# laclouis5/StructureDetector

Measured on AMD Instinct MI355X. Metric: images/sec (train fwd+bwd) and decode us/img at 512x512, higher is better.
Workload: dtype f32

## Files before the change

include/sdnet_hip.h:

```cpp
#ifndef SDNET_HIP_H
#define SDNET_HIP_H

#include <stddef.h>
#include <stdint.h>

#ifdef __cplusplus
extern "C" {
#endif

#define SD_ERR_INVALID   (-1)
#define SD_ERR_WORKSPACE (-2)
#define SD_ERR_ALIGN     (-3)

#define SD_MAX_TOPK 1024

typedef void* sd_stream_t;

int         sd_version(void);
const char* sd_last_error(void);
int         sd_build_flags(void);


int sd_clamped_sigmoid(const float* x, float* y, int64_t n, sd_stream_t stream);

// ... 80 lines not shown

typedef struct sd_loss_desc {
    const float* anchor_hm;  int64_t a_sb, a_sc;
    const float* part_hm;    int64_t p_sb, p_sc;
    const float* offsets;    int64_t o_sb, o_sc;
    const float* embeddings; int64_t e_sb, e_sc;
    const float* t_anchor_hm; int64_t ta_sb, ta_sc;
    const float* t_part_hm;   int64_t tp_sb, tp_sc;
    const int64_t* anchor_inds;
    const int64_t* part_inds;
    const float* anchor_offsets;
    const float* part_offsets;
    const float* t_embeddings;
    const uint8_t* anchor_mask;
    const uint8_t* part_mask;
    int B, M, N, h, w, K, P;
    int hm_loss_fn;
    float hm_weight, offset_weight, embedding_weight;
} sd_loss_desc;

size_t sd_loss_workspace_bytes(int B, int M, int N, int h, int w);
int sd_loss_fwd(const sd_loss_desc* d, float* out8, void* workspace, size_t workspace_bytes, sd_stream_t stream);

int sd_loss_fwd_per_image(const sd_loss_desc* d, float* out, void* workspace, size_t workspace_bytes, sd_stream_t stream);

int sd_loss_bwd(const sd_loss_desc* d, const float* out8, const float* grad_out, float* dhead, sd_stream_t stream);



typedef struct sd_conv_desc {
    int B, Hi, Wi, Cin, Ho, Wo, Cout, R, S, stride, pad;
} sd_conv_desc;

size_t sd_conv2d_fwd_workspace_bytes(const sd_conv_desc* d);
int sd_conv2d_fwd(const float* x_nhwc, const float* w_krsc, float* y_nhwc, const sd_conv_desc* d,
                  const float* scale, const float* shift, const float* residual, int res_up2, int relu,
                  void* workspace, size_t workspace_bytes, sd_stream_t stream);
size_t sd_conv2d_stem_fwd_workspace_bytes(const sd_conv_desc* d);
int sd_conv2d_stem_fwd(const float* x_nchw, const float* w_krsc, void* y_nhwc, const sd_conv_desc* d,
                       const float* scale, const float* shift, int relu, int out_bf16, void* workspace,
                       size_t workspace_bytes, sd_stream_t stream);

int    sd_conv2d_fwd_sb_supported(const sd_conv_desc* d, int bf16);
size_t sd_conv2d_fwd_sb_workspace_bytes(const sd_conv_desc* d, int bf16);
size_t sd_conv2d_fwd_sb_state_bytes(const sd_conv_desc* d, int bf16);
int sd_conv2d_fwd_sb(const void* x_nhwc, const void* w_krsc, void* y_nhwc, const sd_conv_desc* d, const float* scale, const float* shift,
                     const void* residual, int res_up2, int relu, int bf16, void* workspace, size_t workspace_bytes, void* state,
                     size_t state_bytes, sd_stream_t stream);

size_t sd_conv2d_stem_fwd_bn_stats_workspace_bytes(const sd_conv_desc* d);
int sd_conv2d_stem_fwd_bn_stats(const float* x_nchw, const float* w, float* y, const sd_conv_desc* d, float eps, float momentum,
                                float* running_mean, float* running_var, float* mean, float* invstd, void* workspace,
                                size_t workspace_bytes, sd_stream_t stream);

size_t sd_conv2d_fwd_bn_stats_workspace_bytes(const sd_conv_desc* d);
int sd_conv2d_fwd_bn_stats(const float* x, const float* w, float* y, const sd_conv_desc* d, float eps, float momentum,
                           float* running_mean, float* running_var, float* mean, float* invstd, void* workspace,
                           size_t workspace_bytes, sd_stream_t stream);
int sd_bn_finalize_scratch_rows(int rows);
int sd_bn_finalize_stats(const float* partial, int rows, int64_t M, int C, float eps, float momentum, float* running_mean,
                         float* running_var, float* mean, float* invstd, float* scratch, sd_stream_t stream);

size_t sd_conv2d_dgrad_bn_reduce_workspace_bytes(const sd_conv_desc* d);
int sd_conv2d_dgrad_bn_reduce(const float* dy, const float* w_t, float* dx, const sd_conv_desc* d, const float* residual,
                              const float* bn_x, const float* bn_y, int relu, const float* mean, const float* invstd,
                              const float* gamma, const float* beta, float* dgamma, float* dbeta, int accumulate,
                              float* means_out, void* workspace, size_t workspace_bytes, sd_stream_t stream);
int sd_bn_bwd_finalize(const float* partial, int rows, int64_t M, int C, float* dgamma, float* dbeta, int accumulate,
                       float* means_out, float* scratch, sd_stream_t stream);
int sd_bn_bwd_apply(const float* dy, const float* x, const float* y, int relu, int64_t M, int C, const float* mean,
                    const float* invstd, const float* gamma, const float* beta, const float* means, float* dx, float* g_out,
                    sd_stream_t stream);

int sd_set_option(const char* name, int value);

const char* sd_conv2d_kernel_name(const sd_conv_desc* d, int pass);

int sd_cast_f32_to_bf16(const float* x, void* y_bf16, int64_t n, sd_stream_t stream);
size_t sd_conv2d_fwd_bf16_workspace_bytes(const sd_conv_desc* d);
int sd_conv2d_fwd_bf16(const void* x_nhwc_bf16, const void* w_krsc_bf16, void* y_nhwc_bf16, const sd_conv_desc* d,
                       const float* scale, const float* shift, const void* residual_bf16, int res_up2, int relu,
                       void* workspace, size_t workspace_bytes, sd_stream_t stream);
int sd_maxpool3x3s2_fwd_bf16(const void* x_bf16, void* y_bf16, int B, int Hi, int Wi, int C, sd_stream_t stream);
int sd_stem_bn_relu_maxpool_fwd_bf16(const float* x_nchw, const float* w, const float* scale, const float* shift, void* y_bf16,
                                     const sd_conv_desc* d, sd_stream_t stream);

int sd_cast_bf16_to_f32(const void* x_bf16, float* y, int64_t n, sd_stream_t stream);
size_t sd_conv2d_fwd_bf16_bn_stats_workspace_bytes(const sd_conv_desc* d);
int sd_conv2d_fwd_bf16_bn_stats(const void* x_nhwc_bf16, const void* w_krsc_bf16, void* y_nhwc_bf16, const sd_conv_desc* d, float eps,
                                float momentum, float* running_mean, float* running_var, float* mean, float* invstd,
                                void* workspace, size_t workspace_bytes, sd_stream_t stream);
int sd_conv2d_stem_fwd_bn_stats_bf16mm(const float* x_nchw, const float* w, float* y, const sd_conv_desc* d, float eps, float momentum,
                                       float* running_mean, float* running_var, float* mean, float* invstd,
                                       void* workspace, size_t workspace_bytes, sd_stream_t stream);
int sd_conv2d_stem_fwd_bn_stats_bf16(const float* x_nchw, const float* w, void* y_bf16, const sd_conv_desc* d, float eps, float momentum,
                                     float* running_mean, float* running_var, float* mean, float* invstd, void* workspace,
                                     size_t workspace_bytes, sd_stream_t stream);
int sd_bn_relu_maxpool_fwd_bf16(const void* x_bf16, int B, int Hi, int Wi, int C, const float* mean, const float* invstd, const float* gamma,
                                const float* beta, void* y_pool_bf16, uint8_t* idx, sd_stream_t stream);
int sd_maxpool_bn_relu_bwd_bf16(const void* dpool_bf16, const uint8_t* idx, const void* x_bf16, int B, int Hi, int Wi, int C, const float* mean,
                                const float* invstd, const float* gamma, const float* beta, float* dx, float* dgamma, float* dbeta, int accumulate,
                                void* workspace, size_t workspace_bytes, sd_stream_t stream);
int sd_maxpool_bn_relu_bwd_bf16_dx16(const void* dpool_bf16, const uint8_t* idx, const void* x_bf16, int B, int Hi, int Wi, int C, const float* mean,
                                     const float* invstd, const float* gamma, const float* beta, void* dx_bf16, float* dgamma, float* dbeta,
                                     int accumulate, void* workspace, size_t workspace_bytes, sd_stream_t stream);
int sd_conv2d_transpose_weights_bf16(const float* w, void* w_t_bf16, int Cout, int taps, int Cin, sd_stream_t stream);

int sd_conv2d_fwd_bf16_head_supported(const sd_conv_desc* d, int head_co);
size_t sd_head_split_bf16_bytes(void);
int sd_head_split_bf16(const float* head_w, const float* head_bias, int head_co, void* prepared, sd_stream_t stream);
int sd_conv2d_fwd_bf16_head(const void* x_bf16, const void* w_bf16, const sd_conv_desc* d, const float* scale, const float* shift, int relu,
                            const void* head_prepared, int head_co, float* head_y, sd_stream_t stream);
int sd_conv2d_dgrad_bf16(const void* dy_bf16, const void* w_t_bf16, void* dx_bf16, const sd_conv_desc* d, const void* residual_bf16,
                         int res_mode, sd_stream_t stream);
size_t sd_conv2d_wgrad_bf16_workspace_bytes(const sd_conv_desc* d);
int sd_conv2d_wgrad_bf16(const void* dy_bf16, const void* x_nhwc_bf16, float* dw_krsc, const sd_conv_desc* d, int accumulate,
                         void* workspace, size_t workspace_bytes, sd_stream_t stream);
int sd_bn_apply_bf16(const void* x, void* y, int64_t M, int C, const float* mean, const float* invstd, const float* gamma,
                     const float* beta, const void* residual, int relu, uint8_t* relu_mask_out, sd_stream_t stream);
int sd_bn_bwd_bf16(const void* dy, const void* x, const void* y, int relu, int64_t M, int C, const float* mean, const float* invstd,
                   const float* gamma, const float* beta, void* dx, void* g_out, float* dgamma, float* dbeta, int accumulate,
                   void* workspace, size_t workspace_bytes, sd_stream_t stream);
int sd_bn_train_stats_bf16(const void* x, int64_t M, int C, float eps, float momentum, float* running_mean, float* running_var,
                           float* mean, float* invstd, void* workspace, size_t workspace_bytes, sd_stream_t stream);
int sd_col_sum_bf16(const void* x, int64_t M, int C, float* out, int accumulate, void* workspace, size_t workspace_bytes, sd_stream_t stream);
int sd_upsample2x_bwd_bf16(const void* dy, const void* add, void* dx, int B, int H, int W, int C, sd_stream_t stream);
int sd_head_fwd_bf16(const void* x_nhwc_bf16, const float* w, const float* bias, float* y_nchw, int B, int HW, int C,
                     int Co, sd_stream_t stream);
int sd_conv2d_dgrad(const float* dy_nhwc, const float* w_t, float* dx_nhwc, const sd_conv_desc* d,
                    const float* residual, sd_stream_t stream);
int sd_conv2d_dgrad_half_res(const float* dy, const float* w_t, float* dx, const sd_conv_desc* d, const float* residual_half,
                             sd_stream_t stream);
int sd_conv2d_transpose_weights(const float* w, float* w_t, int Cout, int taps, int Cin, sd_stream_t stream);
int sd_conv2d_transpose_weights_batched(const float* w_base, void* w_t_base, const int* table, int nconv, int total_blocks, int out_bf16,
                                        sd_stream_t stream);
size_t sd_conv2d_wgrad_workspace_bytes(const sd_conv_desc* d);
int sd_conv2d_wgrad(const float* dy_nhwc, const float* x_nhwc, float* dw_krsc, const sd_conv_desc* d,
                    int accumulate, void* workspace, size_t workspace_bytes, sd_stream_t stream);
size_t sd_conv2d_stem_wgrad_workspace_bytes(const sd_conv_desc* d);
int sd_conv2d_stem_wgrad(const float* dy_nhwc, const float* x_nchw, float* dw_krsc, const sd_conv_desc* d,
                         int accumulate, void* workspace, size_t workspace_bytes, sd_stream_t stream);
int sd_conv2d_stem_wgrad_bf16mm(const float* dy, const float* x_nchw, float* dw, const sd_conv_desc* d, int accumulate, void* workspace,
                                size_t workspace_bytes, sd_stream_t stream);
int sd_conv2d_stem_wgrad_bf16(const void* dy_bf16, const float* x_nchw, float* dw, const sd_conv_desc* d, int accumulate, void* workspace,
                              size_t workspace_bytes, sd_stream_t stream);

size_t sd_col_reduce_workspace_bytes(int64_t M, int C);
int sd_bn_train_stats(const float* x, int64_t M, int C, float eps, float momentum, float* running_mean,
                      float* running_var, float* mean, float* invstd, void* workspace, size_t workspace_bytes,
                      sd_stream_t stream);
int sd_bn_apply(const float* x, float* y, int64_t M, int C, const float* mean, const float* invstd,
                const float* gamma, const float* beta, const float* residual, int relu, uint8_t* relu_mask_out,
                sd_stream_t stream);
int sd_bn_fold(const float* gamma, const float* beta, const float* running_mean, const float* running_var,
               float eps, int C, float* scale, float* shift, sd_stream_t stream);
int sd_bn_bwd(const float* dy, const float* x, const float* y, int relu, int64_t M, int C, const float* mean,
              const float* invstd, const float* gamma, const float* beta, float* dx, float* g_out, float* dgamma,
              float* dbeta, int accumulate, void* workspace, size_t workspace_bytes, sd_stream_t stream);
int sd_col_sum(const float* x, int64_t M, int C, float* out, int accumulate, void* workspace,
               size_t workspace_bytes, sd_stream_t stream);

int sd_maxpool3x3s2_fwd(const float* x, float* y, uint8_t* idx, int B, int Hi, int Wi, int C, sd_stream_t stream);
int sd_maxpool3x3s2_bwd(const float* dy, const uint8_t* idx, float* dx, int B, int Hi, int Wi, int C, sd_stream_t stream);
int sd_bn_relu_maxpool_fwd(const float* x, int B, int Hi, int Wi, int C, const float* mean, const float* invstd, const float* gamma,
                           const float* beta, float* y_pool, uint8_t* idx, sd_stream_t stream);
int sd_maxpool_bn_relu_bwd(const float* dpool, const uint8_t* idx, const float* x, int B, int Hi, int Wi, int C, const float* mean,
                           const float* invstd, const float* gamma, const float* beta, float* dx, float* dgamma, float* dbeta,
                           int accumulate, void* workspace, size_t workspace_bytes, sd_stream_t stream);
int sd_upsample2x_bwd(const float* dy, const float* add, float* dx, int B, int H, int W, int C, sd_stream_t stream);

#define SD_HEAD_MAX_CO 256
int sd_head_fwd(const float* x_nhwc, const float* w, const float* bias, float* y_nchw, int B, int HW, int C, int Co,
                sd_stream_t stream);
size_t sd_head_bwd_workspace_bytes(int B, int HW, int C, int Co);
int sd_head_bwd(const float* dy_nchw, const float* x_nhwc, const float* w, float* dx_nhwc, float* dw, float* dbias,
                int B, int HW, int C, int Co, int accumulate, void* workspace, size_t workspace_bytes, sd_stream_t stream);
int sd_head_bwd_bf16(const float* dy, const void* x_bf16, const float* w, void* dx_bf16, float* dw, float* dbias, int B, int HW, int C, int Co,
                     int accumulate, void* workspace, size_t workspace_bytes, sd_stream_t stream);

int sd_adam_step(float* param, const float* grad, float* exp_avg, float* exp_avg_sq, int64_t n, int step,
                 float lr, float beta1, float beta2, float eps, float grad_scale, sd_stream_t stream);

#define SD_COMM_ID_BYTES 128
int sd_allreduce_unique_id(void* id_out);
int sd_allreduce_init(const void* id, int rank, int world, void** comm_out);
int sd_allreduce_run(void* comm, float* buf, int64_t count, sd_stream_t stream);
int sd_allreduce_destroy(void* comm);

int sd_comm_sim_copy(const void* src, void* dst, size_t src_bytes, size_t move_bytes, int workgroups, float gbps, sd_stream_t stream);

double sd_mfma_bf16_stream_flops(int iters);
int    sd_mfma_bf16_stream(const void* operands64k, float* out, int iters, sd_stream_t stream);

int         sd_range_enabled(void);
const char* sd_range_library(void);
int         sd_range_push(const char* name);
int         sd_range_pop(void);
int         sd_range_mark(const char* name);

#ifdef __cplusplus
}
#endif
#endif
```

structuredetector_amd/_lib.py:

```python
from __future__ import annotations

import ctypes as C
import os
from pathlib import Path

import torch

_HERE = Path(__file__).resolve().parent
LIB_PATH = Path(os.environ.get("SDNET_HIP_LIB", _HERE / "csrc" / "libsdnet_hip.so"))

_lib = None

c_f32p = C.c_void_p
c_i64 = C.c_int64
c_int = C.c_int
c_float = C.c_float
c_size = C.c_size_t
c_vp = C.c_void_p


class SdError(RuntimeError):
    pass


class LossDesc(C.Structure):
    _fields_ = [
        ("anchor_hm", c_vp), ("a_sb", c_i64), ("a_sc", c_i64),
        ("part_hm", c_vp), ("p_sb", c_i64), ("p_sc", c_i64),
        ("offsets", c_vp), ("o_sb", c_i64), ("o_sc", c_i64),
        ("embeddings", c_vp), ("e_sb", c_i64), ("e_sc", c_i64),
        ("t_anchor_hm", c_vp), ("ta_sb", c_i64), ("ta_sc", c_i64),
        ("t_part_hm", c_vp), ("tp_sb", c_i64), ("tp_sc", c_i64),
        ("anchor_inds", c_vp), ("part_inds", c_vp),
        ("anchor_offsets", c_vp), ("part_offsets", c_vp), ("t_embeddings", c_vp),
        ("anchor_mask", c_vp), ("part_mask", c_vp),
        ("B", c_int), ("M", c_int), ("N", c_int), ("h", c_int), ("w", c_int), ("K", c_int), ("P", c_int),
        ("hm_loss_fn", c_int),
        ("hm_weight", c_float), ("offset_weight", c_float), ("embedding_weight", c_float),
    ]


class ConvDesc(C.Structure):
    _fields_ = [(n, c_int) for n in ("B", "Hi", "Wi", "Cin", "Ho", "Wo", "Cout", "R", "S", "stride", "pad")]


_MAP = [c_vp, c_i64, c_i64]
_PEAK_OUT = [c_vp, c_vp, c_vp, c_vp, c_vp]

_SIGNATURES = {
    "sd_version": (c_int, []),
    "sd_last_error": (C.c_char_p, []),
    "sd_build_flags": (c_int, []),
    "sd_clamped_sigmoid": (c_int, [c_vp, c_vp, c_i64, c_vp]),
    "sd_nms5": (c_int, _MAP + [c_vp, c_int, c_int, c_int, c_int, c_int, c_vp]),
    "sd_topk_workspace_bytes": (c_size, [c_int] * 5),
    "sd_topk": (c_int, _MAP + [c_int] * 5 + _PEAK_OUT + [c_vp, c_size, c_vp]),
    "sd_transpose_and_gather": (c_int, _MAP + [c_int, c_int, c_i64, c_vp, c_int, c_vp, c_vp]),
    "sd_hypot": (c_int, [c_vp, c_vp, c_i64, c_vp]),
    "sd_decode_peaks_workspace_bytes": (c_size, [c_int] * 5),
    "sd_decode_peaks": (c_int, _MAP + [c_int] * 5 + _PEAK_OUT + [c_vp, c_size, c_vp]),
    "sd_decode_workspace_bytes": (c_size, [c_int] * 7),
    "sd_decode_packed_words": (c_size, [c_int] * 3),
    "sd_decode": (c_int, _MAP * 4 + [c_int] * 7 + [c_float, c_float, c_int, c_vp, c_vp, c_size, c_vp]),
    "sd_decode_state_bytes": (c_size, [c_int] * 5),
    "sd_decode_fused_supported": (c_int, [c_int] * 7),
    "sd_decode_fused_recommended": (c_int, [c_int] * 8),
    "sd_stream_synchronize": (c_int, [c_vp]),
    "sd_selfcheck_sigmoid": (c_int, [c_vp, c_vp]),
    "sd_decode_fused_workspace_bytes": (c_size, [c_int] * 7),
    "sd_decode_fused": (c_int, _MAP * 4 + [c_int] * 7 + [c_float, c_float, c_int, c_vp, c_vp, c_size, c_vp, c_size, c_vp]),
    "sd_decode_group": (c_int, [c_vp] * 6 + _MAP * 2 + [c_int] * 5 + [c_float, c_float, c_vp, c_vp]),
    "sd_preprocess_workspace_bytes": (c_size, [c_int] * 4),
    "sd_preprocess_images": (c_int, [c_vp] + [c_int] * 5 + [c_vp, c_vp, c_int, c_vp, c_vp, c_int, c_vp, C.POINTER(c_float), C.POINTER(c_float),
                                                c_vp, c_vp, c_size, c_vp]),
    "sd_preprocess_jitter_workspace_bytes": (c_size, [c_int] * 5),
    "sd_preprocess_images_jitter": (c_int, [c_vp] + [c_int] * 5 + [c_vp, c_vp, c_int, c_vp, c_vp, c_int, c_vp, c_vp, c_vp, C.POINTER(c_float), C.POINTER(c_float),
                                            c_vp, c_vp, c_size, c_vp]),
    "sd_preprocess_images_list": (c_int, [c_vp] + [c_int] * 5 + [c_vp, c_vp, c_int, c_vp, c_vp, c_int, c_vp, C.POINTER(c_float), C.POINTER(c_float),
                                                     c_vp, c_vp, c_size, c_vp]),
    "sd_preprocess_images_list_jitter": (c_int, [c_vp] + [c_int] * 5 + [c_vp, c_vp, c_int, c_vp, c_vp, c_int, c_vp, c_vp, c_vp, C.POINTER(c_float),
                                                            C.POINTER(c_float), c_vp, c_vp, c_size, c_vp]),
    "sd_render_targets": (c_int, [c_vp, c_vp, c_vp, c_int, c_int, c_int, c_int, c_float, c_vp, c_vp]),
    "sd_loss_workspace_bytes": (c_size, [c_int] * 5),
    "sd_loss_fwd": (c_int, [C.POINTER(LossDesc), c_vp, c_vp, c_size, c_vp]),
    "sd_loss_fwd_per_image": (c_int, [C.POINTER(LossDesc), c_vp, c_vp, c_size, c_vp]),
    "sd_loss_bwd": (c_int, [C.POINTER(LossDesc), c_vp, c_vp, c_vp, c_vp]),
    "sd_conv2d_fwd_workspace_bytes": (c_size, [C.POINTER(ConvDesc)]),
    "sd_conv2d_fwd": (c_int, [c_vp, c_vp, c_vp, C.POINTER(ConvDesc), c_vp, c_vp, c_vp, c_int, c_int, c_vp, c_size, c_vp]),
    "sd_conv2d_fwd_sb_supported": (c_int, [C.POINTER(ConvDesc), c_int]),
    "sd_conv2d_fwd_sb_workspace_bytes": (c_size, [C.POINTER(ConvDesc), c_int]),
    "sd_conv2d_fwd_sb_state_bytes": (c_size, [C.POINTER(ConvDesc), c_int]),
    "sd_conv2d_fwd_sb": (c_int, [c_vp, c_vp, c_vp, C.POINTER(ConvDesc), c_vp, c_vp, c_vp, c_int, c_int, c_int, c_vp, c_size, c_vp, c_size, c_vp]),
    "sd_conv2d_stem_fwd_workspace_bytes": (c_size, [C.POINTER(ConvDesc)]),
    "sd_conv2d_stem_fwd": (c_int, [c_vp, c_vp, c_vp, C.POINTER(ConvDesc), c_vp, c_vp, c_int, c_int, c_vp, c_size, c_vp]),
    "sd_cast_f32_to_bf16": (c_int, [c_vp, c_vp, c_i64, c_vp]),
    "sd_conv2d_fwd_bf16_workspace_bytes": (c_size, [C.POINTER(ConvDesc)]),
    "sd_conv2d_fwd_bf16": (c_int, [c_vp, c_vp, c_vp, C.POINTER(ConvDesc), c_vp, c_vp, c_vp, c_int, c_int, c_vp, c_size, c_vp]),
    "sd_conv2d_fwd_bf16_head_supported": (c_int, [C.POINTER(ConvDesc), c_int]),
    "sd_head_split_bf16_bytes": (c_size, []),
    "sd_head_split_bf16": (c_int, [c_vp, c_vp, c_int, c_vp, c_vp]),
    "sd_conv2d_fwd_bf16_head": (c_int, [c_vp, c_vp, C.POINTER(ConvDesc), c_vp, c_vp, c_int, c_vp, c_int, c_vp, c_vp]),
    "sd_cast_bf16_to_f32": (c_int, [c_vp, c_vp, c_i64, c_vp]),
    "sd_conv2d_fwd_bf16_bn_stats_workspace_bytes": (c_size, [c_vp]),
    "sd_conv2d_fwd_bf16_bn_stats": (c_int, [c_vp, c_vp, c_vp, c_vp, c_float, c_float, c_vp, c_vp, c_vp, c_vp, c_vp, c_size, c_vp]),
    "sd_conv2d_wgrad_bf16_workspace_bytes": (c_size, [c_vp]),
    "sd_conv2d_wgrad_bf16": (c_int, [c_vp, c_vp, c_vp, c_vp, c_int, c_vp, c_size, c_vp]),
    "sd_conv2d_transpose_weights_bf16": (c_int, [c_vp, c_vp, c_int, c_int, c_int, c_vp]),
    "sd_conv2d_dgrad_bf16": (c_int, [c_vp, c_vp, c_vp, c_vp, c_vp, c_int, c_vp]),
    "sd_bn_apply_bf16": (c_int, [c_vp, c_vp, c_i64, c_int, c_vp, c_vp, c_vp, c_vp, c_vp, c_int, c_vp, c_vp]),
    "sd_bn_bwd_bf16": (c_int, [c_vp, c_vp, c_vp, c_int, c_i64, c_int, c_vp, c_vp, c_vp, c_vp, c_vp, c_vp, c_vp, c_vp, c_int, c_vp, c_size, c_vp]),
    "sd_bn_train_stats_bf16": (c_int, [c_vp, c_i64, c_int, c_float, c_float, c_vp, c_vp, c_vp, c_vp, c_vp, c_size, c_vp]),
    "sd_col_sum_bf16": (c_int, [c_vp, c_i64, c_int, c_vp, c_int, c_vp, c_size, c_vp]),
    "sd_upsample2x_bwd_bf16": (c_int, [c_vp, c_vp, c_vp, c_int, c_int, c_int, c_int, c_vp]),
    "sd_maxpool3x3s2_fwd_bf16": (c_int, [c_vp, c_vp, c_int, c_int, c_int, c_int, c_vp]),
    "sd_stem_bn_relu_maxpool_fwd_bf16": (c_int, [c_vp, c_vp, c_vp, c_vp, c_vp, c_vp, c_vp]),
    "sd_head_fwd_bf16": (c_int, [c_vp, c_vp, c_vp, c_vp, c_int, c_int, c_int, c_int, c_vp]),
    "sd_conv2d_dgrad": (c_int, [c_vp, c_vp, c_vp, C.POINTER(ConvDesc), c_vp, c_vp]),
    "sd_conv2d_transpose_weights": (c_int, [c_vp, c_vp, c_int, c_int, c_int, c_vp]),
    "sd_conv2d_transpose_weights_batched": (c_int, [c_vp, c_vp, c_vp, c_int, c_int, c_int, c_vp]),
    "sd_conv2d_wgrad_workspace_bytes": (c_size, [C.POINTER(ConvDesc)]),
    "sd_conv2d_wgrad": (c_int, [c_vp, c_vp, c_vp, C.POINTER(ConvDesc), c_int, c_vp, c_size, c_vp]),
    "sd_conv2d_stem_wgrad_workspace_bytes": (c_size, [C.POINTER(ConvDesc)]),
    "sd_conv2d_stem_wgrad": (c_int, [c_vp, c_vp, c_vp, C.POINTER(ConvDesc), c_int, c_vp, c_size, c_vp]),
    "sd_conv2d_stem_wgrad_bf16mm": (c_int, [c_vp, c_vp, c_vp, C.POINTER(ConvDesc), c_int, c_vp, c_size, c_vp]),
    "sd_conv2d_stem_wgrad_bf16": (c_int, [c_vp, c_vp, c_vp, C.POINTER(ConvDesc), c_int, c_vp, c_size, c_vp]),
    "sd_col_reduce_workspace_bytes": (c_size, [c_i64, c_int]),
    "sd_bn_train_stats": (c_int, [c_vp, c_i64, c_int, c_float, c_float, c_vp, c_vp, c_vp, c_vp, c_vp, c_size, c_vp]),
    "sd_bn_apply": (c_int, [c_vp, c_vp, c_i64, c_int, c_vp, c_vp, c_vp, c_vp, c_vp, c_int, c_vp, c_vp]),
    "sd_bn_fold": (c_int, [c_vp, c_vp, c_vp, c_vp, c_float, c_int, c_vp, c_vp, c_vp]),
    "sd_bn_bwd": (c_int, [c_vp, c_vp, c_vp, c_int, c_i64, c_int, c_vp, c_vp, c_vp, c_vp, c_vp, c_vp, c_vp, c_vp, c_int, c_vp, c_size, c_vp]),
    "sd_col_sum": (c_int, [c_vp, c_i64, c_int, c_vp, c_int, c_vp, c_size, c_vp]),
    "sd_maxpool3x3s2_fwd": (c_int, [c_vp, c_vp, c_vp, c_int, c_int, c_int, c_int, c_vp]),
    "sd_maxpool3x3s2_bwd": (c_int, [c_vp, c_vp, c_vp, c_int, c_int, c_int, c_int, c_vp]),
    "sd_upsample2x_bwd": (c_int, [c_vp, c_vp, c_vp, c_int, c_int, c_int, c_int, c_vp]),
    "sd_head_fwd": (c_int, [c_vp, c_vp, c_vp, c_vp, c_int, c_int, c_int, c_int, c_vp]),
    "sd_head_bwd_workspace_bytes": (c_size, [c_int] * 4),
    "sd_head_bwd": (c_int, [c_vp] * 6 + [c_int] * 5 + [c_vp, c_size, c_vp]),
    "sd_head_bwd_bf16": (c_int, [c_vp] * 6 + [c_int] * 5 + [c_vp, c_size, c_vp]),
    "sd_adam_step": (c_int, [c_vp, c_vp, c_vp, c_vp, c_i64, c_int, c_float, c_float, c_float, c_float, c_float, c_vp]),
    "sd_conv2d_kernel_name": (C.c_char_p, [c_vp, c_int]),
    "sd_set_option": (c_int, [C.c_char_p, c_int]),
    "sd_decode_set_option": (c_int, [C.c_char_p, c_int]),
    "sd_conv2d_stem_fwd_bn_stats_workspace_bytes": (c_size, [c_vp]),
    "sd_conv2d_stem_fwd_bn_stats": (c_int, [c_vp, c_vp, c_vp, c_vp, c_float, c_float, c_vp, c_vp, c_vp, c_vp, c_vp, c_size, c_vp]),
    "sd_conv2d_stem_fwd_bn_stats_bf16mm": (c_int, [c_vp, c_vp, c_vp, c_vp, c_float, c_float, c_vp, c_vp, c_vp, c_vp, c_vp, c_size, c_vp]),
    "sd_conv2d_stem_fwd_bn_stats_bf16": (c_int, [c_vp, c_vp, c_vp, c_vp, c_float, c_float, c_vp, c_vp, c_vp, c_vp, c_vp, c_size, c_vp]),
    "sd_conv2d_dgrad_half_res": (c_int, [c_vp] * 6),
    "sd_bn_relu_maxpool_fwd": (c_int, [c_vp, c_int, c_int, c_int, c_int] + [c_vp] * 7),
    "sd_bn_relu_maxpool_fwd_bf16": (c_int, [c_vp, c_int, c_int, c_int, c_int] + [c_vp] * 7),
    "sd_maxpool_bn_relu_bwd": (c_int, [c_vp, c_vp, c_vp, c_int, c_int, c_int, c_int] + [c_vp] * 7 + [c_int, c_vp, c_size, c_vp]),
    "sd_maxpool_bn_relu_bwd_bf16": (c_int, [c_vp, c_vp, c_vp, c_int, c_int, c_int, c_int] + [c_vp] * 7 + [c_int, c_vp, c_size, c_vp]),
    "sd_maxpool_bn_relu_bwd_bf16_dx16": (c_int, [c_vp, c_vp, c_vp, c_int, c_int, c_int, c_int] + [c_vp] * 7 + [c_int, c_vp, c_size, c_vp]),
    "sd_conv2d_fwd_bn_stats_workspace_bytes": (c_size, [c_vp]),
    "sd_conv2d_fwd_bn_stats": (c_int, [c_vp, c_vp, c_vp, c_vp, c_float, c_float, c_vp, c_vp, c_vp, c_vp, c_vp, c_size, c_vp]),
    "sd_conv2d_dgrad_bn_reduce_workspace_bytes": (c_size, [c_vp]),
    "sd_conv2d_dgrad_bn_reduce": (c_int, [c_vp] * 5 + [c_vp, c_vp, c_int] + [c_vp] * 6 + [c_int, c_vp, c_vp, c_size, c_vp]),
    "sd_bn_bwd_finalize": (c_int, [c_vp, c_int, c_i64, c_int, c_vp, c_vp, c_int, c_vp, c_vp, c_vp]),
    "sd_bn_bwd_apply": (c_int, [c_vp, c_vp, c_vp, c_int, c_i64, c_int] + [c_vp] * 8),
    "sd_bn_finalize_scratch_rows": (c_int, [c_int]),
    "sd_bn_finalize_stats": (c_int, [c_vp, c_int, c_i64, c_int, c_float, c_float, c_vp, c_vp, c_vp, c_vp, c_vp, c_vp]),
    "sd_allreduce_unique_id": (c_int, [c_vp]),
    "sd_allreduce_init": (c_int, [c_vp, c_int, c_int, C.POINTER(c_vp)]),
    "sd_allreduce_run": (c_int, [c_vp, c_vp, c_i64, c_vp]),
    "sd_allreduce_destroy": (c_int, [c_vp]),
    "sd_mfma_bf16_stream_flops": (C.c_double, [c_int]),
    "sd_mfma_bf16_stream": (c_int, [c_vp, c_vp, c_int, c_vp]),
    "sd_comm_sim_copy": (c_int, [c_vp, c_vp, c_size, c_size, c_int, c_float, c_vp]),
    "sd_range_enabled": (c_int, []),
    "sd_range_library": (C.c_char_p, []),
    "sd_range_push": (c_int, [C.c_char_p]),
    "sd_range_pop": (c_int, []),
    "sd_range_mark": (c_int, [C.c_char_p]),
}


def declared_symbols():
    return sorted(_SIGNATURES)


def lib():
    global _lib
    if _lib is None:
        if not LIB_PATH.exists():
            raise SdError(
                f"{LIB_PATH} not found: build it with `python -c 'import __graft_entry__ as g; g.build()'` "
                f"(or `make -C {LIB_PATH.parent}`); structuredetector_amd has no CPU / eager fallback.")
        handle = C.CDLL(str(LIB_PATH))
        for name, (res, args) in _SIGNATURES.items():
            fn = getattr(handle, name)
            fn.restype = res
            fn.argtypes = args
        flags = handle.sd_build_flags()
        if flags and os.environ.get("SDNET_ALLOW_ABLATION") != "1":
            raise SdError(f"{LIB_PATH} is a timing-only ablation build (sd_build_flags = {flags}: SD_ABLATE_* switches make the conv "
                          "kernels compute wrong results on purpose); rebuild without EXTRA=-DSD_ABLATE_... "
                          "(set SDNET_ALLOW_ABLATION=1 only for timing experiments)")
        _lib = handle
    return _lib


def check(rc: int, what: str = ""):
    if rc != 0:
        msg = lib().sd_last_error().decode(errors="replace")
        raise SdError(f"{what or 'libsdnet_hip'} failed (code {rc}): {msg}")


def stream() -> int:
    try:
        return torch._C._cuda_getCurrentRawStream(torch.cuda.current_device())
    except AttributeError:
        return torch.cuda.current_stream().cuda_stream


def require_cuda(*tensors):
    for t in tensors:
        if not t.is_cuda:
            raise SdError("structuredetector_amd ops need tensors on the GPU (device 'cuda'); got a "
                          f"{t.device} tensor and there is no CPU fallback")


def map_view(t: torch.Tensor):
    if t.dtype != torch.float32:
        t = t.float()
    B, Cc, h, w = t.shape
    s0, s1, s2, s3 = t.stride()
    ptr = t.data_ptr()
    if not (s3 == 1 and s2 == w and s1 >= h * w and (B == 1 or s0 >= h * w) and s1 % 4 == 0 and s0 % 4 == 0 and ptr % 16 == 0):
        t = t.contiguous()
        s0, s1 = t.stride(0), t.stride(1)
        ptr = t.data_ptr()
    return t, ptr, s0, s1


_ws_cache: dict = {}


def workspace(nbytes: int, device) -> torch.Tensor:
    key = (device.index if device.index is not None else torch.cuda.current_device(), stream())
    buf = _ws_cache.get(key)
    if buf is None or buf.numel() < nbytes:
        buf = torch.empty(max(nbytes, 1 << 20), dtype=torch.uint8, device=device)
        _ws_cache[key] = buf
    return buf


_state_cache: dict = {}


def zero_state(nbytes: int, device, tag: str = "conv") -> torch.Tensor:
    key = (device.index if device.index is not None else torch.cuda.current_device(), stream(), tag)
    buf = _state_cache.get(key)
    if buf is None or buf.numel() < nbytes:
        if buf is not None:
            torch.cuda.current_stream().synchronize()
        buf = torch.zeros(max(nbytes, 1 << 16), dtype=torch.uint8, device=device)
        _state_cache[key] = buf
    return buf
```

structuredetector_amd/csrc/sd_common.h:

```cpp
#pragma once
#include <hip/hip_runtime.h>
#include <stdint.h>
#include <stdio.h>
#include "../../include/sdnet_hip.h"

namespace sd {

void set_error(const char* fmt, ...);

#define SD_REQUIRE(cond, code, ...)            \
    do {                                       \
        if (!(cond)) {                         \
            sd::set_error(__VA_ARGS__);        \
            return (code);                     \
        }                                      \
    } while (0)

#define SD_HIP(call)                                                                    \
    do {                                                                                \
        hipError_t e_ = (call);                                                         \
        if (e_ != hipSuccess) {                                                         \
            sd::set_error("%s failed: %s (%s:%d)", #call, hipGetErrorString(e_), __FILE__, __LINE__); \
            return (int)e_;                                                             \
        }                                                                               \
    } while (0)

#define SD_LAUNCH_CHECK()                                                               \
    do {                                                                                \
        hipError_t e_ = hipGetLastError();                                              \
        if (e_ != hipSuccess) {                                                         \
            sd::set_error("kernel launch failed: %s (%s:%d)", hipGetErrorString(e_), __FILE__, __LINE__); \
            return (int)e_;                                                             \
        }                                                                               \
    } while (0)

static inline bool aligned16(const void* p) { return (reinterpret_cast<uintptr_t>(p) & 15u) == 0; }
static inline size_t align_up(size_t v, size_t a) { return (v + a - 1) / a * a; }
static inline int cdiv(int64_t a, int64_t b) { return (int)((a + b - 1) / b); }

constexpr float kClampLo = 1e-6f;
constexpr float kClampHi = (float)(1.0 - 1e-6);

__device__ __forceinline__ float sigmoid_raw(float x) { return 1.0f / (1.0f + expf(-x)); }
__device__ __forceinline__ float clamped_sigmoid(float x) {
    return fminf(fmaxf(sigmoid_raw(x), kClampLo), kClampHi);
}

__device__ __forceinline__ float bf16_to_f32(uint16_t v) { return __uint_as_float((uint32_t)v << 16); }
__device__ __forceinline__ uint16_t f32_to_bf16(float v) { return __builtin_bit_cast(uint16_t, (__bf16)v); }
typedef float sd_f32x4_nt __attribute__((ext_vector_type(4)));
__device__ __forceinline__ float4 ld4(const float* p, int64_t i) {
    const sd_f32x4_nt v = __builtin_nontemporal_load(reinterpret_cast<const sd_f32x4_nt*>(p) + i);
    return make_float4(v[0], v[1], v[2], v[3]);
}
__device__ __forceinline__ float4 ld4(const uint16_t* p, int64_t i) {
    const uint2 r = reinterpret_cast<const uint2*>(p)[i];
    return make_float4(bf16_to_f32((uint16_t)(r.x & 0xffff)), bf16_to_f32((uint16_t)(r.x >> 16)), bf16_to_f32((uint16_t)(r.y & 0xffff)),
                       bf16_to_f32((uint16_t)(r.y >> 16)));
}
__device__ __forceinline__ void st4(float* p, int64_t i, const float4 v) { reinterpret_cast<float4*>(p)[i] = v; }
__device__ __forceinline__ void st4(uint16_t* p, int64_t i, const float4 v) {
    uint2 pk;
    pk.x = (uint32_t)f32_to_bf16(v.x) | ((uint32_t)f32_to_bf16(v.y) << 16);
    pk.y = (uint32_t)f32_to_bf16(v.z) | ((uint32_t)f32_to_bf16(v.w) << 16);
    reinterpret_cast<uint2*>(p)[i] = pk;
}

constexpr int HEAD_NARROW_MAX_CO = 32;
int head_wide_check(const char* fn, int64_t P, int C, int Co);
int head_wide_fwd(const float* x, const float* w, const float* bias, float* y, int B, int HW, int C, int Co, hipStream_t st);
int head_wide_fwd_bf16(const void* x, const float* w, const float* bias, float* y, int B, int HW, int C, int Co, hipStream_t st);
size_t head_wide_bwd_workspace_bytes(int64_t P, int C, int Co);
int head_wide_wgrad(const float* dy, const float* x, float* partial, int B, int HW, int C, int Co, hipStream_t st, int& rows);
int head_wide_dgrad(const float* dy, const float* w, float* dx, int B, int HW, int C, int Co, hipStream_t st);

__device__ __forceinline__ float wave_sum(float v) {
#pragma unroll
    for (int o = 32; o > 0; o >>= 1) v += __shfl_down(v, o, 64);
    return v;
}
__device__ __forceinline__ double wave_sum(double v) {
#pragma unroll
    for (int o = 32; o > 0; o >>= 1) v += __shfl_down(v, o, 64);
    return v;
}

}
```

structuredetector_amd/csrc/sd_nn.hip:

```cpp
#include "sd_common.h"
#include "sd_mfma.h"
#include <type_traits>

namespace sd {

constexpr int RED_ROWS_PER_BLOCK = 256;

template <int MODE, typename T = float>
__global__ __launch_bounds__(256) void k_col_reduce(const T* __restrict__ a, const T* __restrict__ b, const T* __restrict__ y,
                                                     const float* __restrict__ mean, const float* __restrict__ invstd,
                                                     const float* __restrict__ gamma, const float* __restrict__ beta, int relu,
                                                     int64_t M, int C, float* __restrict__ partial, int rpb) {
    __shared__ float4 red[2][256];
    const int cols = C >> 2;
    const int lanes = 256 / cols;
    const int col = threadIdx.x % cols, rl = threadIdx.x / cols;
    const int64_t r0 = (int64_t)blockIdx.x * rpb;
    const int64_t r1 = min(r0 + rpb, M);
    float4 s0 = make_float4(0.f, 0.f, 0.f, 0.f), s1 = s0;
    float4 mu = s0, is = s0, ga = s0, be = s0;
    if (MODE == 1 && rl < lanes) {
        mu = reinterpret_cast<const float4*>(mean)[col];
        is = reinterpret_cast<const float4*>(invstd)[col];
        if (relu == 2) { ga = reinterpret_cast<const float4*>(gamma)[col]; be = reinterpret_cast<const float4*>(beta)[col]; }
    }
    if (rl < lanes) {
#pragma unroll 4
        for (int64_t r = r0 + rl; r < r1; r += lanes) {
            const float4 v = ld4(a, r * cols + col);
            if (MODE == 0) {
                s0.x += v.x; s0.y += v.y; s0.z += v.z; s0.w += v.w;
                s1.x += v.x * v.x; s1.y += v.y * v.y; s1.z += v.z * v.z; s1.w += v.w * v.w;
            } else if (MODE == 2) {
                s0.x += v.x; s0.y += v.y; s0.z += v.z; s0.w += v.w;
            } else {
                float4 g = v;
                const float4 xv = ld4(b, r * cols + col);
                if (relu == 1) {
                    const float4 yy = ld4(y, r * cols + col);
                    g.x = yy.x > 0.f ? g.x : 0.f; g.y = yy.y > 0.f ? g.y : 0.f;
                    g.z = yy.z > 0.f ? g.z : 0.f; g.w = yy.w > 0.f ? g.w : 0.f;
                } else if (relu == 2) {
                    g.x = ((xv.x - mu.x) * is.x * ga.x + be.x) > 0.f ? g.x : 0.f; g.y = ((xv.y - mu.y) * is.y * ga.y + be.y) > 0.f ? g.y : 0.f;
                    g.z = ((xv.z - mu.z) * is.z * ga.z + be.z) > 0.f ? g.z : 0.f; g.w = ((xv.w - mu.w) * is.w * ga.w + be.w) > 0.f ? g.w : 0.f;
                } else if (relu == 3) {
                    const uint8_t mb = reinterpret_cast<const uint8_t*>(y)[r * cols + col];
                    g.x = (mb & 1) ? g.x : 0.f; g.y = (mb & 2) ? g.y : 0.f; g.z = (mb & 4) ? g.z : 0.f; g.w = (mb & 8) ? g.w : 0.f;
                }
                s0.x += g.x; s0.y += g.y; s0.z += g.z; s0.w += g.w;
                s1.x += g.x * ((xv.x - mu.x) * is.x); s1.y += g.y * ((xv.y - mu.y) * is.y);
                s1.z += g.z * ((xv.z - mu.z) * is.z); s1.w += g.w * ((xv.w - mu.w) * is.w);
            }
        }
    }
    red[0][threadIdx.x] = s0;
    red[1][threadIdx.x] = s1;
    __syncthreads();
    if (rl == 0) {
        for (int l = 1; l < lanes; ++l) {
            const float4 u = red[0][l * cols + col], w = red[1][l * cols + col];
            s0.x += u.x; s0.y += u.y; s0.z += u.z; s0.w += u.w;
            s1.x += w.x; s1.y += w.y; s1.z += w.z; s1.w += w.w;
        }
        float* dst = partial + (int64_t)blockIdx.x * 2 * C;
        reinterpret_cast<float4*>(dst)[col] = s0;
        reinterpret_cast<float4*>(dst + C)[col] = s1;
    }
}

__global__ __launch_bounds__(256) void k_rows_fold(const float* __restrict__ in, int rows, int W, int slab, float* __restrict__ out) {
    __shared__ float4 red[256];
    const int cols = W >> 2, lanes = 256 / cols;
    const int col = threadIdx.x % cols, rl = threadIdx.x / cols;
    const int r0 = blockIdx.x * slab, r1 = min(r0 + slab, rows);
    float4 s = make_float4(0.f, 0.f, 0.f, 0.f);
    if (rl < lanes) {
#pragma unroll 4
        for (int r = r0 + rl; r < r1; r += lanes) {
            const float4 v = reinterpret_cast<const float4*>(in + (int64_t)r * W)[col];
            s.x += v.x; s.y += v.y; s.z += v.z; s.w += v.w;
        }
    }
    red[threadIdx.x] = s;
    __syncthreads();
    if (rl == 0) {
        for (int l = 1; l < lanes; ++l) { const float4 u = red[l * cols + col]; s.x += u.x; s.y += u.y; s.z += u.z; s.w += u.w; }
        reinterpret_cast<float4*>(out + (int64_t)blockIdx.x * W)[col] = s;
    }
}

template <int FIN>
__global__ __launch_bounds__(256) void k_col_finalize(const float* __restrict__ partial, int nblocks, int C, double M, float eps,
                                                       float momentum, float* __restrict__ out0, float* __restrict__ out1,
                                                       float* __restrict__ run_mean, float* __restrict__ run_var,
                                                       float* __restrict__ aux0, float* __restrict__ aux1, int accumulate) {
    __shared__ double r0[4][4], r1[4][4];
    const int lc = threadIdx.x & 3, lr = threadIdx.x >> 2;
    const int c = blockIdx.x * 4 + lc;
    double s0 = 0.0, s1 = 0.0;
    if (c < C) {
        double t0[8] = {0, 0, 0, 0, 0, 0, 0, 0}, t1[8] = {0, 0, 0, 0, 0, 0, 0, 0};
        for (int b = lr; b < nblocks; b += 64 * 8) {
            float v0[8], v1[8];
#pragma unroll
            for (int u = 0; u < 8; ++u) {
                const int row = b + 64 * u;
                const int64_t o = (int64_t)(row < nblocks ? row : 0) * 2 * C + c;
                v0[u] = partial[o];
                v1[u] = partial[o + C];
            }
#pragma unroll
            for (int u = 0; u < 8; ++u) {
                const bool ok = b + 64 * u < nblocks;
                t0[u] += ok ? (double)v0[u] : 0.0; t1[u] += ok ? (double)v1[u] : 0.0;
            }
        }
        s0 = ((t0[0] + t0[1]) + (t0[2] + t0[3])) + ((t0[4] + t0[5]) + (t0[6] + t0[7]));
        s1 = ((t1[0] + t1[1]) + (t1[2] + t1[3])) + ((t1[4] + t1[5]) + (t1[6] + t1[7]));
    }
#pragma unroll
    for (int o = 4; o < 64; o <<= 1) { s0 += __shfl_xor(s0, o); s1 += __shfl_xor(s1, o); }
    if ((threadIdx.x & 63) < 4) { r0[threadIdx.x >> 6][lc] = s0; r1[threadIdx.x >> 6][lc] = s1; }
    __syncthreads();
    if (lr != 0 || c >= C) return;
    s0 = (r0[0][lc] + r0[1][lc]) + (r0[2][lc] + r0[3][lc]);
    s1 = (r1[0][lc] + r1[1][lc]) + (r1[2][lc] + r1[3][lc]);
    if (FIN == 0) {
        const double mean = s0 / M;
        const double var = fmax(s1 / M - mean * mean, 0.0);
        out0[c] = (float)mean;
        out1[c] = (float)(1.0 / sqrt(var + (double)eps));
        if (run_mean) {
            const double unb = M > 1.0 ? var * M / (M - 1.0) : var;
            run_mean[c] = (float)((1.0 - momentum) * run_mean[c] + momentum * mean);
            run_var[c] = (float)((1.0 - momentum) * run_var[c] + momentum * unb);
        }
    } else if (FIN == 1) {
        out0[c] = (accumulate ? out0[c] : 0.f) + (float)s1;
        out1[c] = (accumulate ? out1[c] : 0.f) + (float)s0;
        aux0[c] = (float)(s0 / M);
        aux1[c] = (float)(s1 / M);
    } else {
        out0[c] = (accumulate ? out0[c] : 0.f) + (float)s0;
    }
}

template <typename T>
__global__ __launch_bounds__(256) void k_bn_apply(const T* __restrict__ x, T* __restrict__ y, int64_t n4, int C,
                                                   const float* __restrict__ mean, const float* __restrict__ invstd,
                                                   const float* __restrict__ gamma, const float* __restrict__ beta,
                                                   const T* __restrict__ res, int relu, uint8_t* __restrict__ mask) {
    const int64_t stride = (int64_t)gridDim.x * 256;
    const int cols = C >> 2;
    const bool fixed = stride % cols == 0;
    const int col0 = (int)(((int64_t)blockIdx.x * 256 + threadIdx.x) % cols);
    float4 mu = reinterpret_cast<const float4*>(mean)[col0], is = reinterpret_cast<const float4*>(invstd)[col0];
    float4 g = reinterpret_cast<const float4*>(gamma)[col0], b = reinterpret_cast<const float4*>(beta)[col0];
    for (int64_t i = (int64_t)blockIdx.x * 256 + threadIdx.x; i < n4; i += stride) {
        const float4 v = ld4(x, i);
        if (!fixed) {
            const int col = (int)(i % cols);
            mu = reinterpret_cast<const float4*>(mean)[col]; is = reinterpret_cast<const float4*>(invstd)[col];
            g = reinterpret_cast<const float4*>(gamma)[col]; b = reinterpret_cast<const float4*>(beta)[col];
        }
        float4 o;
        o.x = (v.x - mu.x) * is.x * g.x + b.x; o.y = (v.y - mu.y) * is.y * g.y + b.y;
        o.z = (v.z - mu.z) * is.z * g.z + b.z; o.w = (v.w - mu.w) * is.w * g.w + b.w;
        if (res) {
            const float4 r = ld4(res, i);
            o.x += r.x; o.y += r.y; o.z += r.z; o.w += r.w;
        }
        if (mask) mask[i] = (uint8_t)((o.x > 0.f ? 1 : 0) | (o.y > 0.f ? 2 : 0) | (o.z > 0.f ? 4 : 0) | (o.w > 0.f ? 8 : 0));
        if (relu) { o.x = fmaxf(o.x, 0.f); o.y = fmaxf(o.y, 0.f); o.z = fmaxf(o.z, 0.f); o.w = fmaxf(o.w, 0.f); }
        st4(y, i, o);
    }
}

__global__ __launch_bounds__(256) void k_bn_fold(const float* gamma, const float* beta, const float* rm, const float* rv, float eps,
                                                  int C, float* scale, float* shift) {
    const int c = blockIdx.x * 256 + threadIdx.x;
    if (c >= C) return;
    const float s = gamma[c] / sqrtf(rv[c] + eps);
    scale[c] = s;
    shift[c] = beta[c] - rm[c] * s;
}

template <typename T>
__global__ __launch_bounds__(256) void k_bn_bwd_apply(const T* __restrict__ dy, const T* __restrict__ x, const T* __restrict__ y,
                                                       int relu, int64_t n4, int C, const float* __restrict__ mean,
                                                       const float* __restrict__ invstd, const float* __restrict__ gamma,
                                                       const float* __restrict__ beta, const float* __restrict__ mg,
                                                       const float* __restrict__ mgx, T* __restrict__ dx, T* __restrict__ g_out) {
    const int64_t stride = (int64_t)gridDim.x * 256;
    const int cols = C >> 2;
    const bool fixed = stride % cols == 0;
    const int col0 = (int)(((int64_t)blockIdx.x * 256 + threadIdx.x) % cols);
    float4 mu = reinterpret_cast<const float4*>(mean)[col0], is = reinterpret_cast<const float4*>(invstd)[col0];
    float4 ga = reinterpret_cast<const float4*>(gamma)[col0];
    float4 be = relu == 2 ? reinterpret_cast<const float4*>(beta)[col0] : make_float4(0.f, 0.f, 0.f, 0.f);
    float4 a = reinterpret_cast<const float4*>(mg)[col0], b = reinterpret_cast<const float4*>(mgx)[col0];
    for (int64_t i = (int64_t)blockIdx.x * 256 + threadIdx.x; i < n4; i += stride) {
        float4 g = ld4(dy, i);
        const float4 xv = ld4(x, i);
        if (!fixed) {
            const int col = (int)(i % cols);
            mu = reinterpret_cast<const float4*>(mean)[col]; is = reinterpret_cast<const float4*>(invstd)[col];
            ga = reinterpret_cast<const float4*>(gamma)[col];
            if (relu == 2) be = reinterpret_cast<const float4*>(beta)[col];
            a = reinterpret_cast<const float4*>(mg)[col]; b = reinterpret_cast<const float4*>(mgx)[col];
        }
        if (relu == 1) {
            const float4 yy = ld4(y, i);
            g.x = yy.x > 0.f ? g.x : 0.f; g.y = yy.y > 0.f ? g.y : 0.f; g.z = yy.z > 0.f ? g.z : 0.f; g.w = yy.w > 0.f ? g.w : 0.f;
        } else if (relu == 3) {
            const uint8_t mb = reinterpret_cast<const uint8_t*>(y)[i];
            g.x = (mb & 1) ? g.x : 0.f; g.y = (mb & 2) ? g.y : 0.f; g.z = (mb & 4) ? g.z : 0.f; g.w = (mb & 8) ? g.w : 0.f;
        } else if (relu == 2) {
            g.x = ((xv.x - mu.x) * is.x * ga.x + be.x) > 0.f ? g.x : 0.f; g.y = ((xv.y - mu.y) * is.y * ga.y + be.y) > 0.f ? g.y : 0.f;
            g.z = ((xv.z - mu.z) * is.z * ga.z + be.z) > 0.f ? g.z : 0.f; g.w = ((xv.w - mu.w) * is.w * ga.w + be.w) > 0.f ? g.w : 0.f;
        }
        float4 o;
        o.x = ga.x * is.x * (g.x - a.x - (xv.x - mu.x) * is.x * b.x);
        o.y = ga.y * is.y * (g.y - a.y - (xv.y - mu.y) * is.y * b.y);
        o.z = ga.z * is.z * (g.z - a.z - (xv.z - mu.z) * is.z * b.z);
        o.w = ga.w * is.w * (g.w - a.w - (xv.w - mu.w) * is.w * b.w);
        st4(dx, i, o);
        if (g_out) st4(g_out, i, g);
    }
}

__global__ __launch_bounds__(256) void k_maxpool_fwd(const float* __restrict__ x, float* __restrict__ y, uint8_t* __restrict__ idx, int B,
                                                      int Hi, int Wi, int Ho, int Wo, int C) {
    const int cols = C >> 2;
    const int64_t n4 = (int64_t)B * Ho * Wo * cols;
    const int64_t i = (int64_t)blockIdx.x * 256 + threadIdx.x;
    if (i >= n4) return;
    const int col = (int)(i % cols);
    int64_t t = i / cols;
    const int ox = (int)(t % Wo); t /= Wo;
    const int oy = (int)(t % Ho);
    const int b = (int)(t / Ho);
    float4 m = make_float4(-INFINITY, -INFINITY, -INFINITY, -INFINITY);
    uchar4 w = make_uchar4(0, 0, 0, 0);
#pragma unroll
    for (int r = 0; r < 3; ++r) {
#pragma unroll
        for (int s = 0; s < 3; ++s) {
            const int iy = oy * 2 - 1 + r, ix = ox * 2 - 1 + s;
            if (iy < 0 || iy >= Hi || ix < 0 || ix >= Wi) continue;
            const float4 v = reinterpret_cast<const float4*>(x + (((int64_t)b * Hi + iy) * Wi + ix) * C)[col];
            const uint8_t tap = (uint8_t)(r * 3 + s);
            if (v.x > m.x) { m.x = v.x; w.x = tap; }
            if (v.y > m.y) { m.y = v.y; w.y = tap; }
            if (v.z > m.z) { m.z = v.z; w.z = tap; }
            if (v.w > m.w) { m.w = v.w; w.w = tap; }
        }
    }
    reinterpret_cast<float4*>(y)[i] = m;
    reinterpret_cast<uchar4*>(idx)[i] = w;
}

__global__ __launch_bounds__(256) void k_maxpool_bwd(const float* __restrict__ dy, const uint8_t* __restrict__ idx, float* __restrict__ dx,
                                                      int B, int Hi, int Wi, int Ho, int Wo, int C) {
    const int cols = C >> 2;
    const int64_t n4 = (int64_t)B * Hi * Wi * cols;
    const int64_t i = (int64_t)blockIdx.x * 256 + threadIdx.x;
    if (i >= n4) return;
    const int col = (int)(i % cols);
    int64_t t = i / cols;
    const int ix = (int)(t % Wi); t /= Wi;
    const int iy = (int)(t % Hi);
    const int b = (int)(t / Hi);
    float4 acc = make_float4(0.f, 0.f, 0.f, 0.f);
    for (int oy = (iy + 1) / 2 - ((iy + 1) % 2 == 0 ? 1 : 0); oy <= (iy + 1) / 2; ++oy) {
        if (oy < 0 || oy >= Ho) continue;
        const int r = iy - (oy * 2 - 1);
        if (r < 0 || r > 2) continue;
        for (int ox = (ix + 1) / 2 - ((ix + 1) % 2 == 0 ? 1 : 0); ox <= (ix + 1) / 2; ++ox) {
            if (ox < 0 || ox >= Wo) continue;
            const int s = ix - (ox * 2 - 1);
            if (s < 0 || s > 2) continue;
            const int64_t o = (((int64_t)b * Ho + oy) * Wo + ox) * cols + col;
            const uchar4 w = reinterpret_cast<const uchar4*>(idx)[o];
            const float4 g = reinterpret_cast<const float4*>(dy)[o];
            const uint8_t tap = (uint8_t)(r * 3 + s);
            if (w.x == tap) acc.x += g.x;
            if (w.y == tap) acc.y += g.y;
            if (w.z == tap) acc.z += g.z;
            if (w.w == tap) acc.w += g.w;
        }
    }
    reinterpret_cast<float4*>(dx)[i] = acc;
}

template <typename XT, typename PT>
__global__ __launch_bounds__(256) void k_bn_relu_maxpool_fwd(const XT* __restrict__ x, const float* __restrict__ mean,
                                                              const float* __restrict__ invstd, const float* __restrict__ gamma,
                                                              const float* __restrict__ beta, PT* __restrict__ y,
                                                              uint8_t* __restrict__ idx, int B, int Hi, int Wi, int Ho, int Wo, int C) {
    const int cols = C >> 2;
    const int64_t n4 = (int64_t)B * Ho * Wo * cols;
    const int64_t i = (int64_t)blockIdx.x * 256 + threadIdx.x;
    if (i >= n4) return;
    const int col = (int)(i % cols);
    int64_t t = i / cols;
    const int ox = (int)(t % Wo); t /= Wo;
    const int oy = (int)(t % Ho);
    const int b = (int)(t / Ho);
    const float4 mu = reinterpret_cast<const float4*>(mean)[col], is = reinterpret_cast<const float4*>(invstd)[col];
    const float4 ga = reinterpret_cast<const float4*>(gamma)[col], be = reinterpret_cast<const float4*>(beta)[col];
    float4 m = make_float4(-INFINITY, -INFINITY, -INFINITY, -INFINITY);
    uchar4 w = make_uchar4(0, 0, 0, 0);
#pragma unroll
    for (int r = 0; r < 3; ++r) {
#pragma unroll
        for (int s = 0; s < 3; ++s) {
            const int iy = oy * 2 - 1 + r, ix = ox * 2 - 1 + s;
            if (iy < 0 || iy >= Hi || ix < 0 || ix >= Wi) continue;
            const float4 xv = ld4(x, (((int64_t)b * Hi + iy) * Wi + ix) * cols + col);
            float4 v;
            v.x = fmaxf((xv.x - mu.x) * is.x * ga.x + be.x, 0.f); v.y = fmaxf((xv.y - mu.y) * is.y * ga.y + be.y, 0.f);
            v.z = fmaxf((xv.z - mu.z) * is.z * ga.z + be.z, 0.f); v.w = fmaxf((xv.w - mu.w) * is.w * ga.w + be.w, 0.f);
            const uint8_t tap = (uint8_t)(r * 3 + s);
            if (v.x > m.x) { m.x = v.x; w.x = tap; }
// ... 201 lines not shown
    const float4 ga = reinterpret_cast<const float4*>(gamma)[col], be = reinterpret_cast<const float4*>(beta)[col];
    const float4 a = reinterpret_cast<const float4*>(mg)[col], bb = reinterpret_cast<const float4*>(mgx)[col];
    const int64_t p00 = (((int64_t)b * Hi + 2 * k) * Wi + 2 * j) * cols + col;
    const int64_t off[4] = {p00, p00 + cols, p00 + (int64_t)Wi * cols, p00 + (int64_t)(Wi + 1) * cols};
    float4 xv[4], g[4];
#pragma unroll
    for (int u = 0; u < 4; ++u) xv[u] = ld4(x, off[u]);
    pool_relu_grad_quad(dpool, idx, b, k, j, col, cols, Ho, Wo, xv, mu, is, ga, be, g);
#pragma unroll
    for (int u = 0; u < 4; ++u) {
        float4 o;
        o.x = ga.x * is.x * (g[u].x - a.x - (xv[u].x - mu.x) * is.x * bb.x);
        o.y = ga.y * is.y * (g[u].y - a.y - (xv[u].y - mu.y) * is.y * bb.y);
        o.z = ga.z * is.z * (g[u].z - a.z - (xv[u].z - mu.z) * is.z * bb.z);
        o.w = ga.w * is.w * (g[u].w - a.w - (xv[u].w - mu.w) * is.w * bb.w);
        st4(dx, off[u], o);
    }
}
#undef SD_ADD4

__global__ __launch_bounds__(256) void k_pool_bn_bwd_reduce(const float* __restrict__ dpool, const uint8_t* __restrict__ idx,
                                                             const float* __restrict__ x, const float* __restrict__ mean,
                                                             const float* __restrict__ invstd, const float* __restrict__ gamma,
                                                             const float* __restrict__ beta, int Hi, int Wi, int Ho, int Wo, int64_t M,
                                                             int C, float* __restrict__ partial) {
    __shared__ float4 red[2][256];
    const int cols = C >> 2, lanes = 256 / cols;
    const int col = threadIdx.x % cols, rl = threadIdx.x / cols;
    const int64_t r0 = (int64_t)blockIdx.x * RED_ROWS_PER_BLOCK, r1 = min(r0 + RED_ROWS_PER_BLOCK, M);
    float4 s0 = make_float4(0.f, 0.f, 0.f, 0.f), s1 = s0;
    if (rl < lanes) {
        const float4 mu = reinterpret_cast<const float4*>(mean)[col], is = reinterpret_cast<const float4*>(invstd)[col];
        const float4 ga = reinterpret_cast<const float4*>(gamma)[col], be = reinterpret_cast<const float4*>(beta)[col];
        for (int64_t r = r0 + rl; r < r1; r += lanes) {
            const int ix = (int)(r % Wi);
            const int64_t t = r / Wi;
            const int iy = (int)(t % Hi), b = (int)(t / Hi);
            const float4 xv = reinterpret_cast<const float4*>(x + r * C)[col];
            const float4 g = pool_relu_grad(dpool, idx, b, iy, ix, col, cols, Ho, Wo, xv, mu, is, ga, be);
            s0.x += g.x; s0.y += g.y; s0.z += g.z; s0.w += g.w;
            s1.x += g.x * ((xv.x - mu.x) * is.x); s1.y += g.y * ((xv.y - mu.y) * is.y);
            s1.z += g.z * ((xv.z - mu.z) * is.z); s1.w += g.w * ((xv.w - mu.w) * is.w);
        }
    }
    red[0][threadIdx.x] = s0;
    red[1][threadIdx.x] = s1;
    __syncthreads();
    if (rl == 0) {
        for (int l = 1; l < lanes; ++l) {
            const float4 u = red[0][l * cols + col], w = red[1][l * cols + col];
            s0.x += u.x; s0.y += u.y; s0.z += u.z; s0.w += u.w;
            s1.x += w.x; s1.y += w.y; s1.z += w.z; s1.w += w.w;
        }
        float* dst = partial + (int64_t)blockIdx.x * 2 * C;
        reinterpret_cast<float4*>(dst)[col] = s0;
        reinterpret_cast<float4*>(dst + C)[col] = s1;
    }
}

__global__ __launch_bounds__(256) void k_pool_bn_bwd_apply(const float* __restrict__ dpool, const uint8_t* __restrict__ idx,
                                                            const float* __restrict__ x, const float* __restrict__ mean,
                                                            const float* __restrict__ invstd, const float* __restrict__ gamma,
                                                            const float* __restrict__ beta, const float* __restrict__ mg,
                                                            const float* __restrict__ mgx, int Hi, int Wi, int Ho, int Wo, int64_t n4, int C,
                                                            float* __restrict__ dx) {
    const int64_t i = (int64_t)blockIdx.x * 256 + threadIdx.x;
    if (i >= n4) return;
    const int cols = C >> 2;
    const int col = (int)(i % cols);
    const int64_t r = i / cols;
    const int ix = (int)(r % Wi);
    const int64_t t = r / Wi;
    const int iy = (int)(t % Hi), b = (int)(t / Hi);
    const float4 mu = reinterpret_cast<const float4*>(mean)[col], is = reinterpret_cast<const float4*>(invstd)[col];
    const float4 ga = reinterpret_cast<const float4*>(gamma)[col], be = reinterpret_cast<const float4*>(beta)[col];
    const float4 xv = reinterpret_cast<const float4*>(x)[i];
    const float4 g = pool_relu_grad(dpool, idx, b, iy, ix, col, cols, Ho, Wo, xv, mu, is, ga, be);
    const float4 a = reinterpret_cast<const float4*>(mg)[col], bb = reinterpret_cast<const float4*>(mgx)[col];
    float4 o;
    o.x = ga.x * is.x * (g.x - a.x - (xv.x - mu.x) * is.x * bb.x);
    o.y = ga.y * is.y * (g.y - a.y - (xv.y - mu.y) * is.y * bb.y);
    o.z = ga.z * is.z * (g.z - a.z - (xv.z - mu.z) * is.z * bb.z);
    o.w = ga.w * is.w * (g.w - a.w - (xv.w - mu.w) * is.w * bb.w);
    reinterpret_cast<float4*>(dx)[i] = o;
}

template <typename T>
__global__ __launch_bounds__(256) void k_up2_bwd(const T* __restrict__ dy, const T* __restrict__ add, T* __restrict__ dx, int B,
                                                  int H, int W, int C) {
    const int cols = C >> 2;
    const int64_t n4 = (int64_t)B * H * W * cols;
    const int64_t i = (int64_t)blockIdx.x * 256 + threadIdx.x;
    if (i >= n4) return;
    const int col = (int)(i % cols);
    int64_t t = i / cols;
    const int x = (int)(t % W); t /= W;
    const int y = (int)(t % H);
    const int b = (int)(t / H);
    const T* base = dy + (((int64_t)b * 2 * H + 2 * y) * 2 * W + 2 * x) * C;
    const float4 v0 = ld4(base, col), v1 = ld4(base + C, col);
    const float4 v2 = ld4(base + (int64_t)2 * W * C, col);
    const float4 v3 = ld4(base + (int64_t)2 * W * C + C, col);
    float4 o = make_float4(v0.x + v1.x + v2.x + v3.x, v0.y + v1.y + v2.y + v3.y, v0.z + v1.z + v2.z + v3.z, v0.w + v1.w + v2.w + v3.w);
    if (add) {
        const float4 a = ld4(add, i);
        o.x += a.x; o.y += a.y; o.z += a.z; o.w += a.w;
    }
    st4(dx, i, o);
}

__global__ __launch_bounds__(256) void k_head_fwd(const float* __restrict__ x, const float* __restrict__ w, const float* __restrict__ bias,
                                                   float* __restrict__ y, int64_t M, int HW, int C, int Co) {
    extern __shared__ __attribute__((aligned(16))) float lds[];
    const int LD = C + 4;
    float* xs = lds;
    float* ws = lds + 64 * LD;
    const int64_t m0 = (int64_t)blockIdx.x * 64;
    const int c4 = C >> 2;
    for (int i = threadIdx.x; i < 64 * c4; i += 256) {
        const int row = i / c4, col = i - row * c4;
        const int64_t m = m0 + row;
        const float4 v = m < M ? reinterpret_cast<const float4*>(x + m * C)[col] : make_float4(0.f, 0.f, 0.f, 0.f);
        *reinterpret_cast<float4*>(xs + row * LD + col * 4) = v;
    }
    for (int i = threadIdx.x; i < Co * C; i += 256) ws[i] = w[i];
    __syncthreads();
    const int px = threadIdx.x & 63, grp = threadIdx.x >> 6;
    float acc[HEAD_NARROW_MAX_CO / 4];
#pragma unroll
    for (int j = 0; j < HEAD_NARROW_MAX_CO / 4; ++j) acc[j] = 0.f;
    for (int c = 0; c < C; c += 4) {
        const float4 v = *reinterpret_cast<const float4*>(xs + px * LD + c);
#pragma unroll
        for (int j = 0; j < HEAD_NARROW_MAX_CO / 4; ++j) {
            const int co = grp + 4 * j;
            if (co < Co) {
                const float4 ww = *reinterpret_cast<const float4*>(ws + co * C + c);
                acc[j] += v.x * ww.x + v.y * ww.y + v.z * ww.z + v.w * ww.w;
            }
        }
    }
    const int64_t m = m0 + px;
    if (m < M) {
        const int64_t b = m / HW, pix = m - b * HW;
#pragma unroll
        for (int j = 0; j < HEAD_NARROW_MAX_CO / 4; ++j) {
            const int co = grp + 4 * j;
            if (co < Co) y[(b * Co + co) * HW + pix] = acc[j] + bias[co];
        }
    }
}

constexpr int HF_NST = 4;
__global__ __launch_bounds__(256) void k_head_fwd_f32_c128(const float* __restrict__ x, const float* __restrict__ w, const float* __restrict__ bias,
                                                            float* __restrict__ y, int HW, int Co, int ntiles) {
    extern __shared__ __attribute__((aligned(16))) float hf_lds[];
    const int lane = threadIdx.x & 63, wave = __builtin_amdgcn_readfirstlane(threadIdx.x >> 6);
    float* const T = hf_lds + wave * (HF_NST * 2048);
    const uint32_t t_base = lds_addr(T);
    const int row = lane & 15, kq = lane >> 4;
    f32x4 bw[8];
#pragma unroll
    for (int j = 0; j < 8; ++j) {
        bw[j] = f32x4{0.f, 0.f, 0.f, 0.f};
        if (row < Co) bw[j] = *reinterpret_cast<const f32x4*>(w + row * 128 + 16 * j + 4 * kq);
    }
    const float bv = row < Co ? bias[row] : 0.f;
    const int nwaves = gridDim.x * 4;
    const int dr = lane >> 5, dsl = lane & 31;
#define HF_ISSUE(t_, st_)                                                                                          \
    {                                                                                                              \
        const int64_t m0_ = (int64_t)min((t_), ntiles - 1) * 16;                                                  \
        _Pragma("unroll") for (int d = 0; d < 8; ++d) {                                                            \
            const int r = 2 * d + dr;                                                                              \
            lds_dma16(x + (m0_ + r) * 128 + ((dsl ^ (r & 15)) << 2), T + (st_) * 2048 + d * 256);                   \
        }                                                                                                          \
    }
    int tile = blockIdx.x * 4 + wave;
#pragma unroll
    for (int s = 0; s < HF_NST - 1; ++s) HF_ISSUE(tile + s * nwaves, s)
    int stage = 0;
    for (; tile < ntiles; tile += nwaves) {
        const int nst = stage == 0 ? HF_NST - 1 : stage - 1;
        HF_ISSUE(tile + (HF_NST - 1) * nwaves, nst)
        wait_vmcnt<8 * (HF_NST - 1)>();
        const uint32_t a0 = t_base + (uint32_t)stage * 8192u + (uint32_t)row * 512u;
        f32x4 a[8];
#pragma unroll
        for (int j = 0; j < 8; ++j) a[j] = lds_read128_async<0>(a0 + (uint32_t)(((4 * j + kq) ^ row) << 4));
        SD_LDS_WAIT4(0, a[0], a[1], a[2], a[3]);
        SD_LDS_WAIT4(0, a[4], a[5], a[6], a[7]);
        f32x4 acc0 = {0.f, 0.f, 0.f, 0.f}, acc1 = {0.f, 0.f, 0.f, 0.f};
#pragma unroll
        for (int j = 0; j < 8; j += 2)
#pragma unroll
            for (int t = 0; t < 4; ++t) {
                acc0 = __builtin_amdgcn_mfma_f32_16x16x4f32(a[j][t], bw[j][t], acc0, 0, 0, 0);
                acc1 = __builtin_amdgcn_mfma_f32_16x16x4f32(a[j + 1][t], bw[j + 1][t], acc1, 0, 0, 0);
            }
        if (row < Co) {
            const uint32_t m0 = (uint32_t)tile * 16u;
            const uint32_t b = m0 / (uint32_t)HW, pix = m0 - b * (uint32_t)HW;
            const f32x4 o = {acc0[0] + acc1[0] + bv, acc0[1] + acc1[1] + bv, acc0[2] + acc1[2] + bv, acc0[3] + acc1[3] + bv};
            *reinterpret_cast<f32x4*>(y + ((int64_t)b * Co + row) * HW + pix + 4 * kq) = o;
        }
        stage = stage + 1 == HF_NST ? 0 : stage + 1;
    }
    wait_vmcnt<0>();
#undef HF_ISSUE
}

constexpr int HEAD_WG_PIX = 1024;
template <typename T>
__global__ __launch_bounds__(256) void k_head_dgrad(const float* __restrict__ dy, const float* __restrict__ w, T* __restrict__ dx,
                                                     int64_t M, int HW, int C, int Co) {
    __shared__ float gs[HEAD_NARROW_MAX_CO][64];
    extern __shared__ __attribute__((aligned(16))) float lds[];
    float* ws = lds;
    const int64_t m0 = (int64_t)blockIdx.x * 64;
    for (int i = threadIdx.x; i < Co * 64; i += 256) {
        const int co = i >> 6, px = i & 63;
        const int64_t m = m0 + px;
        float v = 0.f;
        if (m < M) { const int64_t b = m / HW, pix = m - b * HW; v = dy[(b * Co + co) * HW + pix]; }
        gs[co][px] = v;
    }
    for (int i = threadIdx.x; i < Co * C; i += 256) ws[i] = w[i];
    __syncthreads();
    const int c4 = C >> 2;
    for (int i = threadIdx.x; i < 64 * c4; i += 256) {
        const int row = i / c4, col = i - row * c4;
        const int64_t m = m0 + row;
        if (m >= M) continue;
        float4 o = make_float4(0.f, 0.f, 0.f, 0.f);
        for (int co = 0; co < Co; ++co) {
            const float g = gs[co][row];
            const float4 ww = *reinterpret_cast<const float4*>(ws + co * C + col * 4);
            o.x += g * ww.x; o.y += g * ww.y; o.z += g * ww.z; o.w += g * ww.w;
        }
        if constexpr (sizeof(T) == 2) {
            uint2 pk;
            pk.x = (uint32_t)f32_to_bf16(o.x) | ((uint32_t)f32_to_bf16(o.y) << 16);
            pk.y = (uint32_t)f32_to_bf16(o.z) | ((uint32_t)f32_to_bf16(o.w) << 16);
            reinterpret_cast<uint2*>(dx + m * C)[col] = pk;
        } else {
            reinterpret_cast<float4*>(dx + m * C)[col] = o;
        }
    }
}

template <int CO>
__global__ __launch_bounds__(256) void k_head_wgrad_bf16(const float* __restrict__ dy, const uint16_t* __restrict__ x, float* __restrict__ partial,
                                                          int64_t M, int HW, int C, int Co) {
    __shared__ float gs[CO][64];
    __shared__ float comb[4][CO * 128];
    const int64_t mb = (int64_t)blockIdx.x * HEAD_WG_PIX;
    const int CG = C >> 3, PL = 256 / CG;
    const int cg = threadIdx.x % CG, pl = threadIdx.x / CG;
    float acc[CO][8];
#pragma unroll
    for (int j = 0; j < CO; ++j)
#pragma unroll
        for (int k = 0; k < 8; ++k) acc[j][k] = 0.f;
    float bsum = 0.f;
    for (int64_t m0 = mb; m0 < min(mb + HEAD_WG_PIX, M); m0 += 64) {
        __syncthreads();
        for (int i = threadIdx.x; i < Co * 64; i += 256) {
            const int co = i >> 6, px = i & 63;
            const int64_t m = m0 + px;
            float v = 0.f;
            if (m < M) { const int64_t b = m / HW, pix = m - b * HW; v = dy[(b * Co + co) * HW + pix]; }
            gs[co][px] = v;
        }
        __syncthreads();
        for (int p0 = 0; p0 < 64; p0 += 4 * PL) {
            uint4 xv[4];
#pragma unroll
            for (int u = 0; u < 4; ++u) {
                const int px = p0 + u * PL + pl;
                const int64_t m = m0 + px;
                xv[u] = reinterpret_cast<const uint4*>(x + (px < 64 && m < M ? m : mb) * C)[cg];
            }
#pragma unroll
            for (int u = 0; u < 4; ++u) {
                const int px = p0 + u * PL + pl;
                if (px >= 64) continue;
                const float f[8] = {__uint_as_float(xv[u].x << 16), __uint_as_float(xv[u].x & 0xffff0000u), __uint_as_float(xv[u].y << 16),
                                    __uint_as_float(xv[u].y & 0xffff0000u), __uint_as_float(xv[u].z << 16), __uint_as_float(xv[u].z & 0xffff0000u),
                                    __uint_as_float(xv[u].w << 16), __uint_as_float(xv[u].w & 0xffff0000u)};
#pragma unroll
                for (int j = 0; j < CO; ++j) {
                    if (j < Co) {
                        const float g = gs[j][px];
#pragma unroll
                        for (int k = 0; k < 8; ++k) acc[j][k] += g * f[k];
                    }
                }
            }
        }
        if (threadIdx.x < Co) {
            for (int px = 0; px < 64; ++px) bsum += gs[threadIdx.x][px];
        }
    }
    const int lane = threadIdx.x & 63, wave = threadIdx.x >> 6;
#pragma unroll
    for (int j = 0; j < CO; ++j)
#pragma unroll
        for (int k = 0; k < 8; ++k) {
            float v = acc[j][k];
            for (int o = CG; o < 64; o <<= 1) v += __shfl_xor(v, o);
            acc[j][k] = v;
        }
    if (lane < CG) {
#pragma unroll
        for (int j = 0; j < CO; ++j)
            if (j < Co) {
#pragma unroll
                for (int k = 0; k < 8; ++k) comb[wave][j * C + lane * 8 + k] = acc[j][k];
            }
    }
    __syncthreads();
    float* dst = partial + (int64_t)blockIdx.x * (Co * C + Co);
    for (int i = threadIdx.x; i < Co * C; i += 256) dst[i] = (comb[0][i] + comb[1][i]) + (comb[2][i] + comb[3][i]);
    if (threadIdx.x < Co) dst[Co * C + threadIdx.x] = bsum;
}

__global__ __launch_bounds__(256) void k_head_wgrad(const float* __restrict__ dy, const float* __restrict__ x, float* __restrict__ partial,
                                                     int64_t M, int HW, int C, int Co) {
    __shared__ float gs[HEAD_NARROW_MAX_CO][64];
    __shared__ float comb[HEAD_NARROW_MAX_CO][256];
    const int64_t mb = (int64_t)blockIdx.x * HEAD_WG_PIX;
    const int halves = max(1, 256 / C);
    const int c = threadIdx.x % C, hf = threadIdx.x / C;
    const int span = 64 / halves;
    float acc[HEAD_NARROW_MAX_CO];
#pragma unroll
    for (int j = 0; j < HEAD_NARROW_MAX_CO; ++j) acc[j] = 0.f;
    float bsum = 0.f;
    for (int64_t m0 = mb; m0 < min(mb + HEAD_WG_PIX, M); m0 += 64) {
        __syncthreads();
        for (int i = threadIdx.x; i < Co * 64; i += 256) {
            const int co = i >> 6, px = i & 63;
            const int64_t m = m0 + px;
            float v = 0.f;
            if (m < M) { const int64_t b = m / HW, pix = m - b * HW; v = dy[(b * Co + co) * HW + pix]; }
            gs[co][px] = v;
        }
        __syncthreads();
        if (hf < halves) {
            const int p0 = hf * span;
#pragma unroll 1
            for (int pb = 0; pb < span; pb += 8) {
                float xv[8];
#pragma unroll
                for (int u = 0; u < 8; ++u) {
                    const int64_t m = m0 + p0 + pb + u;
                    xv[u] = x[(m < M ? m : mb) * C + c];
                }
#pragma unroll
                for (int u = 0; u < 8; ++u)
#pragma unroll
                    for (int j = 0; j < HEAD_NARROW_MAX_CO; ++j)
                        if (j < Co) acc[j] += gs[j][p0 + pb + u] * xv[u];
            }
        }
        if (threadIdx.x < Co) {
            for (int px = 0; px < 64; ++px) bsum += gs[threadIdx.x][px];
        }
    }
    for (int j = 0; j < Co; ++j) comb[j][threadIdx.x] = (hf < halves) ? acc[j] : 0.f;
    __syncthreads();
    float* dst = partial + (int64_t)blockIdx.x * (Co * C + Co);
    if (threadIdx.x < C) {
        for (int j = 0; j < Co; ++j) {
            float t = 0.f;
            for (int h2 = 0; h2 < halves; ++h2) t += comb[j][h2 * C + threadIdx.x];
            dst[j * C + threadIdx.x] = t;
        }
    }
    if (threadIdx.x < Co) dst[Co * C + threadIdx.x] = bsum;
}

constexpr int HWG_STAGE = 2048 + 256;
__global__ __launch_bounds__(256) void k_head_wgrad_f32_c128(const float* __restrict__ dy, const float* __restrict__ x, float* __restrict__ partial,
                                                              int HW, int Co, int ntiles) {
    extern __shared__ __attribute__((aligned(16))) float hw_lds[];
    const int lane = threadIdx.x & 63, wave = __builtin_amdgcn_readfirstlane(threadIdx.x >> 6);
    float* const T = hw_lds + wave * (HF_NST * HWG_STAGE);
    const uint32_t t_base = lds_addr(T);
    const int n = lane & 15, kq = lane >> 4;
    const int gw = blockIdx.x * 4 + wave, nwaves = gridDim.x * 4;
    const int dr = lane >> 5, dsl = lane & 31;
    const int nco = min(n, Co - 1);
#define HWG_ISSUE(t_, st_)                                                                                         \
    {                                                                                                              \
        const uint32_t m0_ = (uint32_t)min((t_), ntiles - 1) * 16u;                              \
        const uint32_t b_ = m0_ / (uint32_t)HW, pix_ = m0_ - b_ * (uint32_t)HW;                                     \
        _Pragma("unroll") for (int d = 0; d < 8; ++d) {                                                            \
            const int r = 2 * d + dr;                                                                              \
            lds_dma16(x + ((int64_t)m0_ + r) * 128 + ((dsl ^ (r & 15)) << 2), T + (st_) * HWG_STAGE + d * 256);     \
        }                                                                                                          \
        lds_dma16(dy + ((int64_t)b_ * Co + nco) * HW + pix_ + 4 * kq, T + (st_) * HWG_STAGE + 2048);               \
    }
    f32x4 acc[8];
#pragma unroll
    for (int cb = 0; cb < 8; ++cb) acc[cb] = f32x4{0.f, 0.f, 0.f, 0.f};
    float bsum = 0.f;
    int tile = gw;
#pragma unroll
    for (int s = 0; s < HF_NST - 1; ++s) HWG_ISSUE(tile + s * nwaves, s)
    int stage = 0;
    for (; tile < ntiles; tile += nwaves) {
        const int nst = stage == 0 ? HF_NST - 1 : stage - 1;
        HWG_ISSUE(tile + (HF_NST - 1) * nwaves, nst)
        wait_vmcnt<9 * (HF_NST - 1)>();
        const uint32_t s0 = t_base + (uint32_t)stage * (HWG_STAGE * 4);
        f32x4 a = lds_read128_async<0>(s0 + 8192u + (uint32_t)lane * 16u);
        f32x4 xa[4], xb[4];
#pragma unroll
        for (int i = 0; i < 4; ++i) {
            const uint32_t row = (uint32_t)(4 * kq + i);
            xa[i] = lds_read128_async<0>(s0 + row * 512u + (((uint32_t)n ^ (row & 15u)) << 4));
            xb[i] = lds_read128_async<0>(s0 + row * 512u + (((uint32_t)(16 + n) ^ (row & 15u)) << 4));
        }
        SD_LDS_WAIT4(0, xa[0], xa[1], xa[2], xa[3]);
        SD_LDS_WAIT4(0, xb[0], xb[1], xb[2], xb[3]);
        SD_LDS_WAIT2(0, a, xa[0]);
        if (n >= Co) a = f32x4{0.f, 0.f, 0.f, 0.f};
#pragma unroll
        for (int i = 0; i < 4; ++i)
#pragma unroll
            for (int cb = 0; cb < 4; ++cb) {
                acc[cb] = __builtin_amdgcn_mfma_f32_16x16x4f32(a[i], xa[i][cb], acc[cb], 0, 0, 0);
                acc[4 + cb] = __builtin_amdgcn_mfma_f32_16x16x4f32(a[i], xb[i][cb], acc[4 + cb], 0, 0, 0);
            }
        bsum += (a[0] + a[1]) + (a[2] + a[3]);
        stage = stage + 1 == HF_NST ? 0 : stage + 1;
    }
    wait_vmcnt<0>();
#undef HWG_ISSUE
    float* dst = partial + (int64_t)gw * (Co * 128 + Co);
#pragma unroll
    for (int r = 0; r < 4; ++r) {
        const int co = 4 * kq + r;
        if (co < Co) {
#pragma unroll
            for (int cb = 0; cb < 4; ++cb) { dst[co * 128 + 4 * n + cb] = acc[cb][r]; dst[co * 128 + 64 + 4 * n + cb] = acc[4 + cb][r]; }
        }
    }
    bsum += __shfl_xor(bsum, 16);
    bsum += __shfl_xor(bsum, 32);
    if (kq == 0 && n < Co) dst[Co * 128 + n] = bsum;
}

__global__ __launch_bounds__(256) void k_head_wgrad_fin(const float* __restrict__ partial, int nblocks, int n, float* __restrict__ dw,
                                                         float* __restrict__ db, int nw, int accumulate) {
    __shared__ double red[32][8];
    const int lo = threadIdx.x & 7, lr = threadIdx.x >> 3;
    const int i = blockIdx.x * 8 + lo;
    double s = 0.0;
    if (i < n)
        for (int b = lr; b < nblocks; b += 32) s += (double)partial[(int64_t)b * n + i];
    red[lr][lo] = s;
    __syncthreads();
    if (lr != 0 || i >= n) return;
    for (int k = 1; k < 32; ++k) s += red[k][lo];
    float* dst = i < nw ? dw + i : db + (i - nw);
    *dst = (accumulate ? *dst : 0.f) + (float)s;
}

__global__ __launch_bounds__(256) void k_adam(float* __restrict__ p, const float* __restrict__ g, float* __restrict__ m,
                                               float* __restrict__ v, int64_t n4, float lr, float b1, float b2, float eps, float bc1,
                                               float bc2_sqrt, float gscale) {
    const int64_t stride = (int64_t)gridDim.x * 256;
    for (int64_t i = (int64_t)blockIdx.x * 256 + threadIdx.x; i < n4; i += stride) {
        float4 pp = reinterpret_cast<float4*>(p)[i];
        const float4 gg = reinterpret_cast<const float4*>(g)[i];
        float4 mm = reinterpret_cast<float4*>(m)[i], vv = reinterpret_cast<float4*>(v)[i];
        float* P = &pp.x; const float* G = &gg.x; float* Mo = &mm.x; float* V = &vv.x;
#pragma unroll
        for (int j = 0; j < 4; ++j) {
            const float gr = G[j] * gscale;
            Mo[j] = b1 * Mo[j] + (1.f - b1) * gr;
            V[j] = b2 * V[j] + (1.f - b2) * gr * gr;
            const float denom = sqrtf(V[j]) / bc2_sqrt + eps;
            P[j] -= (lr / bc1) * (Mo[j] / denom);
        }
        reinterpret_cast<float4*>(p)[i] = pp;
        reinterpret_cast<float4*>(m)[i] = mm;
        reinterpret_cast<float4*>(v)[i] = vv;
    }
}

__device__ __forceinline__ float bf2f_(uint16_t v) { return __uint_as_float((uint32_t)v << 16); }
__device__ __forceinline__ uint16_t f2bf_(float v) { return __builtin_bit_cast(uint16_t, (__bf16)v); }

__global__ __launch_bounds__(256) void k_cast_bf16(const float* __restrict__ x, uint16_t* __restrict__ y, int64_t n4) {
    const int64_t stride = (int64_t)gridDim.x * 256;
    for (int64_t i = (int64_t)blockIdx.x * 256 + threadIdx.x; i < n4; i += stride) {
        const float4 v = reinterpret_cast<const float4*>(x)[i];
        reinterpret_cast<ushort4*>(y)[i] = make_ushort4(f2bf_(v.x), f2bf_(v.y), f2bf_(v.z), f2bf_(v.w));
    }
}

__global__ __launch_bounds__(256) void k_cast_f32(const uint16_t* __restrict__ x, float* __restrict__ y, int64_t n4) {
    const int64_t stride = (int64_t)gridDim.x * 256;
    for (int64_t i = (int64_t)blockIdx.x * 256 + threadIdx.x; i < n4; i += stride) st4(y, i, ld4(x, i));
}

__global__ __launch_bounds__(256) void k_maxpool_fwd_bf16(const uint16_t* __restrict__ x, uint16_t* __restrict__ y, int B, int Hi, int Wi,
                                                           int Ho, int Wo, int C) {
    const int cols = C >> 3;
    const int64_t n8 = (int64_t)B * Ho * Wo * cols;
    const int64_t i = (int64_t)blockIdx.x * 256 + threadIdx.x;
    if (i >= n8) return;
    const int col = (int)(i % cols);
    int64_t t = i / cols;
    const int ox = (int)(t % Wo); t /= Wo;
    const int oy = (int)(t % Ho);
    const int b = (int)(t / Ho);
    float m[8];
#pragma unroll
    for (int j = 0; j < 8; ++j) m[j] = -INFINITY;
#pragma unroll
    for (int r = 0; r < 3; ++r)
#pragma unroll
        for (int s = 0; s < 3; ++s) {
            const int iy = oy * 2 - 1 + r, ix = ox * 2 - 1 + s;
            if (iy < 0 || iy >= Hi || ix < 0 || ix >= Wi) continue;
            const uint4 v = reinterpret_cast<const uint4*>(x + (((int64_t)b * Hi + iy) * Wi + ix) * C)[col];
            const uint32_t w[4] = {v.x, v.y, v.z, v.w};
#pragma unroll
            for (int j = 0; j < 4; ++j) {
                m[2 * j] = fmaxf(m[2 * j], __uint_as_float(w[j] << 16));
                m[2 * j + 1] = fmaxf(m[2 * j + 1], __uint_as_float(w[j] & 0xffff0000u));
            }
        }
    uint4 o;
    o.x = (uint32_t)f2bf_(m[0]) | ((uint32_t)f2bf_(m[1]) << 16); o.y = (uint32_t)f2bf_(m[2]) | ((uint32_t)f2bf_(m[3]) << 16);
    o.z = (uint32_t)f2bf_(m[4]) | ((uint32_t)f2bf_(m[5]) << 16); o.w = (uint32_t)f2bf_(m[6]) | ((uint32_t)f2bf_(m[7]) << 16);
    reinterpret_cast<uint4*>(y)[i] = o;
}

__global__ __launch_bounds__(256) void k_head_fwd_bf16(const uint16_t* __restrict__ x, const float* __restrict__ w, const float* __restrict__ bias,
                                                        float* __restrict__ y, int64_t M, int HW, int C, int Co) {
    extern __shared__ __attribute__((aligned(16))) float lds[];
    const int LD = C + 4;
    float* xs = lds;
    float* ws = lds + 64 * LD;
    const int64_t m0 = (int64_t)blockIdx.x * 64;
    const int c8 = C >> 3;
    for (int i = threadIdx.x; i < 64 * c8; i += 256) {
        const int row = i / c8, col = i - row * c8;
        const int64_t m = m0 + row;
        uint4 v = make_uint4(0, 0, 0, 0);
        if (m < M) v = reinterpret_cast<const uint4*>(x + m * C)[col];
        float* d = xs + row * LD + col * 8;
        d[0] = __uint_as_float(v.x << 16); d[1] = __uint_as_float(v.x & 0xffff0000u);
        d[2] = __uint_as_float(v.y << 16); d[3] = __uint_as_float(v.y & 0xffff0000u);
        d[4] = __uint_as_float(v.z << 16); d[5] = __uint_as_float(v.z & 0xffff0000u);
        d[6] = __uint_as_float(v.w << 16); d[7] = __uint_as_float(v.w & 0xffff0000u);
    }
    for (int i = threadIdx.x; i < Co * C; i += 256) ws[i] = w[i];
    __syncthreads();
    const int px = threadIdx.x & 63, grp = threadIdx.x >> 6;
    float acc[HEAD_NARROW_MAX_CO / 4];
#pragma unroll
    for (int j = 0; j < HEAD_NARROW_MAX_CO / 4; ++j) acc[j] = 0.f;
    for (int c = 0; c < C; c += 4) {
        const float4 v = *reinterpret_cast<const float4*>(xs + px * LD + c);
#pragma unroll
        for (int j = 0; j < HEAD_NARROW_MAX_CO / 4; ++j) {
            const int co = grp + 4 * j;
            if (co < Co) {
                const float4 ww = *reinterpret_cast<const float4*>(ws + co * C + c);
                acc[j] += v.x * ww.x + v.y * ww.y + v.z * ww.z + v.w * ww.w;
            }
        }
    }
    const int64_t m = m0 + px;
    if (m < M) {
        const int64_t b = m / HW, pix = m - b * HW;
#pragma unroll
        for (int j = 0; j < HEAD_NARROW_MAX_CO / 4; ++j) {
            const int co = grp + 4 * j;
            if (co < Co) y[(b * Co + co) * HW + pix] = acc[j] + bias[co];
        }
    }
}

typedef float head_f32x16 __attribute__((ext_vector_type(16)));
typedef __bf16 head_bf16x8 __attribute__((ext_vector_type(8)));
template <bool SPLIT>
__global__ __launch_bounds__(256) void k_head_fwd_bf16_c128(const uint16_t* __restrict__ x, const float* __restrict__ w, const float* __restrict__ bias,
                                                             float* __restrict__ y, int64_t M, int HW, int Co, int ntiles) {
    __shared__ __attribute__((aligned(16))) float lds[4 * 4096];
    const int lane = threadIdx.x & 63, wave = __builtin_amdgcn_readfirstlane(threadIdx.x >> 6);
    float* T = lds + wave * 4096;
    const int nwaves = gridDim.x * 4;
    const int rsub = lane >> 4, slot = lane & 15;
    const int fr = lane & 31, fh = lane >> 5;
    head_bf16x8 bh[8], bl[8];
    {
        const int n = SPLIT ? fr : (fr & 15);
        const bool lo_col = !SPLIT && fr >= 16;
// ... 181 lines not shown
        st8(dx, i, o);
        if (g_out) st8(g_out, i, gm);
    }
}

__global__ __launch_bounds__(256) void k_col_reduce_bwd_bf16x8(const uint16_t* __restrict__ a, const uint16_t* __restrict__ b, const uint8_t* __restrict__ maskb,
                                                                const float* __restrict__ mean, const float* __restrict__ invstd,
                                                                const float* __restrict__ gamma, const float* __restrict__ beta, int relu,
                                                                int64_t M, int C, float* __restrict__ partial, int rpb) {
    __shared__ float4 red[4][256];
    const int cols = C >> 3;
    const int lanes = 256 / cols;
    const int col = threadIdx.x % cols, rl = threadIdx.x / cols;
    const int64_t r0 = (int64_t)blockIdx.x * rpb, r1 = min(r0 + rpb, M);
    float4 s0[2], s1[2], mu[2], is[2], ga[2], be[2];
#pragma unroll
    for (int h = 0; h < 2; ++h) {
        s0[h] = s1[h] = ga[h] = be[h] = make_float4(0.f, 0.f, 0.f, 0.f);
        mu[h] = reinterpret_cast<const float4*>(mean)[2 * col + h]; is[h] = reinterpret_cast<const float4*>(invstd)[2 * col + h];
        if (relu == 2) { ga[h] = reinterpret_cast<const float4*>(gamma)[2 * col + h]; be[h] = reinterpret_cast<const float4*>(beta)[2 * col + h]; }
    }
    if (rl < lanes) {
#pragma unroll 2
        for (int64_t r = r0 + rl; r < r1; r += lanes) {
            const F8 gy = ld8(a, r * cols + col), xv = ld8(b, r * cols + col);
            uchar2 mb = make_uchar2(0, 0);
            if (relu == 3) mb = reinterpret_cast<const uchar2*>(maskb)[r * cols + col];
#pragma unroll
            for (int h = 0; h < 2; ++h) {
                const float4 xx = h ? xv.b : xv.a;
                const float4 g = bn_mask4(h ? gy.b : gy.a, xx, mu[h], is[h], ga[h], be[h], relu, h ? mb.y : mb.x);
                s0[h].x += g.x; s0[h].y += g.y; s0[h].z += g.z; s0[h].w += g.w;
                s1[h].x += g.x * ((xx.x - mu[h].x) * is[h].x); s1[h].y += g.y * ((xx.y - mu[h].y) * is[h].y);
                s1[h].z += g.z * ((xx.z - mu[h].z) * is[h].z); s1[h].w += g.w * ((xx.w - mu[h].w) * is[h].w);
            }
        }
    }
    red[0][threadIdx.x] = s0[0]; red[1][threadIdx.x] = s0[1]; red[2][threadIdx.x] = s1[0]; red[3][threadIdx.x] = s1[1];
    __syncthreads();
    if (rl == 0) {
        for (int l = 1; l < lanes; ++l) {
#pragma unroll
            for (int h = 0; h < 2; ++h) {
                const float4 u = red[h][l * cols + col], w = red[2 + h][l * cols + col];
                s0[h].x += u.x; s0[h].y += u.y; s0[h].z += u.z; s0[h].w += u.w;
                s1[h].x += w.x; s1[h].y += w.y; s1[h].z += w.z; s1[h].w += w.w;
            }
        }
        float* dst = partial + (int64_t)blockIdx.x * 2 * C;
#pragma unroll
        for (int h = 0; h < 2; ++h) {
            reinterpret_cast<float4*>(dst)[2 * col + h] = s0[h];
            reinterpret_cast<float4*>(dst + C)[2 * col + h] = s1[h];
        }
    }
}

static inline int ew_grid(int64_t n4) { return (int)std::min<int64_t>(cdiv(n4, 256), 256 * 16); }

}

using namespace sd;

static thread_local int g_pool_pair = 1;
namespace sd { void sd_nn_set_pool_pair(int v) { g_pool_pair = v; } }

extern "C" {

static int red_rows(int64_t M) {
    int r = RED_ROWS_PER_BLOCK;
    while (r > 16 && M / r < 1024) r >>= 1;
    return r;
}

static int fold_rows(int rows) { return rows > 2048 ? cdiv(rows, std::max(16, rows / 128)) : 0; }

size_t sd_col_reduce_workspace_bytes(int64_t M, int C) {
    const int nb = cdiv(M, red_rows(M));
    return align_up(((size_t)nb + fold_rows(nb)) * 2 * C * sizeof(float) + 2 * (size_t)C * sizeof(float), 256);
}

static const float* fold_partials(const float* partial, int& rows, int C, float* scratch, hipStream_t st) {
    if (!scratch || fold_rows(rows) == 0 || 2 * C > 1024) return partial;
    const int slab = std::max(16, rows / 128), nb2 = cdiv(rows, slab);
    hipLaunchKernelGGL(k_rows_fold, dim3(nb2), dim3(256), 0, st, partial, rows, 2 * C, slab, scratch);
    rows = nb2;
    return scratch;
}

static int check_mc(const char* what, int64_t M, int C) {
    SD_REQUIRE(M > 0 && C > 0 && C % 4 == 0 && C <= 1024 && (C / 4) <= 256 && 256 % (C / 4) == 0, SD_ERR_INVALID,
               "%s: needs M > 0 and C in {4..1024} with C/4 dividing 256 (got M=%lld C=%d)", what, (long long)M, C);
    return 0;
}

int sd_bn_train_stats(const float* x, int64_t M, int C, float eps, float momentum, float* running_mean, float* running_var,
                      float* mean, float* invstd, void* workspace, size_t workspace_bytes, sd_stream_t stream) {
    if (int e = check_mc("sd_bn_train_stats", M, C)) return e;
    SD_REQUIRE(x && mean && invstd && workspace, SD_ERR_INVALID, "sd_bn_train_stats: null pointer");
    SD_REQUIRE(workspace_bytes >= sd_col_reduce_workspace_bytes(M, C), SD_ERR_WORKSPACE, "sd_bn_train_stats: workspace too small");
    const int rpb = red_rows(M), nb = cdiv(M, rpb);
    hipStream_t st = (hipStream_t)stream;
    hipLaunchKernelGGL(k_col_reduce<0>, dim3(nb), dim3(256), 0, st, x, (const float*)nullptr, (const float*)nullptr, (const float*)nullptr,
                       (const float*)nullptr, (const float*)nullptr, (const float*)nullptr, 0, M, C, (float*)workspace, rpb);
    SD_LAUNCH_CHECK();
    int rows = nb;
    const float* fin = fold_partials((const float*)workspace, rows, C, (float*)workspace + ((size_t)nb + 1) * 2 * C, st);
    hipLaunchKernelGGL(k_col_finalize<0>, dim3(cdiv(C, 4)), dim3(256), 0, st, fin, rows, C, (double)M, eps, momentum,
                       mean, invstd, running_mean, running_var, (float*)nullptr, (float*)nullptr, 0);
    SD_LAUNCH_CHECK();
    return 0;
}

int sd_bn_train_stats_bf16(const void* x, int64_t M, int C, float eps, float momentum, float* running_mean, float* running_var,
                           float* mean, float* invstd, void* workspace, size_t workspace_bytes, sd_stream_t stream) {
    if (int e = check_mc("sd_bn_train_stats_bf16", M, C)) return e;
    SD_REQUIRE(x && mean && invstd && workspace, SD_ERR_INVALID, "sd_bn_train_stats_bf16: null pointer");
    SD_REQUIRE(workspace_bytes >= sd_col_reduce_workspace_bytes(M, C), SD_ERR_WORKSPACE, "sd_bn_train_stats_bf16: workspace too small");
    const int rpb = red_rows(M), nb = cdiv(M, rpb);
    hipStream_t st = (hipStream_t)stream;
    hipLaunchKernelGGL((k_col_reduce<0, uint16_t>), dim3(nb), dim3(256), 0, st, (const uint16_t*)x, (const uint16_t*)nullptr, (const uint16_t*)nullptr,
                       (const float*)nullptr, (const float*)nullptr, (const float*)nullptr, (const float*)nullptr, 0, M, C, (float*)workspace, rpb);
    SD_LAUNCH_CHECK();
    int rows = nb;
    const float* fin = fold_partials((const float*)workspace, rows, C, (float*)workspace + ((size_t)nb + 1) * 2 * C, st);
    hipLaunchKernelGGL(k_col_finalize<0>, dim3(cdiv(C, 4)), dim3(256), 0, st, fin, rows, C, (double)M, eps, momentum,
                       mean, invstd, running_mean, running_var, (float*)nullptr, (float*)nullptr, 0);
    SD_LAUNCH_CHECK();
    return 0;
}

int sd_bn_finalize_scratch_rows(int rows) { return fold_rows(rows); }

int sd_bn_finalize_stats(const float* partial, int rows, int64_t M, int C, float eps, float momentum, float* running_mean,
                         float* running_var, float* mean, float* invstd, float* scratch, sd_stream_t stream) {
    if (int e = check_mc("sd_bn_finalize_stats", M, C)) return e;
    SD_REQUIRE(partial && mean && invstd && rows > 0, SD_ERR_INVALID, "sd_bn_finalize_stats: bad arguments");
    hipStream_t st = (hipStream_t)stream;
    partial = fold_partials(partial, rows, C, scratch, st);
    SD_LAUNCH_CHECK();
    hipLaunchKernelGGL(k_col_finalize<0>, dim3(cdiv(C, 4)), dim3(256), 0, st, partial, rows, C, (double)M, eps, momentum,
                       mean, invstd, running_mean, running_var, (float*)nullptr, (float*)nullptr, 0);
    SD_LAUNCH_CHECK();
    return 0;
}

int sd_bn_apply(const float* x, float* y, int64_t M, int C, const float* mean, const float* invstd, const float* gamma, const float* beta,
                const float* residual, int relu, uint8_t* relu_mask_out, sd_stream_t stream) {
    if (int e = check_mc("sd_bn_apply", M, C)) return e;
    SD_REQUIRE(x && y && mean && invstd && gamma && beta, SD_ERR_INVALID, "sd_bn_apply: null pointer");
    const int64_t n4 = M * C / 4;
    hipLaunchKernelGGL(k_bn_apply<float>, dim3(ew_grid(n4)), dim3(256), 0, (hipStream_t)stream, x, y, n4, C, mean, invstd, gamma, beta, residual, relu,
                       relu_mask_out);
    SD_LAUNCH_CHECK();
    return 0;
}

int sd_bn_fold(const float* gamma, const float* beta, const float* running_mean, const float* running_var, float eps, int C, float* scale,
               float* shift, sd_stream_t stream) {
    SD_REQUIRE(gamma && beta && running_mean && running_var && scale && shift && C > 0, SD_ERR_INVALID, "sd_bn_fold: bad arguments");
    hipLaunchKernelGGL(k_bn_fold, dim3(cdiv(C, 256)), dim3(256), 0, (hipStream_t)stream, gamma, beta, running_mean, running_var, eps, C, scale, shift);
    SD_LAUNCH_CHECK();
    return 0;
}

int sd_bn_bwd(const float* dy, const float* x, const float* y, int relu, int64_t M, int C, const float* mean, const float* invstd,
              const float* gamma, const float* beta, float* dx, float* g_out, float* dgamma, float* dbeta, int accumulate, void* workspace,
              size_t workspace_bytes, sd_stream_t stream) {
    if (int e = check_mc("sd_bn_bwd", M, C)) return e;
    SD_REQUIRE(relu >= 0 && relu <= 3, SD_ERR_INVALID, "sd_bn_bwd: relu must be 0 (none), 1 (mask from y), 2 (mask recomputed from x) or 3 (mask bytes)");
    SD_REQUIRE(dy && x && mean && invstd && gamma && dx && dgamma && dbeta && workspace && ((relu != 1 && relu != 3) || y) && (relu != 2 || beta),
               SD_ERR_INVALID, "sd_bn_bwd: null pointer");
    SD_REQUIRE(workspace_bytes >= sd_col_reduce_workspace_bytes(M, C), SD_ERR_WORKSPACE, "sd_bn_bwd: workspace too small");
    const int rpb = red_rows(M), nb = cdiv(M, rpb);
    hipStream_t st = (hipStream_t)stream;
    float* partial = (float*)workspace;
    float* mg = partial + (size_t)nb * 2 * C;
    float* mgx = mg + C;
    hipLaunchKernelGGL(k_col_reduce<1>, dim3(nb), dim3(256), 0, st, dy, x, y, mean, invstd, gamma, beta, relu, M, C, partial, rpb);
    SD_LAUNCH_CHECK();
    int rows = nb;
    const float* fin = fold_partials(partial, rows, C, mgx + C, st);
    hipLaunchKernelGGL(k_col_finalize<1>, dim3(cdiv(C, 4)), dim3(256), 0, st, fin, rows, C, (double)M, 0.f, 0.f, dgamma, dbeta,
                       (float*)nullptr, (float*)nullptr, mg, mgx, accumulate);
    SD_LAUNCH_CHECK();
    const int64_t n4 = M * C / 4;
    hipLaunchKernelGGL(k_bn_bwd_apply<float>, dim3(ew_grid(n4)), dim3(256), 0, st, dy, x, y, relu, n4, C, mean, invstd, gamma, beta,
                       (const float*)mg, (const float*)mgx, dx, g_out);
    SD_LAUNCH_CHECK();
    return 0;
}

int sd_bn_bwd_finalize(const float* partial, int rows, int64_t M, int C, float* dgamma, float* dbeta, int accumulate, float* means_out,
                       float* scratch, sd_stream_t stream) {
    if (int e = check_mc("sd_bn_bwd_finalize", M, C)) return e;
    SD_REQUIRE(partial && dgamma && dbeta && means_out && rows > 0, SD_ERR_INVALID, "sd_bn_bwd_finalize: bad arguments");
    hipStream_t st = (hipStream_t)stream;
    const float* fin = fold_partials(partial, rows, C, scratch, st);
    SD_LAUNCH_CHECK();
    hipLaunchKernelGGL(k_col_finalize<1>, dim3(cdiv(C, 4)), dim3(256), 0, st, fin, rows, C, (double)M, 0.f, 0.f, dgamma, dbeta,
                       (float*)nullptr, (float*)nullptr, means_out, means_out + C, accumulate);
    SD_LAUNCH_CHECK();
    return 0;
}

int sd_bn_bwd_apply(const float* dy, const float* x, const float* y, int relu, int64_t M, int C, const float* mean, const float* invstd,
                    const float* gamma, const float* beta, const float* means, float* dx, float* g_out, sd_stream_t stream) {
    if (int e = check_mc("sd_bn_bwd_apply", M, C)) return e;
    SD_REQUIRE(relu >= 0 && relu <= 3, SD_ERR_INVALID, "sd_bn_bwd_apply: relu must be 0 (none), 1 (mask from y), 2 (mask recomputed from x) or 3 (mask bytes)");
    SD_REQUIRE(dy && x && mean && invstd && gamma && means && dx && ((relu != 1 && relu != 3) || y) && (relu != 2 || beta), SD_ERR_INVALID,
               "sd_bn_bwd_apply: null pointer");
    const int64_t n4 = M * C / 4;
    hipLaunchKernelGGL(k_bn_bwd_apply<float>, dim3(ew_grid(n4)), dim3(256), 0, (hipStream_t)stream, dy, x, y, relu, n4, C, mean, invstd, gamma, beta,
                       means, means + C, dx, g_out);
    SD_LAUNCH_CHECK();
    return 0;
}

int sd_col_sum(const float* x, int64_t M, int C, float* out, int accumulate, void* workspace, size_t workspace_bytes, sd_stream_t stream) {
    if (int e = check_mc("sd_col_sum", M, C)) return e;
    SD_REQUIRE(x && out && workspace, SD_ERR_INVALID, "sd_col_sum: null pointer");
    SD_REQUIRE(workspace_bytes >= sd_col_reduce_workspace_bytes(M, C), SD_ERR_WORKSPACE, "sd_col_sum: workspace too small");
    const int rpb = red_rows(M), nb = cdiv(M, rpb);
    hipStream_t st = (hipStream_t)stream;
    hipLaunchKernelGGL(k_col_reduce<2>, dim3(nb), dim3(256), 0, st, x, (const float*)nullptr, (const float*)nullptr, (const float*)nullptr,
                       (const float*)nullptr, (const float*)nullptr, (const float*)nullptr, 0, M, C, (float*)workspace, rpb);
    SD_LAUNCH_CHECK();
    int rows = nb;
    const float* fin = fold_partials((const float*)workspace, rows, C, (float*)workspace + ((size_t)nb + 1) * 2 * C, st);
    hipLaunchKernelGGL(k_col_finalize<2>, dim3(cdiv(C, 4)), dim3(256), 0, st, fin, rows, C, (double)M, 0.f, 0.f, out,
                       (float*)nullptr, (float*)nullptr, (float*)nullptr, (float*)nullptr, (float*)nullptr, accumulate);
    SD_LAUNCH_CHECK();
    return 0;
}

int sd_maxpool3x3s2_fwd(const float* x, float* y, uint8_t* idx, int B, int Hi, int Wi, int C, sd_stream_t stream) {
    SD_REQUIRE(x && y && idx && B > 0 && Hi > 0 && Wi > 0 && C > 0 && C % 4 == 0, SD_ERR_INVALID, "sd_maxpool3x3s2_fwd: bad arguments");
    const int Ho = (Hi + 2 - 3) / 2 + 1, Wo = (Wi + 2 - 3) / 2 + 1;
    const int64_t n4 = (int64_t)B * Ho * Wo * C / 4;
    hipLaunchKernelGGL(k_maxpool_fwd, dim3(cdiv(n4, 256)), dim3(256), 0, (hipStream_t)stream, x, y, idx, B, Hi, Wi, Ho, Wo, C);
    SD_LAUNCH_CHECK();
    return 0;
}

int sd_maxpool3x3s2_bwd(const float* dy, const uint8_t* idx, float* dx, int B, int Hi, int Wi, int C, sd_stream_t stream) {
    SD_REQUIRE(dy && dx && idx && B > 0 && Hi > 0 && Wi > 0 && C > 0 && C % 4 == 0, SD_ERR_INVALID, "sd_maxpool3x3s2_bwd: bad arguments");
    const int Ho = (Hi + 2 - 3) / 2 + 1, Wo = (Wi + 2 - 3) / 2 + 1;
    const int64_t n4 = (int64_t)B * Hi * Wi * C / 4;
    hipLaunchKernelGGL(k_maxpool_bwd, dim3(cdiv(n4, 256)), dim3(256), 0, (hipStream_t)stream, dy, idx, dx, B, Hi, Wi, Ho, Wo, C);
    SD_LAUNCH_CHECK();
    return 0;
}

int sd_bn_relu_maxpool_fwd(const float* x, int B, int Hi, int Wi, int C, const float* mean, const float* invstd, const float* gamma,
                           const float* beta, float* y_pool, uint8_t* idx, sd_stream_t stream) {
    SD_REQUIRE(x && mean && invstd && gamma && beta && y_pool && idx && B > 0 && Hi > 0 && Wi > 0 && C > 0 && C % 4 == 0, SD_ERR_INVALID,
               "sd_bn_relu_maxpool_fwd: bad arguments");
    const int Ho = (Hi + 2 - 3) / 2 + 1, Wo = (Wi + 2 - 3) / 2 + 1;
    const int64_t n4 = (int64_t)B * Ho * Wo * C / 4;
    if (g_pool_pair && Wo % 2 == 0 && aligned16(x) && aligned16(y_pool) && (reinterpret_cast<uintptr_t>(idx) & 3u) == 0)
        hipLaunchKernelGGL((k_bn_relu_maxpool_fwd_pair<float, float, 4>), dim3(cdiv(n4 / 2, 256)), dim3(256), 0, (hipStream_t)stream, x, mean, invstd, gamma, beta,
                           y_pool, idx, B, Hi, Wi, Ho, Wo, C);
    else
    hipLaunchKernelGGL((k_bn_relu_maxpool_fwd<float, float>), dim3(cdiv(n4, 256)), dim3(256), 0, (hipStream_t)stream, x, mean, invstd, gamma, beta, y_pool, idx,
                       B, Hi, Wi, Ho, Wo, C);
    SD_LAUNCH_CHECK();
    return 0;
}

int sd_bn_relu_maxpool_fwd_bf16(const void* x_bf16, int B, int Hi, int Wi, int C, const float* mean, const float* invstd, const float* gamma,
                                const float* beta, void* y_pool_bf16, uint8_t* idx, sd_stream_t stream) {
    SD_REQUIRE(x_bf16 && mean && invstd && gamma && beta && y_pool_bf16 && idx && B > 0 && Hi > 0 && Wi > 0 && C > 0 && C % 4 == 0, SD_ERR_INVALID,
               "sd_bn_relu_maxpool_fwd_bf16: bad arguments");
    const int Ho = (Hi + 2 - 3) / 2 + 1, Wo = (Wi + 2 - 3) / 2 + 1;
    const int64_t n4 = (int64_t)B * Ho * Wo * C / 4;
    if (g_pool_pair && Wo % 2 == 0 && C % 8 == 0 && aligned16(x_bf16) && aligned16(y_pool_bf16) && (reinterpret_cast<uintptr_t>(idx) & 7u) == 0)
        hipLaunchKernelGGL((k_bn_relu_maxpool_fwd_pair<uint16_t, uint16_t, 8>), dim3(cdiv(n4 / 4, 256)), dim3(256), 0, (hipStream_t)stream, (const uint16_t*)x_bf16,
                           mean, invstd, gamma, beta, (uint16_t*)y_pool_bf16, idx, B, Hi, Wi, Ho, Wo, C);
    else
    hipLaunchKernelGGL((k_bn_relu_maxpool_fwd<uint16_t, uint16_t>), dim3(cdiv(n4, 256)), dim3(256), 0, (hipStream_t)stream, (const uint16_t*)x_bf16, mean,
                       invstd, gamma, beta, (uint16_t*)y_pool_bf16, idx, B, Hi, Wi, Ho, Wo, C);
    SD_LAUNCH_CHECK();
    return 0;
}

extern "C++" {
template <typename XT, typename PT, typename DT = float>
static int maxpool_bn_relu_bwd_any(const char* what, const PT* dpool, const uint8_t* idx, const XT* x, int B, int Hi, int Wi, int C, const float* mean,
                                   const float* invstd, const float* gamma, const float* beta, DT* dx, float* dgamma, float* dbeta, int accumulate,
                                   void* workspace, size_t workspace_bytes, sd_stream_t stream) {
    const int64_t M = (int64_t)B * Hi * Wi;
    if (int e = check_mc(what, M, C)) return e;
    SD_REQUIRE(dpool && idx && x && mean && invstd && gamma && beta && dx && dgamma && dbeta && workspace, SD_ERR_INVALID, "%s: null pointer", what);
    SD_REQUIRE(workspace_bytes >= sd_col_reduce_workspace_bytes(M, C), SD_ERR_WORKSPACE, "%s: workspace too small", what);
    const int Ho = (Hi + 2 - 3) / 2 + 1, Wo = (Wi + 2 - 3) / 2 + 1;
    const int nb = cdiv(M, RED_ROWS_PER_BLOCK);
    hipStream_t st = (hipStream_t)stream;
    float* partial = (float*)workspace;
    float* mg = partial + (size_t)nb * 2 * C;
    float* mgx = mg + C;
    const bool quad = Hi % 2 == 0 && Wi % 2 == 0;
    constexpr bool F32 = std::is_same<XT, float>::value && std::is_same<PT, float>::value && std::is_same<DT, float>::value;
    SD_REQUIRE(quad || F32, SD_ERR_INVALID, "%s: the bf16 form needs even Hi, Wi", what);
    if (quad) hipLaunchKernelGGL((k_pool_bn_bwd_reduce_quad<XT, PT>), dim3(nb), dim3(256), 0, st, dpool, idx, x, mean, invstd, gamma, beta, Hi, Wi, Ho, Wo, M / 4, C, partial);
    else if constexpr (F32) hipLaunchKernelGGL(k_pool_bn_bwd_reduce, dim3(nb), dim3(256), 0, st, dpool, idx, x, mean, invstd, gamma, beta, Hi, Wi, Ho, Wo, M, C, partial);
    SD_LAUNCH_CHECK();
// ... 30 lines not shown
                                     const float* invstd, const float* gamma, const float* beta, void* dx_bf16, float* dgamma, float* dbeta, int accumulate,
                                     void* workspace, size_t workspace_bytes, sd_stream_t stream) {
    return maxpool_bn_relu_bwd_any<uint16_t, uint16_t, uint16_t>("sd_maxpool_bn_relu_bwd_bf16_dx16", (const uint16_t*)dpool_bf16, idx, (const uint16_t*)x_bf16,
                                                                 B, Hi, Wi, C, mean, invstd, gamma, beta, (uint16_t*)dx_bf16, dgamma, dbeta, accumulate,
                                                                 workspace, workspace_bytes, stream);
}

int sd_upsample2x_bwd(const float* dy, const float* add, float* dx, int B, int H, int W, int C, sd_stream_t stream) {
    SD_REQUIRE(dy && dx && B > 0 && H > 0 && W > 0 && C > 0 && C % 4 == 0, SD_ERR_INVALID, "sd_upsample2x_bwd: bad arguments");
    const int64_t n4 = (int64_t)B * H * W * C / 4;
    hipLaunchKernelGGL(k_up2_bwd<float>, dim3(cdiv(n4, 256)), dim3(256), 0, (hipStream_t)stream, dy, add, dx, B, H, W, C);
    SD_LAUNCH_CHECK();
    return 0;
}

int sd_cast_f32_to_bf16(const float* x, void* y, int64_t n, sd_stream_t stream) {
    SD_REQUIRE(x && y && n > 0 && n % 4 == 0 && aligned16(x), SD_ERR_INVALID, "sd_cast_f32_to_bf16: bad arguments (n %% 4 == 0, 16-byte aligned source)");
    hipLaunchKernelGGL(k_cast_bf16, dim3(ew_grid(n / 4)), dim3(256), 0, (hipStream_t)stream, x, (uint16_t*)y, n / 4);
    SD_LAUNCH_CHECK();
    return 0;
}

int sd_cast_bf16_to_f32(const void* x, float* y, int64_t n, sd_stream_t stream) {
    SD_REQUIRE(x && y && n > 0 && n % 4 == 0 && aligned16(y) && (reinterpret_cast<uintptr_t>(x) & 7u) == 0, SD_ERR_INVALID,
               "sd_cast_bf16_to_f32: bad arguments (n %% 4 == 0, 8-byte aligned source, 16-byte aligned destination)");
    hipLaunchKernelGGL(k_cast_f32, dim3(ew_grid(n / 4)), dim3(256), 0, (hipStream_t)stream, (const uint16_t*)x, y, n / 4);
    SD_LAUNCH_CHECK();
    return 0;
}

int sd_bn_apply_bf16(const void* x, void* y, int64_t M, int C, const float* mean, const float* invstd, const float* gamma, const float* beta,
                     const void* residual, int relu, uint8_t* relu_mask_out, sd_stream_t stream) {
    if (int e = check_mc("sd_bn_apply_bf16", M, C)) return e;
    SD_REQUIRE(x && y && mean && invstd && gamma && beta, SD_ERR_INVALID, "sd_bn_apply_bf16: null pointer");
    const int64_t n4 = M * C / 4;
    if (C % 8 == 0 && aligned16(x) && aligned16(y) && aligned16(residual)) {
        hipLaunchKernelGGL(k_bn_apply_bf16x8, dim3(ew_grid(n4 / 2)), dim3(256), 0, (hipStream_t)stream, (const uint16_t*)x, (uint16_t*)y, n4 / 2, C, mean,
                           invstd, gamma, beta, (const uint16_t*)residual, relu, relu_mask_out);
        SD_LAUNCH_CHECK();
        return 0;
    }
    hipLaunchKernelGGL(k_bn_apply<uint16_t>, dim3(ew_grid(n4)), dim3(256), 0, (hipStream_t)stream, (const uint16_t*)x, (uint16_t*)y, n4, C, mean,
                       invstd, gamma, beta, (const uint16_t*)residual, relu, relu_mask_out);
    SD_LAUNCH_CHECK();
    return 0;
}

int sd_bn_bwd_bf16(const void* dy, const void* x, const void* y, int relu, int64_t M, int C, const float* mean, const float* invstd,
                   const float* gamma, const float* beta, void* dx, void* g_out, float* dgamma, float* dbeta, int accumulate, void* workspace,
                   size_t workspace_bytes, sd_stream_t stream) {
    if (int e = check_mc("sd_bn_bwd_bf16", M, C)) return e;
    SD_REQUIRE(relu >= 0 && relu <= 3, SD_ERR_INVALID, "sd_bn_bwd_bf16: relu must be 0 (none), 1 (mask from y), 2 (mask recomputed from x) or 3 (mask bytes)");
    SD_REQUIRE(dy && x && mean && invstd && gamma && dx && dgamma && dbeta && workspace && ((relu != 1 && relu != 3) || y) && (relu != 2 || beta),
               SD_ERR_INVALID, "sd_bn_bwd_bf16: null pointer");
    SD_REQUIRE(workspace_bytes >= sd_col_reduce_workspace_bytes(M, C), SD_ERR_WORKSPACE, "sd_bn_bwd_bf16: workspace too small");
    const int rpb = red_rows(M), nb = cdiv(M, rpb);
    hipStream_t st = (hipStream_t)stream;
    float* partial = (float*)workspace;
    float* mg = partial + (size_t)nb * 2 * C;
    float* mgx = mg + C;
    const bool wide = C % 8 == 0 && relu != 1 && aligned16(dy) && aligned16(x) && aligned16(dx) && aligned16(g_out);
    if (wide) hipLaunchKernelGGL(k_col_reduce_bwd_bf16x8, dim3(nb), dim3(256), 0, st, (const uint16_t*)dy, (const uint16_t*)x, (const uint8_t*)y, mean,
                                 invstd, gamma, beta, relu, M, C, partial, rpb);
    else hipLaunchKernelGGL((k_col_reduce<1, uint16_t>), dim3(nb), dim3(256), 0, st, (const uint16_t*)dy, (const uint16_t*)x, (const uint16_t*)y, mean,
                            invstd, gamma, beta, relu, M, C, partial, rpb);
    SD_LAUNCH_CHECK();
    int rows = nb;
    const float* fin = fold_partials(partial, rows, C, mgx + C, st);
    hipLaunchKernelGGL(k_col_finalize<1>, dim3(cdiv(C, 4)), dim3(256), 0, st, fin, rows, C, (double)M, 0.f, 0.f, dgamma, dbeta,
                       (float*)nullptr, (float*)nullptr, mg, mgx, accumulate);
    SD_LAUNCH_CHECK();
    const int64_t n4 = M * C / 4;
    if (wide) hipLaunchKernelGGL(k_bn_bwd_apply_bf16x8, dim3(ew_grid(n4 / 2)), dim3(256), 0, st, (const uint16_t*)dy, (const uint16_t*)x, (const uint8_t*)y,
                                 relu, n4 / 2, C, mean, invstd, gamma, beta, (const float*)mg, (const float*)mgx, (uint16_t*)dx, (uint16_t*)g_out);
    else hipLaunchKernelGGL(k_bn_bwd_apply<uint16_t>, dim3(ew_grid(n4)), dim3(256), 0, st, (const uint16_t*)dy, (const uint16_t*)x, (const uint16_t*)y,
                       relu, n4, C, mean, invstd, gamma, beta, (const float*)mg, (const float*)mgx, (uint16_t*)dx, (uint16_t*)g_out);
    SD_LAUNCH_CHECK();
    return 0;
}

int sd_col_sum_bf16(const void* x, int64_t M, int C, float* out, int accumulate, void* workspace, size_t workspace_bytes, sd_stream_t stream) {
    if (int e = check_mc("sd_col_sum_bf16", M, C)) return e;
    SD_REQUIRE(x && out && workspace, SD_ERR_INVALID, "sd_col_sum_bf16: null pointer");
    SD_REQUIRE(workspace_bytes >= sd_col_reduce_workspace_bytes(M, C), SD_ERR_WORKSPACE, "sd_col_sum_bf16: workspace too small");
    const int rpb = red_rows(M), nb = cdiv(M, rpb);
    hipStream_t st = (hipStream_t)stream;
    hipLaunchKernelGGL((k_col_reduce<2, uint16_t>), dim3(nb), dim3(256), 0, st, (const uint16_t*)x, (const uint16_t*)nullptr, (const uint16_t*)nullptr,
                       (const float*)nullptr, (const float*)nullptr, (const float*)nullptr, (const float*)nullptr, 0, M, C, (float*)workspace, rpb);
    SD_LAUNCH_CHECK();
    int rows = nb;
    const float* fin = fold_partials((const float*)workspace, rows, C, (float*)workspace + ((size_t)nb + 1) * 2 * C, st);
    hipLaunchKernelGGL(k_col_finalize<2>, dim3(cdiv(C, 4)), dim3(256), 0, st, fin, rows, C, (double)M, 0.f, 0.f, out,
                       (float*)nullptr, (float*)nullptr, (float*)nullptr, (float*)nullptr, (float*)nullptr, accumulate);
    SD_LAUNCH_CHECK();
    return 0;
}

int sd_upsample2x_bwd_bf16(const void* dy, const void* add, void* dx, int B, int H, int W, int C, sd_stream_t stream) {
    SD_REQUIRE(dy && dx && B > 0 && H > 0 && W > 0 && C > 0 && C % 4 == 0, SD_ERR_INVALID, "sd_upsample2x_bwd_bf16: bad arguments");
    const int64_t n4 = (int64_t)B * H * W * C / 4;
    hipLaunchKernelGGL(k_up2_bwd<uint16_t>, dim3(cdiv(n4, 256)), dim3(256), 0, (hipStream_t)stream, (const uint16_t*)dy, (const uint16_t*)add,
                       (uint16_t*)dx, B, H, W, C);
    SD_LAUNCH_CHECK();
    return 0;
}

int sd_maxpool3x3s2_fwd_bf16(const void* x, void* y, int B, int Hi, int Wi, int C, sd_stream_t stream) {
    SD_REQUIRE(x && y && B > 0 && Hi > 0 && Wi > 0 && C > 0 && C % 8 == 0, SD_ERR_INVALID, "sd_maxpool3x3s2_fwd_bf16: bad arguments");
    const int Ho = (Hi + 2 - 3) / 2 + 1, Wo = (Wi + 2 - 3) / 2 + 1;
    const int64_t n8 = (int64_t)B * Ho * Wo * C / 8;
    hipLaunchKernelGGL(k_maxpool_fwd_bf16, dim3(cdiv(n8, 256)), dim3(256), 0, (hipStream_t)stream, (const uint16_t*)x, (uint16_t*)y, B, Hi, Wi, Ho, Wo, C);
    SD_LAUNCH_CHECK();
    return 0;
}

int sd_head_fwd_bf16(const void* x, const float* w, const float* bias, float* y, int B, int HW, int C, int Co, sd_stream_t stream) {
    SD_REQUIRE(x && w && bias && y && B > 0 && HW > 0, SD_ERR_INVALID, "sd_head_fwd_bf16: bad arguments");
    if (Co > HEAD_NARROW_MAX_CO) return head_wide_fwd_bf16(x, w, bias, y, B, HW, C, Co, (hipStream_t)stream);
    SD_REQUIRE(C % 8 == 0 && C <= 512 && Co > 0 && Co <= HEAD_NARROW_MAX_CO, SD_ERR_INVALID, "sd_head_fwd_bf16: needs C %% 8 == 0, C <= 512, Co <= %d", HEAD_NARROW_MAX_CO);
    const int64_t M = (int64_t)B * HW;
    if (C == 128 && HW % 4 == 0 && aligned16(x) && aligned16(y)) {
        const int ntiles = (int)cdiv(M, 64), blocks = std::max(1, std::min(cdiv(ntiles, 4), 1024));
        if (Co <= 16) hipLaunchKernelGGL(k_head_fwd_bf16_c128<false>, dim3(blocks), dim3(256), 0, (hipStream_t)stream, (const uint16_t*)x, w, bias, y, M, HW, Co, ntiles);
        else hipLaunchKernelGGL(k_head_fwd_bf16_c128<true>, dim3(blocks), dim3(256), 0, (hipStream_t)stream, (const uint16_t*)x, w, bias, y, M, HW, Co, ntiles);
        SD_LAUNCH_CHECK();
        return 0;
    }
    const size_t lds = ((size_t)64 * (C + 4) + (size_t)Co * C) * sizeof(float);
    hipLaunchKernelGGL(k_head_fwd_bf16, dim3(cdiv(M, 64)), dim3(256), lds, (hipStream_t)stream, (const uint16_t*)x, w, bias, y, M, HW, C, Co);
    SD_LAUNCH_CHECK();
    return 0;
}

int sd_head_fwd(const float* x, const float* w, const float* bias, float* y, int B, int HW, int C, int Co, sd_stream_t stream) {
    SD_REQUIRE(x && w && bias && y && B > 0 && HW > 0, SD_ERR_INVALID, "sd_head_fwd: bad arguments");
    if (Co > HEAD_NARROW_MAX_CO) return head_wide_fwd(x, w, bias, y, B, HW, C, Co, (hipStream_t)stream);
    SD_REQUIRE(C % 4 == 0 && C <= 512 && Co > 0 && Co <= HEAD_NARROW_MAX_CO, SD_ERR_INVALID, "sd_head_fwd: needs C %% 4 == 0, C <= 512, Co <= %d", HEAD_NARROW_MAX_CO);
    const int64_t M = (int64_t)B * HW;
    if (C == 128 && Co <= 16 && HW % 16 == 0 && M < (1ll << 31) && aligned16(x) && aligned16(w) && aligned16(y)) {
        const int ntiles = (int)(M / 16);
        const size_t lds_b = (size_t)4 * HF_NST * 2048 * sizeof(float);
        static const hipError_t attr_once = hipFuncSetAttribute(reinterpret_cast<const void*>(&k_head_fwd_f32_c128), hipFuncAttributeMaxDynamicSharedMemorySize, (int)lds_b);
        SD_HIP(attr_once);
        hipLaunchKernelGGL(k_head_fwd_f32_c128, dim3(std::min(cdiv(ntiles, 4), 256)), dim3(256), lds_b, (hipStream_t)stream, x, w, bias, y, HW, Co, ntiles);
        SD_LAUNCH_CHECK();
        return 0;
    }
    const size_t lds = ((size_t)64 * (C + 4) + (size_t)Co * C) * sizeof(float);
    hipLaunchKernelGGL(k_head_fwd, dim3(cdiv(M, 64)), dim3(256), lds, (hipStream_t)stream, x, w, bias, y, M, HW, C, Co);
    SD_LAUNCH_CHECK();
    return 0;
}

static int head_wgrad_wave_rows(int64_t M) { return (int)std::min<int64_t>(1024, (cdiv(M, 16) + 3) / 4 * 4); }
size_t sd_head_bwd_workspace_bytes(int B, int HW, int C, int Co) {
    const int64_t M = (int64_t)B * HW;
    if (Co > HEAD_NARROW_MAX_CO) return head_wide_bwd_workspace_bytes(M, C, Co);
    return align_up((size_t)std::max<int64_t>(cdiv(M, HEAD_WG_PIX), head_wgrad_wave_rows(M)) * (Co * C + Co) * sizeof(float), 256);
}

int sd_head_bwd(const float* dy, const float* x, const float* w, float* dx, float* dw, float* dbias, int B, int HW, int C, int Co,
                int accumulate, void* workspace, size_t workspace_bytes, sd_stream_t stream) {
    SD_REQUIRE(dy && x && w && dx && dw && dbias && workspace && B > 0 && HW > 0, SD_ERR_INVALID, "sd_head_bwd: bad arguments");
    if (Co > HEAD_NARROW_MAX_CO) {
        const int64_t P = (int64_t)B * HW;
        if (int e = head_wide_check("sd_head_bwd", P, C, Co)) return e;
        SD_REQUIRE(workspace_bytes >= sd_head_bwd_workspace_bytes(B, HW, C, Co), SD_ERR_WORKSPACE, "sd_head_bwd: workspace too small");
        hipStream_t st = (hipStream_t)stream;
        int rows = 0;
        if (int e = head_wide_wgrad(dy, x, (float*)workspace, B, HW, C, Co, st, rows)) return e;
        const int n = Co * C + Co;
        hipLaunchKernelGGL(k_head_wgrad_fin, dim3(cdiv(n, 8)), dim3(256), 0, st, (const float*)workspace, rows, n, dw, dbias, Co * C, accumulate);
        SD_LAUNCH_CHECK();
        return head_wide_dgrad(dy, w, dx, B, HW, C, Co, st);
    }
    SD_REQUIRE(C % 4 == 0 && C <= 256 && (256 % C == 0) && (64 % (256 / C) == 0) && ((64 / (256 / C)) % 8 == 0) && Co > 0 && Co <= HEAD_NARROW_MAX_CO,
               SD_ERR_INVALID, "sd_head_bwd: needs C in {64, 128, 256} and Co <= %d", HEAD_NARROW_MAX_CO);
    SD_REQUIRE(workspace_bytes >= sd_head_bwd_workspace_bytes(B, HW, C, Co), SD_ERR_WORKSPACE, "sd_head_bwd: workspace too small");
    const int64_t M = (int64_t)B * HW;
    hipStream_t st = (hipStream_t)stream;
    int nb = cdiv(M, HEAD_WG_PIX);
    if (C == 128 && Co <= 16 && HW % 16 == 0 && M < (1ll << 31) && aligned16(x) && aligned16(dy)) {
        nb = head_wgrad_wave_rows(M);
        const int blocks = nb / 4;
        const size_t lds_b = (size_t)4 * HF_NST * HWG_STAGE * sizeof(float);
        static const hipError_t attr_once = hipFuncSetAttribute(reinterpret_cast<const void*>(&k_head_wgrad_f32_c128), hipFuncAttributeMaxDynamicSharedMemorySize, (int)lds_b);
        SD_HIP(attr_once);
        hipLaunchKernelGGL(k_head_wgrad_f32_c128, dim3(blocks), dim3(256), lds_b, st, dy, x, (float*)workspace, HW, Co, (int)(M / 16));
    } else {
        hipLaunchKernelGGL(k_head_wgrad, dim3(nb), dim3(256), 0, st, dy, x, (float*)workspace, M, HW, C, Co);
    }
    SD_LAUNCH_CHECK();
    const int n = Co * C + Co;
    hipLaunchKernelGGL(k_head_wgrad_fin, dim3(cdiv(n, 8)), dim3(256), 0, st, (const float*)workspace, nb, n, dw, dbias, Co * C, accumulate);
    SD_LAUNCH_CHECK();
    hipLaunchKernelGGL(k_head_dgrad<float>, dim3(cdiv(M, 64)), dim3(256), (size_t)Co * C * sizeof(float), st, dy, w, dx, M, HW, C, Co);
    SD_LAUNCH_CHECK();
    return 0;
}

int sd_head_bwd_bf16(const float* dy, const void* x_bf16, const float* w, void* dx_bf16, float* dw, float* dbias, int B, int HW, int C, int Co,
                     int accumulate, void* workspace, size_t workspace_bytes, sd_stream_t stream) {
    SD_REQUIRE(dy && x_bf16 && w && dx_bf16 && dw && dbias && workspace && B > 0 && HW > 0, SD_ERR_INVALID, "sd_head_bwd_bf16: bad arguments");
    SD_REQUIRE((C == 64 || C == 128) && Co > 0 && Co <= 8, SD_ERR_INVALID, "sd_head_bwd_bf16: needs C in {64, 128} and Co <= 8 (got %d, %d)", C, Co);
    SD_REQUIRE(aligned16(x_bf16) && aligned16(dx_bf16), SD_ERR_ALIGN, "sd_head_bwd_bf16: x and dx must be 16-byte aligned");
    SD_REQUIRE(workspace_bytes >= sd_head_bwd_workspace_bytes(B, HW, C, Co), SD_ERR_WORKSPACE, "sd_head_bwd_bf16: workspace too small");
    const int64_t M = (int64_t)B * HW;
    hipStream_t st = (hipStream_t)stream;
    hipLaunchKernelGGL(k_head_dgrad<uint16_t>, dim3(cdiv(M, 64)), dim3(256), (size_t)Co * C * sizeof(float), st, dy, w, (uint16_t*)dx_bf16, M, HW, C, Co);
    SD_LAUNCH_CHECK();
    const int nb = cdiv(M, HEAD_WG_PIX);
    hipLaunchKernelGGL(k_head_wgrad_bf16<8>, dim3(nb), dim3(256), 0, st, dy, (const uint16_t*)x_bf16, (float*)workspace, M, HW, C, Co);
    SD_LAUNCH_CHECK();
    const int n = Co * C + Co;
    hipLaunchKernelGGL(k_head_wgrad_fin, dim3(cdiv(n, 8)), dim3(256), 0, st, (const float*)workspace, nb, n, dw, dbias, Co * C, accumulate);
    SD_LAUNCH_CHECK();
    return 0;
}

int sd_adam_step(float* param, const float* grad, float* exp_avg, float* exp_avg_sq, int64_t n, int step, float lr, float beta1, float beta2,
                 float eps, float grad_scale, sd_stream_t stream) {
    SD_REQUIRE(param && grad && exp_avg && exp_avg_sq && n > 0 && n % 4 == 0 && step >= 1, SD_ERR_INVALID, "sd_adam_step: bad arguments (n %% 4 == 0, step >= 1)");
    SD_REQUIRE(aligned16(param) && aligned16(grad) && aligned16(exp_avg) && aligned16(exp_avg_sq), SD_ERR_ALIGN, "sd_adam_step: pointers must be 16-byte aligned");
    const double bc1 = 1.0 - pow((double)beta1, step), bc2 = 1.0 - pow((double)beta2, step);
    hipLaunchKernelGGL(k_adam, dim3(ew_grid(n / 4)), dim3(256), 0, (hipStream_t)stream, param, grad, exp_avg, exp_avg_sq, n / 4, lr, beta1, beta2, eps,
                       (float)bc1, (float)sqrt(bc2), grad_scale);
    SD_LAUNCH_CHECK();
    return 0;
}

}
```

structuredetector_amd/model/network.py:

```python
from __future__ import annotations

import ctypes as C
import math
import warnings

import torch
import torch.nn as nn

from .. import _lib as L
from ..utils import trace as T

BN_EPS = 1e-5
BN_MOMENTUM = 0.1


class ConvParams(nn.Module):
    def __init__(self, cin, cout, k, stride=1, pad=0, bias=False):
        super().__init__()
        self.cin, self.cout, self.k, self.stride, self.pad = cin, cout, k, stride, pad
        w = torch.empty((cout, cin, k, k), memory_format=torch.channels_last)
        self.weight = nn.Parameter(w)
        self.bias = nn.Parameter(torch.zeros(cout)) if bias else None


class BNParams(nn.Module):
    def __init__(self, c):
        super().__init__()
        self.c = c
        self.weight = nn.Parameter(torch.ones(c))
        self.bias = nn.Parameter(torch.zeros(c))
        self.register_buffer("running_mean", torch.zeros(c))
        self.register_buffer("running_var", torch.ones(c))
        self.register_buffer("num_batches_tracked", torch.tensor(0, dtype=torch.long))


class Slot(nn.Module):
    """Parameter-less position (ReLU / MaxPool / Upsample) kept so Sequential indices match the reference."""


class BasicBlock(nn.Module):
    def __init__(self, cin, cout, stride):
        super().__init__()
        self.conv1 = ConvParams(cin, cout, 3, stride, 1)
        self.bn1 = BNParams(cout)
        self.relu = Slot()
        self.conv2 = ConvParams(cout, cout, 3, 1, 1)
        self.bn2 = BNParams(cout)
        self.downsample = None
        if stride != 1 or cin != cout:
            self.downsample = nn.Sequential(ConvParams(cin, cout, 1, stride, 0), BNParams(cout))


class Fpn(nn.Module):

    def __init__(self, in_channels, out_channels):
        super().__init__()
        self.up = Slot()
        self.lateral = ConvParams(in_channels, out_channels, 1, bias=True)
        self.conv = nn.Sequential(ConvParams(out_channels, out_channels, 3, 1, 1), BNParams(out_channels), Slot())


class Head(nn.Module):

    def __init__(self, in_channels, out_channels):
        super().__init__()
        self.conv = ConvParams(in_channels, out_channels, 1, bias=True)


BACKBONE_FILE_GLOB = "resnet34-*.pth"


def find_backbone_weights(args=None):
    import os
    from pathlib import Path
    for given in (getattr(args, "backbone_weights", None), os.environ.get("SDNET_BACKBONE_WEIGHTS")):
        if given:
            path = Path(given).expanduser()
            if not path.is_file():
                raise L.SdError(f"backbone weights file not found: {path}")
            return path
    homes = []
    if os.environ.get("TORCH_HOME"):
        homes.append(Path(os.environ["TORCH_HOME"]))
    homes.append(Path(os.environ.get("XDG_CACHE_HOME", "~/.cache")).expanduser() / "torch")
    for home in homes:
        hits = sorted((home / "hub" / "checkpoints").glob(BACKBONE_FILE_GLOB))
        if hits:
            return hits[0]
    return None


def _layer(cin, cout, n, stride):
    return nn.Sequential(*[BasicBlock(cin if i == 0 else cout, cout, stride if i == 0 else 1) for i in range(n)])


def _desc(B, Hi, Wi, conv: ConvParams):
    d = L.ConvDesc()
    d.B, d.Hi, d.Wi, d.Cin, d.Cout, d.R, d.S, d.stride, d.pad = B, Hi, Wi, conv.cin, conv.cout, conv.k, conv.k, conv.stride, conv.pad
    d.Ho = (Hi + 2 * conv.pad - conv.k) // conv.stride + 1
    d.Wo = (Wi + 2 * conv.pad - conv.k) // conv.stride + 1
    return d


def _ptr(t):
    return 0 if t is None else t.data_ptr()


class _Engine:

    def __init__(self, net: "Network"):
        self.net = net
        self.lib = L.lib()
        self.prof = None
        self.prof_shapes = None
        self._nbt = []
        self.overlap_wgrad = False
        self._side = None
        self.fuse_bn_bwd = False
        self._wt_plan, self._wt_flat, self._wt_valid = None, {}, None
        self._head_ok = {}
        self.stem_ring = True
        self.fuse_head = True
        self.small_batch_kernel = True

    def _kname(self, d, which):
        if self.prof is None:
            return ""
        if self.prof_shapes is not None:
            self.prof_shapes.append((d.B, d.Hi, d.Wi, d.Cin, d.Cout, d.R, d.stride, d.Ho, d.Wo))
        return self.lib.sd_conv2d_kernel_name(C.byref(d), which).decode()

    def _timed(self, kind, flops, fn, phase="fwd"):
        if self.prof is None:
            return fn()
        e0, e1 = torch.cuda.Event(enable_timing=True), torch.cuda.Event(enable_timing=True)
        e0.record()
        fn()
        e1.record()
        self.prof.append((kind, flops, e0, e1, phase))

    def _ws(self, nbytes, dev):
        return L.workspace(max(int(nbytes), 256), dev)

    def _to_bf16(self, t):
        out = torch.empty(t.shape, dtype=torch.bfloat16, device=t.device)
        L.check(self.lib.sd_cast_f32_to_bf16(t.data_ptr(), out.data_ptr(), t.numel(), L.stream()), "sd_cast_f32_to_bf16")
        return out

    def _to_f32(self, t):
        out = torch.empty(t.shape, dtype=torch.float32, device=t.device)
        L.check(self.lib.sd_cast_bf16_to_f32(t.data_ptr(), out.data_ptr(), t.numel(), L.stream()), "sd_cast_bf16_to_f32")
        return out

    def refresh_bf16_weights(self):
        net = self.net
        if net.flat_params_bf16 is None:
            net.flat_params_bf16 = torch.empty(net.flat_params.numel(), dtype=torch.bfloat16, device=net.flat_params.device)
        L.check(self.lib.sd_cast_f32_to_bf16(net.flat_params.data_ptr(), net.flat_params_bf16.data_ptr(), net.flat_params.numel(), L.stream()),
                "sd_cast_f32_to_bf16")

    def _w16(self, conv):
        off, n = self.net._flat_off[id(conv.weight)]
        return self.net.flat_params_bf16[off:off + n]

    def _conv_sb(self, x, w, y, d, scale, shift, res, res_up2, relu, bf16):
        nws = self.lib.sd_conv2d_fwd_sb_workspace_bytes(C.byref(d), bf16)
        ws = self._ws(nws, x.device) if nws else None
        st = L.zero_state(self.lib.sd_conv2d_fwd_sb_state_bytes(C.byref(d), bf16), x.device) if nws else None
        L.check(self.lib.sd_conv2d_fwd_sb(x.data_ptr(), w.data_ptr(), y.data_ptr(), C.byref(d), _ptr(scale), _ptr(shift), _ptr(res), int(res_up2),
                                          int(relu), bf16, _ptr(ws), ws.numel() if nws else 0, _ptr(st), st.numel() if nws else 0, L.stream()),
                "sd_conv2d_fwd_sb")

    def conv(self, x, conv, B, Hi, Wi, scale=None, shift=None, res=None, res_up2=False, relu=False, amp=False, sb=False):
        d = _desc(B, Hi, Wi, conv)
        if amp:
            y = torch.empty((B, d.Ho, d.Wo, conv.cout), dtype=torch.bfloat16, device=x.device)
            flops = 2.0 * B * d.Ho * d.Wo * conv.cout * conv.cin * conv.k * conv.k
            self._timed("bf16:" + self._kname(d, 16), flops, lambda: L.check(
                self.lib.sd_conv2d_fwd_bf16(x.data_ptr(), self._w16(conv).data_ptr(), y.data_ptr(), C.byref(d), _ptr(scale), _ptr(shift),
                                            _ptr(res), int(res_up2), int(relu), 0, 0, L.stream()), "sd_conv2d_fwd_bf16"))
            return y, d
        y = torch.empty((B, d.Ho, d.Wo, conv.cout), dtype=torch.float32, device=x.device)
        flops = 2.0 * B * d.Ho * d.Wo * conv.cout * conv.cin * conv.k * conv.k
        if sb and self.small_batch_kernel and self.lib.sd_conv2d_fwd_sb_supported(C.byref(d), 0):
            self._timed("k_conv_fwd_sb<false>" if self.prof is not None else "", flops,
                        lambda: self._conv_sb(x, conv.weight, y, d, scale, shift, res, res_up2, relu, 0))
            return y, d
        nws = self.lib.sd_conv2d_fwd_workspace_bytes(C.byref(d))
        ws = self._ws(nws, x.device) if nws else None
        self._timed(self._kname(d, 0), flops, lambda: L.check(
            self.lib.sd_conv2d_fwd(x.data_ptr(), conv.weight.data_ptr(), y.data_ptr(), C.byref(d), _ptr(scale), _ptr(shift),
                                   _ptr(res), int(res_up2), int(relu), _ptr(ws), ws.numel() if nws else 0, L.stream()),
            "sd_conv2d_fwd"))
        return y, d

    def conv_stats(self, x, conv, B, Hi, Wi, bn: BNParams, update_running=True, amp=False):
        d = _desc(B, Hi, Wi, conv)
        y = torch.empty((B, d.Ho, d.Wo, conv.cout), dtype=torch.bfloat16 if amp else torch.float32, device=x.device)
        mean = torch.empty(conv.cout, dtype=torch.float32, device=x.device)
        invstd = torch.empty_like(mean)
        flops = 2.0 * B * d.Ho * d.Wo * conv.cout * conv.cin * conv.k * conv.k
        if amp:
            ws = self._ws(self.lib.sd_conv2d_fwd_bf16_bn_stats_workspace_bytes(C.byref(d)), x.device)
            self._timed("bf16:" + self._kname(d, 16), flops, lambda: L.check(
                self.lib.sd_conv2d_fwd_bf16_bn_stats(x.data_ptr(), self._w16(conv).data_ptr(), y.data_ptr(), C.byref(d), BN_EPS, BN_MOMENTUM,
                                                     bn.running_mean.data_ptr() if update_running else 0,
                                                     bn.running_var.data_ptr() if update_running else 0,
                                                     mean.data_ptr(), invstd.data_ptr(), ws.data_ptr(), ws.numel(), L.stream()),
                "sd_conv2d_fwd_bf16_bn_stats"))
            return y, d, (mean, invstd)
        ws = self._ws(self.lib.sd_conv2d_fwd_bn_stats_workspace_bytes(C.byref(d)), x.device)
        self._timed(self._kname(d, 0), flops, lambda: L.check(
            self.lib.sd_conv2d_fwd_bn_stats(x.data_ptr(), conv.weight.data_ptr(), y.data_ptr(), C.byref(d), BN_EPS, BN_MOMENTUM,
                                            bn.running_mean.data_ptr() if update_running else 0,
                                            bn.running_var.data_ptr() if update_running else 0,
                                            mean.data_ptr(), invstd.data_ptr(), ws.data_ptr(), ws.numel(), L.stream()),
            "sd_conv2d_fwd_bn_stats"))
        return y, d, (mean, invstd)

    def bn_train(self, x, bn: BNParams, res=None, relu=True, update_running=True, stats=None, want_mask=False):
        Mrows, Cc = x.numel() // x.shape[-1], x.shape[-1]
        if stats is not None:
            mean, invstd = stats
        else:
            mean = torch.empty(Cc, dtype=torch.float32, device=x.device)
            invstd = torch.empty_like(mean)
            ws = self._ws(self.lib.sd_col_reduce_workspace_bytes(Mrows, Cc), x.device)
            L.check(self.lib.sd_bn_train_stats(x.data_ptr(), Mrows, Cc, BN_EPS, BN_MOMENTUM,
                                               bn.running_mean.data_ptr() if update_running else 0,
                                               bn.running_var.data_ptr() if update_running else 0,
                                               mean.data_ptr(), invstd.data_ptr(), ws.data_ptr(), ws.numel(), L.stream()), "sd_bn_train_stats")
        y = torch.empty_like(x)
        mask = torch.empty(x.numel() // 4, dtype=torch.uint8, device=x.device) if want_mask else None
        apply = self.lib.sd_bn_apply_bf16 if x.dtype == torch.bfloat16 else self.lib.sd_bn_apply
        L.check(apply(x.data_ptr(), y.data_ptr(), Mrows, Cc, mean.data_ptr(), invstd.data_ptr(), bn.weight.data_ptr(),
                      bn.bias.data_ptr(), _ptr(res), int(relu), _ptr(mask), L.stream()), "sd_bn_apply")
        if update_running:
            self._nbt.append(bn.num_batches_tracked)
        return (y, mean, invstd, mask) if want_mask else (y, mean, invstd)

    def bn_fold(self, bn: BNParams):
        cached = self.net._folded.get(id(bn))
        if cached is not None:
            return cached
        scale = torch.empty(bn.c, dtype=torch.float32, device=bn.weight.device)
        shift = torch.empty_like(scale)
        L.check(self.lib.sd_bn_fold(bn.weight.data_ptr(), bn.bias.data_ptr(), bn.running_mean.data_ptr(), bn.running_var.data_ptr(),
                                    BN_EPS, bn.c, scale.data_ptr(), shift.data_ptr(), L.stream()), "sd_bn_fold")
        self.net._folded[id(bn)] = (scale, shift)
        return scale, shift

    def forward(self, x, training, tape=None, amp=False):
        net, lib = self.net, self.lib
        if amp:
            if not training:
                raise L.SdError("amp=True is the mixed-precision TRAINING forward; inference uses forward_bf16")
            self.refresh_bf16_weights()
        if x.dim() != 4 or x.shape[1] != 3:
            raise L.SdError(f"Network expects (B, 3, H, W) input, got {tuple(x.shape)}")
        L.require_cuda(x)
        x = x.contiguous().float()
        B, _, H, W = x.shape
        if H % 32 or W % 32:
            raise L.SdError("input height/width must be multiples of 32 (args.py:181-186)")
        rec = tape is not None

        T.push("fwd:stem")
        stem, bn0 = net.adpater[0], net.adpater[1]
        d0 = _desc(B, H, W, stem)
        amp_stem = bool(amp and training and d0.Ho % 2 == 0 and d0.Wo % 2 == 0)
        s0 = torch.empty((B, d0.Ho, d0.Wo, 64), dtype=torch.bfloat16 if amp_stem else torch.float32, device=x.device)
        wss = self._ws(lib.sd_conv2d_stem_fwd_workspace_bytes(C.byref(d0)), x.device)
        Hp, Wp = (d0.Ho + 2 - 3) // 2 + 1, (d0.Wo + 2 - 3) // 2 + 1
        p1 = torch.empty((B, Hp, Wp, 64), dtype=torch.bfloat16 if amp_stem else torch.float32, device=x.device)
        pidx = torch.empty((B, Hp, Wp, 64), dtype=torch.uint8, device=x.device)
        if training:
            m0 = torch.empty(64, dtype=torch.float32, device=x.device)
            i0 = torch.empty_like(m0)
            ws = self._ws(lib.sd_conv2d_stem_fwd_bn_stats_workspace_bytes(C.byref(d0)), x.device)
            stem_fwd = (lib.sd_conv2d_stem_fwd_bn_stats_bf16 if amp_stem else lib.sd_conv2d_stem_fwd_bn_stats_bf16mm) if amp \
                else lib.sd_conv2d_stem_fwd_bn_stats
            L.check(stem_fwd(x.data_ptr(), stem.weight.data_ptr(), s0.data_ptr(), C.byref(d0), BN_EPS, BN_MOMENTUM,
                             bn0.running_mean.data_ptr(), bn0.running_var.data_ptr(), m0.data_ptr(), i0.data_ptr(),
                             ws.data_ptr(), ws.numel(), L.stream()), "sd_conv2d_stem_fwd_bn_stats")
            self._nbt.append(bn0.num_batches_tracked)
            pool_fwd = lib.sd_bn_relu_maxpool_fwd_bf16 if amp_stem else lib.sd_bn_relu_maxpool_fwd
            L.check(pool_fwd(s0.data_ptr(), B, d0.Ho, d0.Wo, 64, m0.data_ptr(), i0.data_ptr(), bn0.weight.data_ptr(),
                             bn0.bias.data_ptr(), p1.data_ptr(), pidx.data_ptr(), L.stream()), "sd_bn_relu_maxpool_fwd")
        else:
            sc, sh = self.bn_fold(bn0)
            L.check(lib.sd_conv2d_stem_fwd(x.data_ptr(), stem.weight.data_ptr(), s0.data_ptr(), C.byref(d0), sc.data_ptr(), sh.data_ptr(), 1, 0,
                                           wss.data_ptr(), wss.numel(), L.stream()), "stem")
            m0 = i0 = None
            L.check(lib.sd_maxpool3x3s2_fwd(s0.data_ptr(), p1.data_ptr(), pidx.data_ptr(), B, d0.Ho, d0.Wo, 64, L.stream()), "maxpool")
        if rec:
            tape["x"], tape["stem"], tape["amp"] = x, (d0, s0, m0, i0, pidx), bool(amp)
        if amp and not amp_stem:
            p1 = self._to_bf16(p1)

        T.pop()
        feats, cur, Hc, Wc = [], p1, Hp, Wp
        blocks_tape = []
        for li, layer in enumerate((net.down1, net.down2, net.down3, net.down4), start=1):
            T.push(f"fwd:down{li}")
            for blk in layer:
                if training:
                    c1, d1, st1 = self.conv_stats(cur, blk.conv1, B, Hc, Wc, blk.bn1, amp=amp)
                    a1, m1, i1 = self.bn_train(c1, blk.bn1, stats=st1)
                    c2, d2, st2 = self.conv_stats(a1, blk.conv2, B, d1.Ho, d1.Wo, blk.bn2, amp=amp)
                    if blk.downsample is not None:
                        cd, dd, std_ = self.conv_stats(cur, blk.downsample[0], B, Hc, Wc, blk.downsample[1], amp=amp)
                        idt, md, idd = self.bn_train(cd, blk.downsample[1], relu=False, stats=std_)
                    else:
                        cd = dd = md = idd = None
                        idt = cur
                    out, m2, i2, msk = self.bn_train(c2, blk.bn2, res=idt, relu=True, stats=st2, want_mask=True)
                    if rec:
                        blocks_tape.append((blk, cur, (Hc, Wc), d1, c1, a1, m1, i1, d2, c2, m2, i2, out, dd, cd, md, idd, msk))
                else:
                    s1, h1 = self.bn_fold(blk.bn1)
                    a1, d1 = self.conv(cur, blk.conv1, B, Hc, Wc, scale=s1, shift=h1, relu=True, sb=True)
                    if blk.downsample is not None:
                        sd_, hd = self.bn_fold(blk.downsample[1])
                        idt, _ = self.conv(cur, blk.downsample[0], B, Hc, Wc, scale=sd_, shift=hd, sb=True)
                    else:
                        idt = cur
                    s2, h2 = self.bn_fold(blk.bn2)
                    out, _ = self.conv(a1, blk.conv2, B, d1.Ho, d1.Wo, scale=s2, shift=h2, res=idt, relu=True, sb=True)
                cur, Hc, Wc = out, d1.Ho, d1.Wo
            feats.append((cur, Hc, Wc))
            T.pop()
        (p2, H2, W2), (p3, H3, W3), (p4, H4, W4), (p5, H5, W5) = feats

        T.push("fwd:fpn")
        f, _ = self.conv(p5, net.up1, B, H5, W5, shift=net.up1.bias, amp=amp, sb=not training)
        fpn_tape = []
        for fpn, (sc_t, Hs, Ws) in ((net.up2, (p4, H4, W4)), (net.up3, (p3, H3, W3)), (net.up4, (p2, H2, W2))):
            t, dl = self.conv(sc_t, fpn.lateral, B, Hs, Ws, shift=fpn.lateral.bias, res=f, res_up2=True, amp=amp, sb=not training)
            if training:
                c, dc, stf = self.conv_stats(t, fpn.conv[0], B, Hs, Ws, fpn.conv[1], amp=amp)
                fn, mf, if_ = self.bn_train(c, fpn.conv[1], stats=stf)
                if rec:
                    fpn_tape.append((fpn, sc_t, (Hs, Ws), dl, t, dc, c, mf, if_, fn))
            else:
                sf, hf = self.bn_fold(fpn.conv[1])
                fn, _ = self.conv(t, fpn.conv[0], B, Hs, Ws, scale=sf, shift=hf, relu=True, sb=True)
            f = fn
        T.pop()

        T.push("fwd:head")
        hc = net.head.conv
        out = torch.empty((B, hc.cout, H2, W2), dtype=torch.float32, device=x.device)
        head_fwd = lib.sd_head_fwd_bf16 if amp else lib.sd_head_fwd
        L.check(head_fwd(f.data_ptr(), hc.weight.data_ptr(), hc.bias.data_ptr(), out.data_ptr(), B, H2 * W2, hc.cin, hc.cout,
                         L.stream()), "sd_head_fwd")
        T.pop()
        if rec:
            tape.update(blocks=blocks_tape, fpn=fpn_tape, p5=(p5, H5, W5), f1=f, B=B, hw=(H2, W2))
        if self._nbt:
            torch._foreach_add_(self._nbt, 1)
            self._nbt = []
        return out

    def _w_bf16(self, conv):
        key = ("w", id(conv))
        w = self.net._folded.get(key)
        if w is None:
            n = conv.weight.numel()
            w = torch.empty(n, dtype=torch.bfloat16, device=conv.weight.device)
            L.check(self.lib.sd_cast_f32_to_bf16(conv.weight.data_ptr(), w.data_ptr(), n, L.stream()), "sd_cast_f32_to_bf16")
            self.net._folded[key] = w
        return w

    def _head_fusable(self, B, Hs, Ws, conv, hc):
        key = (B, Hs, Ws, hc.cout)
        ok = self._head_ok.get(key)
        if ok is None:
            ok = hc.cin == 128 and bool(self.lib.sd_conv2d_fwd_bf16_head_supported(C.byref(_desc(B, Hs, Ws, conv)), hc.cout))
            self._head_ok[key] = ok
        return ok

    def _head_prepared(self, hc):
        key = ("head", id(hc))
        buf = self.net._folded.get(key)
        if buf is None:
            buf = torch.empty(self.lib.sd_head_split_bf16_bytes(), dtype=torch.uint8, device=hc.weight.device)
            L.check(self.lib.sd_head_split_bf16(hc.weight.data_ptr(), hc.bias.data_ptr(), hc.cout, buf.data_ptr(), L.stream()), "sd_head_split_bf16")
            self.net._folded[key] = buf
        return buf

    def conv_bf16(self, x, conv, B, Hi, Wi, scale=None, shift=None, res=None, res_up2=False, relu=False):
        d = _desc(B, Hi, Wi, conv)
        y = torch.empty((B, d.Ho, d.Wo, conv.cout), dtype=torch.bfloat16, device=x.device)
        if self.small_batch_kernel and self.lib.sd_conv2d_fwd_sb_supported(C.byref(d), 1):
            self._conv_sb(x, self._w_bf16(conv), y, d, scale, shift, res, res_up2, relu, 1)
            return y, d
        nws = self.lib.sd_conv2d_fwd_bf16_workspace_bytes(C.byref(d))
        ws = self._ws(nws, x.device) if nws else None
        L.check(self.lib.sd_conv2d_fwd_bf16(x.data_ptr(), self._w_bf16(conv).data_ptr(), y.data_ptr(), C.byref(d), _ptr(scale), _ptr(shift),
                                            _ptr(res), int(res_up2), int(relu), _ptr(ws), ws.numel() if nws else 0, L.stream()),
                "sd_conv2d_fwd_bf16")
        return y, d

    def forward_bf16(self, x):
        net, lib = self.net, self.lib
        L.require_cuda(x)
        x = x.contiguous().float()
        B, _, H, W = x.shape
        if x.dim() != 4 or x.shape[1] != 3 or H % 32 or W % 32:
            raise L.SdError("Network expects (B, 3, H, W) input with H, W multiples of 32")
        stem, bn0 = net.adpater[0], net.adpater[1]
        d0 = _desc(B, H, W, stem)
        sc, sh = self.bn_fold(bn0)
        Hc, Wc = (d0.Ho + 2 - 3) // 2 + 1, (d0.Wo + 2 - 3) // 2 + 1
        cur = torch.empty((B, Hc, Wc, 64), dtype=torch.bfloat16, device=x.device)
        if stem.k == 7 and stem.stride == 2 and stem.pad == 3 and d0.Wo <= 4096:
            L.check(lib.sd_stem_bn_relu_maxpool_fwd_bf16(x.data_ptr(), stem.weight.data_ptr(), sc.data_ptr(), sh.data_ptr(), cur.data_ptr(),
                                                         C.byref(d0), L.stream()), "stem+maxpool")
        else:
            a0 = torch.empty((B, d0.Ho, d0.Wo, 64), dtype=torch.bfloat16, device=x.device)
            wss = self._ws(lib.sd_conv2d_stem_fwd_workspace_bytes(C.byref(d0)), x.device)
            L.check(lib.sd_conv2d_stem_fwd(x.data_ptr(), stem.weight.data_ptr(), a0.data_ptr(), C.byref(d0), sc.data_ptr(), sh.data_ptr(), 1, 1,
                                           wss.data_ptr(), wss.numel(), L.stream()), "stem")
            L.check(lib.sd_maxpool3x3s2_fwd_bf16(a0.data_ptr(), cur.data_ptr(), B, d0.Ho, d0.Wo, 64, L.stream()), "maxpool")
        feats = []
        for layer in (net.down1, net.down2, net.down3, net.down4):
            for blk in layer:
                s1, h1 = self.bn_fold(blk.bn1)
                a1, d1 = self.conv_bf16(cur, blk.conv1, B, Hc, Wc, scale=s1, shift=h1, relu=True)
                if blk.downsample is not None:
                    sd_, hd = self.bn_fold(blk.downsample[1])
                    idt, _ = self.conv_bf16(cur, blk.downsample[0], B, Hc, Wc, scale=sd_, shift=hd)
                else:
                    idt = cur
                s2, h2 = self.bn_fold(blk.bn2)
                cur, _ = self.conv_bf16(a1, blk.conv2, B, d1.Ho, d1.Wo, scale=s2, shift=h2, res=idt, relu=True)
                Hc, Wc = d1.Ho, d1.Wo
            feats.append((cur, Hc, Wc))
        (p2, H2, W2), (p3, H3, W3), (p4, H4, W4), (p5, H5, W5) = feats
        f, _ = self.conv_bf16(p5, net.up1, B, H5, W5, shift=net.up1.bias)
        hc = net.head.conv
        out = torch.empty((B, hc.cout, H2, W2), dtype=torch.float32, device=x.device)
        for fpn, (sc_t, Hs, Ws) in ((net.up2, (p4, H4, W4)), (net.up3, (p3, H3, W3)), (net.up4, (p2, H2, W2))):
            t, _ = self.conv_bf16(sc_t, fpn.lateral, B, Hs, Ws, shift=fpn.lateral.bias, res=f, res_up2=True)
            sf, hf = self.bn_fold(fpn.conv[1])
            if fpn is net.up4 and self.fuse_head and self._head_fusable(B, Hs, Ws, fpn.conv[0], hc):
                dl = _desc(B, Hs, Ws, fpn.conv[0])
                rc = lib.sd_conv2d_fwd_bf16_head(t.data_ptr(), self._w_bf16(fpn.conv[0]).data_ptr(), C.byref(dl), sf.data_ptr(), hf.data_ptr(), 1,
                                                 self._head_prepared(hc).data_ptr(), hc.cout, out.data_ptr(), L.stream())
                if rc == 0:
                    return out
                if rc > 0:
                    L.check(rc, "sd_conv2d_fwd_bf16_head")
                self._head_ok.pop((B, Hs, Ws, hc.cout), None)
            f, _ = self.conv_bf16(t, fpn.conv[0], B, Hs, Ws, scale=sf, shift=hf, relu=True)
        L.check(lib.sd_head_fwd_bf16(f.data_ptr(), hc.weight.data_ptr(), hc.bias.data_ptr(), out.data_ptr(), B, H2 * W2, hc.cin, hc.cout,
                                     L.stream()), "sd_head_fwd_bf16")
        return out

    def _transpose_all(self, amp):
        net = self.net
        if self._wt_plan is None:
            convs = [m for m in net.modules() if isinstance(m, ConvParams) and m.cin % 64 == 0 and m.cout % 64 == 0]
            rows, views, dst, blk = [], {}, 0, 0
            for m in convs:
                taps, n = m.k * m.k, m.weight.numel()
                nbx, nby = (m.cin + 31) // 32, (m.cout + 31) // 32
                rows.append([net._flat_off[id(m.weight)][0], dst, m.cout, taps, m.cin, blk, nbx, nby])
                views[id(m)] = (dst, n)
                dst += n; blk += nbx * nby * taps
            table = torch.tensor(rows, dtype=torch.int32, device=net.flat_params.device).contiguous()
            self._wt_plan = (table, len(convs), blk, views, dst)
        table, nconv, blocks, _, total = self._wt_plan
        key = "bf16" if amp else "f32"
        if key not in self._wt_flat:
            self._wt_flat[key] = torch.empty(total, dtype=torch.bfloat16 if amp else torch.float32, device=net.flat_params.device)
        L.check(self.lib.sd_conv2d_transpose_weights_batched(net.flat_params.data_ptr(), self._wt_flat[key].data_ptr(), table.data_ptr(), nconv, blocks,
                                                             int(amp), L.stream()), "sd_conv2d_transpose_weights_batched")
        self._wt_valid = key

    def _wt(self, conv, amp=False):
        if self._wt_valid == ("bf16" if amp else "f32") and id(conv) in self._wt_plan[3]:
            off, n = self._wt_plan[3][id(conv)]
            return self._wt_flat[self._wt_valid][off:off + n]
        wt = torch.empty(conv.cin * conv.k * conv.k * conv.cout, dtype=torch.bfloat16 if amp else torch.float32, device=conv.weight.device)
        transpose = self.lib.sd_conv2d_transpose_weights_bf16 if amp else self.lib.sd_conv2d_transpose_weights
        L.check(transpose(conv.weight.data_ptr(), wt.data_ptr(), conv.cout, conv.k * conv.k, conv.cin, L.stream()), "transpose_weights")
        return wt

    def _dgrad(self, dy, conv, d, res=None, bn_next=None, res_half=False):
        amp = dy.dtype == torch.bfloat16
        dx = torch.empty((d.B, d.Hi, d.Wi, conv.cin), dtype=dy.dtype, device=dy.device)
        wt = self._wt(conv, amp)
        flops = 2.0 * d.B * d.Ho * d.Wo * conv.cout * conv.cin * conv.k * conv.k
        if amp:
            assert bn_next is None, "fuse_bn_bwd is an fp32-path experiment"
            mode = 2 if res_half else (1 if res is not None else 0)
            self._timed("bf16:" + self._kname(d, 17), flops, lambda: L.check(
                self.lib.sd_conv2d_dgrad_bf16(dy.data_ptr(), wt.data_ptr(), dx.data_ptr(), C.byref(d), _ptr(res), mode, L.stream()),
                "sd_conv2d_dgrad_bf16"), phase="dgrad")
            return dx
        if bn_next is None:
            if res_half:
                fn = lambda: L.check(self.lib.sd_conv2d_dgrad_half_res(dy.data_ptr(), wt.data_ptr(), dx.data_ptr(), C.byref(d), res.data_ptr(),
                                                                       L.stream()), "sd_conv2d_dgrad_half_res")
            else:
                fn = lambda: L.check(self.lib.sd_conv2d_dgrad(dy.data_ptr(), wt.data_ptr(), dx.data_ptr(), C.byref(d), _ptr(res), L.stream()),
                                     "sd_conv2d_dgrad")
            self._timed(self._kname(d, 1), flops, fn, phase="dgrad")
            return dx
        assert not res_half
        x, y, relu, bn, mean, invstd = bn_next
        means = torch.empty(2 * conv.cin, dtype=torch.float32, device=dy.device)
        ws = self._ws(self.lib.sd_conv2d_dgrad_bn_reduce_workspace_bytes(C.byref(d)), dy.device)
        self._timed(self._kname(d, 1), flops, lambda: L.check(
            self.lib.sd_conv2d_dgrad_bn_reduce(dy.data_ptr(), wt.data_ptr(), dx.data_ptr(), C.byref(d), _ptr(res), x.data_ptr(),
                                               _ptr(y) if int(relu) in (1, 3) else 0, int(relu), mean.data_ptr(), invstd.data_ptr(),
                                               bn.weight.data_ptr(), bn.bias.data_ptr(), self.net.grad_of(bn.weight).data_ptr(),
                                               self.net.grad_of(bn.bias).data_ptr(), 0, means.data_ptr(), ws.data_ptr(), ws.numel(),
                                               L.stream()), "sd_conv2d_dgrad_bn_reduce"), phase="dgrad")
        return dx, means

    def _side_stream(self):
        if self._side is None:
            self._side = torch.cuda.Stream()
        return self._side

    def _wgrad(self, dy, x, conv, d):
        if not self.overlap_wgrad:
            return self._wgrad_now(dy, x, conv, d)
        main, side = torch.cuda.current_stream(), self._side_stream()
        ready = torch.cuda.Event()
        ready.record(main)
        with torch.cuda.stream(side):
            side.wait_event(ready)
            self._wgrad_now(dy, x, conv, d)
        dy.record_stream(side); x.record_stream(side)

    def _join_side(self):
        if self.overlap_wgrad and self._side is not None:
            torch.cuda.current_stream().wait_stream(self._side)

    def _wgrad_now(self, dy, x, conv, d):
        g = self.net.grad_of(conv.weight)
        flops = 2.0 * d.B * d.Ho * d.Wo * conv.cout * conv.cin * conv.k * conv.k
        if dy.dtype == torch.bfloat16:
            ws = self._ws(self.lib.sd_conv2d_wgrad_bf16_workspace_bytes(C.byref(d)), dy.device)
            self._timed("bf16:" + self._kname(d, 2), flops, lambda: L.check(
                self.lib.sd_conv2d_wgrad_bf16(dy.data_ptr(), x.data_ptr(), g.data_ptr(), C.byref(d), 0, ws.data_ptr(), ws.numel(), L.stream()),
                "sd_conv2d_wgrad_bf16"), phase="wgrad")
            return
        nbytes = self.lib.sd_conv2d_wgrad_workspace_bytes(C.byref(d))
        ws = self._ws(nbytes, dy.device)
        self._timed(self._kname(d, 2), flops, lambda: L.check(
            self.lib.sd_conv2d_wgrad(dy.data_ptr(), x.data_ptr(), g.data_ptr(), C.byref(d), 0, ws.data_ptr(), ws.numel(), L.stream()),
            "sd_conv2d_wgrad"), phase="wgrad")

    def _bias_grad(self, dy, conv):
        Mrows, Cc = dy.numel() // dy.shape[-1], dy.shape[-1]
        ws = self._ws(self.lib.sd_col_reduce_workspace_bytes(Mrows, Cc), dy.device)
        col_sum = self.lib.sd_col_sum_bf16 if dy.dtype == torch.bfloat16 else self.lib.sd_col_sum
        L.check(col_sum(dy.data_ptr(), Mrows, Cc, self.net.grad_of(conv.bias).data_ptr(), 0, ws.data_ptr(), ws.numel(), L.stream()),
                "sd_col_sum")

    def _bn_bwd(self, dy, x, y, relu, bn, mean, invstd, want_g=False, means=None):
        Mrows, Cc = x.numel() // x.shape[-1], x.shape[-1]
        dx = torch.empty_like(x)
        g = torch.empty_like(x) if want_g else None
        if means is not None:
            L.check(self.lib.sd_bn_bwd_apply(dy.data_ptr(), x.data_ptr(), _ptr(y) if int(relu) in (1, 3) else 0, int(relu), Mrows, Cc,
                                             mean.data_ptr(), invstd.data_ptr(), bn.weight.data_ptr(), bn.bias.data_ptr(), means.data_ptr(),
                                             dx.data_ptr(), _ptr(g), L.stream()), "sd_bn_bwd_apply")
            return dx, g
        ws = self._ws(self.lib.sd_col_reduce_workspace_bytes(Mrows, Cc), x.device)
        bn_bwd = self.lib.sd_bn_bwd_bf16 if x.dtype == torch.bfloat16 else self.lib.sd_bn_bwd
        L.check(bn_bwd(dy.data_ptr(), x.data_ptr(), _ptr(y) if int(relu) in (1, 3) else 0, int(relu), Mrows, Cc, mean.data_ptr(),
                                   invstd.data_ptr(), bn.weight.data_ptr(), bn.bias.data_ptr(), dx.data_ptr(), _ptr(g),
                                   self.net.grad_of(bn.weight).data_ptr(),
                                   self.net.grad_of(bn.bias).data_ptr(), 0, ws.data_ptr(), ws.numel(), L.stream()), "sd_bn_bwd")
        return dx, g

    def backward(self, tape, dhead, on_stage=None):
        net, lib = self.net, self.lib
        B = tape["B"]
        H2, W2 = tape["hw"]
        dhead = dhead.contiguous().float()
        hc = net.head.conv
        amp = bool(tape.get("amp"))
        if amp and self.fuse_bn_bwd:
            raise L.SdError("fuse_bn_bwd is an fp32-path experiment; switch it off for mixed-precision training")
        T.push("bwd:fpn_head")
        self._transpose_all(amp)
        ws = self._ws(lib.sd_head_bwd_workspace_bytes(B, H2 * W2, hc.cin, hc.cout), dhead.device)
        if amp and hc.cin in (64, 128) and hc.cout <= 8:
            f1 = tape["f1"]
            df = torch.empty_like(f1)
            L.check(lib.sd_head_bwd_bf16(dhead.data_ptr(), f1.data_ptr(), hc.weight.data_ptr(), df.data_ptr(), net.grad_of(hc.weight).data_ptr(),
                                         net.grad_of(hc.bias).data_ptr(), B, H2 * W2, hc.cin, hc.cout, 0, ws.data_ptr(), ws.numel(), L.stream()),
                    "sd_head_bwd_bf16")
        else:
            f1 = self._to_f32(tape["f1"]) if amp else tape["f1"]
            df = torch.empty_like(f1)
            L.check(lib.sd_head_bwd(dhead.data_ptr(), f1.data_ptr(), hc.weight.data_ptr(), df.data_ptr(), net.grad_of(hc.weight).data_ptr(),
                                    net.grad_of(hc.bias).data_ptr(), B, H2 * W2, hc.cin, hc.cout, 0, ws.data_ptr(), ws.numel(), L.stream()),
                    "sd_head_bwd")
            if amp:
                df = self._to_bf16(df)

        lateral_grad = {}
        for (fpn, sc_t, (Hs, Ws), dl, t, dc, c, mf, if_, fn) in reversed(tape["fpn"]):
            dcv, _ = self._bn_bwd(df, c, fn, 2, fpn.conv[1], mf, if_)
            dt = self._dgrad(dcv, fpn.conv[0], dc)
            self._wgrad(dcv, t, fpn.conv[0], dc)
            self._wgrad(dt, sc_t, fpn.lateral, dl)
            self._bias_grad(dt, fpn.lateral)
            lateral_grad[sc_t.data_ptr()] = (dt, fpn.lateral, dl)
            dfp = torch.empty((B, Hs // 2, Ws // 2, fpn.lateral.cout), dtype=dt.dtype, device=dt.device)
            up2_bwd = lib.sd_upsample2x_bwd_bf16 if amp else lib.sd_upsample2x_bwd
            L.check(up2_bwd(dt.data_ptr(), 0, dfp.data_ptr(), B, Hs // 2, Ws // 2, fpn.lateral.cout, L.stream()), "up2_bwd")
            df = dfp
        p5, H5, W5 = tape["p5"]
        d5 = _desc(B, H5, W5, net.up1)
        self._wgrad(df, p5, net.up1, d5)
        self._bias_grad(df, net.up1)
        blocks = tape["blocks"]

        def bn2_of(i):
            if i < 0 or not self.fuse_bn_bwd:
                return None
            b = blocks[i]
            return (b[9], b[17], 3, b[0].bn2, b[10], b[11])

        last = len(blocks) - 1
        has_lateral = blocks[last][12].data_ptr() in lateral_grad
        nxt = None if has_lateral else bn2_of(last)
        r = self._dgrad(df, net.up1, d5, bn_next=nxt)
        dcur, mcur = r if nxt is not None else (r, None)
        T.pop()
        if on_stage:
            self._join_side()
            on_stage("fpn_head")

        first_of = {id(net.down4[0]): "down4", id(net.down3[0]): "down3", id(net.down2[0]): "down2"}
        T.push("bwd:down4")
        for bi in range(last, -1, -1):
            (blk, xin, (Hc, Wc), d1, c1, a1, m1, i1, d2, c2, m2, i2, out, dd, cd, md, idd, msk) = blocks[bi]
            extra = lateral_grad.pop(out.data_ptr(), None)
            if extra is not None:
                nxt = bn2_of(bi)
                r = self._dgrad(extra[0], extra[1], extra[2], res=dcur, bn_next=nxt)
                dcur, mcur = r if nxt is not None else (r, None)
            dc2, g = self._bn_bwd(dcur, c2, msk, 3, blk.bn2, m2, i2, want_g=True, means=mcur)
            nxt = (c1, None, 2, blk.bn1, m1, i1) if self.fuse_bn_bwd else None
            r = self._dgrad(dc2, blk.conv2, d2, bn_next=nxt)
            da1, ma1 = r if nxt is not None else (r, None)
            self._wgrad(dc2, a1, blk.conv2, d2)
            dc1, _ = self._bn_bwd(da1, c1, a1, 2, blk.bn1, m1, i1, means=ma1)
            half = False
            if blk.downsample is not None:
                dcd, _ = self._bn_bwd(g, cd, None, False, blk.downsample[1], md, idd)
                ds = blk.downsample[0]
                half = ds.k == 1 and ds.stride == 2 and ds.pad == 0 and Hc % 2 == 0 and Wc % 2 == 0 and not self.fuse_bn_bwd
                if half:
                    dsm = L.ConvDesc()
                    dsm.B, dsm.Hi, dsm.Wi, dsm.Cin, dsm.Cout, dsm.R, dsm.S, dsm.stride, dsm.pad = B, dd.Ho, dd.Wo, ds.cin, ds.cout, 1, 1, 1, 0
                    dsm.Ho, dsm.Wo = dd.Ho, dd.Wo
                    skip = self._dgrad(dcd, ds, dsm)
                else:
                    skip = self._dgrad(dcd, ds, dd)
                self._wgrad(dcd, xin, ds, dd)
            else:
                skip = g
            prev_lateral = bi > 0 and blocks[bi - 1][12].data_ptr() in lateral_grad
            nxt = None if (bi == 0 or prev_lateral) else bn2_of(bi - 1)
            r = self._dgrad(dc1, blk.conv1, d1, res=skip, bn_next=nxt, res_half=half)
            dcur, mcur = r if nxt is not None else (r, None)
            self._wgrad(dc1, xin, blk.conv1, d1)
            if id(blk) in first_of:
                T.pop()
                if on_stage:
                    self._join_side()
                    on_stage(first_of[id(blk)])
                T.push("bwd:" + {"down4": "down3", "down3": "down2", "down2": "down1_stem"}[first_of[id(blk)]])

        d0, s0, m0, i0, pidx = tape["stem"]
        bn0 = net.adpater[1]
        amp_stem = s0.dtype == torch.bfloat16
        if amp and not amp_stem:
            dcur = self._to_f32(dcur)
        ring = amp_stem and self.stem_ring and d0.Wi % 4 == 0
        ds0 = torch.empty(s0.shape, dtype=torch.bfloat16 if ring else torch.float32, device=s0.device)
        ws = self._ws(lib.sd_col_reduce_workspace_bytes(B * d0.Ho * d0.Wo, 64), s0.device)
        pool_bwd = lib.sd_maxpool_bn_relu_bwd_bf16_dx16 if ring else (lib.sd_maxpool_bn_relu_bwd_bf16 if amp_stem else lib.sd_maxpool_bn_relu_bwd)
        L.check(pool_bwd(dcur.data_ptr(), pidx.data_ptr(), s0.data_ptr(), B, d0.Ho, d0.Wo, 64, m0.data_ptr(), i0.data_ptr(),
                         bn0.weight.data_ptr(), bn0.bias.data_ptr(), ds0.data_ptr(), net.grad_of(bn0.weight).data_ptr(),
                         net.grad_of(bn0.bias).data_ptr(), 0, ws.data_ptr(), ws.numel(), L.stream()), "sd_maxpool_bn_relu_bwd")
        stem = net.adpater[0]
        ws = self._ws(lib.sd_conv2d_stem_wgrad_workspace_bytes(C.byref(d0)), ds0.device)
        stem_wgrad = lib.sd_conv2d_stem_wgrad_bf16 if ring else (lib.sd_conv2d_stem_wgrad_bf16mm if amp else lib.sd_conv2d_stem_wgrad)
        L.check(stem_wgrad(ds0.data_ptr(), tape["x"].data_ptr(), net.grad_of(stem.weight).data_ptr(), C.byref(d0), 0,
                           ws.data_ptr(), ws.numel(), L.stream()), "sd_conv2d_stem_wgrad")
        self._join_side()
        self._wt_valid = None
        T.pop()
        if on_stage:
            on_stage("down1_stem")


class _NetFn(torch.autograd.Function):

    @staticmethod
    def forward(ctx, net, x, *params):
        tape = {}
        out = net._engine.forward(x, True, tape)
        ctx.net, ctx.tape = net, tape
        return out

    @staticmethod
    def backward(ctx, dhead):
        net = ctx.net
        net._engine.backward(ctx.tape, dhead)
        ctx.tape = None
        return (None, None) + tuple(net.grad_of(p) for p in net._flat_order)


class Network(nn.Module):
    def __init__(self, args, pretrained=True, raw_output: bool = False, init_weights: bool = True):
        super().__init__()
        self.raw_output = raw_output
        self.bf16_inference = bool(getattr(args, "use_amp", False) or getattr(args, "bf16_inference", False))
        self.label_count = len(args.labels)
        self.part_count = len(args.parts)
        self.out_channels = self.label_count + self.part_count + 4
        self.fpn_depth = args.fpn_depth
        if self.fpn_depth % 64:
            raise L.SdError("fpn_depth must be a multiple of 64 for the MFMA tiles")
        if self.out_channels > 256:
            raise L.SdError(f"labels + parts + 4 must be <= 256 (head kernel limit SD_HEAD_MAX_CO); got {self.out_channels}")
        if self.out_channels > 32 and self.fpn_depth not in (64, 128, 256):
            raise L.SdError(f"labels + parts + 4 > 32 needs fpn_depth in (64, 128, 256) (the wide head kernels); got {self.fpn_depth}")

        self.adpater = nn.Sequential(ConvParams(3, 64, 7, 2, 3), BNParams(64), Slot(), Slot())
        self.down1 = _layer(64, 64, 3, 1)
        self.down2 = _layer(64, 128, 4, 2)
        self.down3 = _layer(128, 256, 6, 2)
        self.down4 = _layer(256, 512, 3, 2)
        self.up1 = ConvParams(512, self.fpn_depth, 1, bias=True)
        self.up2 = Fpn(256, self.fpn_depth)
        self.up3 = Fpn(128, self.fpn_depth)
        self.up4 = Fpn(64, self.fpn_depth)
        self.head = Head(self.fpn_depth, self.out_channels)
        if init_weights:
# ... 167 lines not shown
```

Before: 879.3.

## Fold downsample BN into residual apply and last FPN BN into head kernels

Adds a bn_apply variant that normalizes the downsample branch inline as the residual, so the separate downsample BN apply and its output tensor are skipped. The last FPN BN+ReLU is no longer materialized. The head forward and wgrad kernels instead apply the affine+ReLU on the fly to the raw conv output, which saves one full-resolution write and read. The cost is extra ALU and parameter registers in the head kernels. The backward fpn tape now stores None for the normalized output, and the existing _bn_bwd has to cope with that.

```diff
diff --git a/include/sdnet_hip.h b/include/sdnet_hip.h
--- a/include/sdnet_hip.h
+++ b/include/sdnet_hip.h
@@ -256,6 +256,10 @@
 int sd_bn_apply(const float* x, float* y, int64_t M, int C, const float* mean, const float* invstd,
                 const float* gamma, const float* beta, const float* residual, int relu, uint8_t* relu_mask_out,
                 sd_stream_t stream);
+int sd_bn_apply_res_bn_supported(int64_t M, int C);
+int sd_bn_apply_res_bn(const float* x, float* y, int64_t M, int C, const float* mean, const float* invstd, const float* gamma,
+                       const float* beta, const float* residual, const float* res_mean, const float* res_invstd,
+                       const float* res_gamma, const float* res_beta, int relu, uint8_t* relu_mask_out, sd_stream_t stream);
 int sd_bn_fold(const float* gamma, const float* beta, const float* running_mean, const float* running_var,
                float eps, int C, float* scale, float* shift, sd_stream_t stream);
 int sd_bn_bwd(const float* dy, const float* x, const float* y, int relu, int64_t M, int C, const float* mean,
@@ -279,6 +283,13 @@
 size_t sd_head_bwd_workspace_bytes(int B, int HW, int C, int Co);
 int sd_head_bwd(const float* dy_nchw, const float* x_nhwc, const float* w, float* dx_nhwc, float* dw, float* dbias,
                 int B, int HW, int C, int Co, int accumulate, void* workspace, size_t workspace_bytes, sd_stream_t stream);
+int sd_head_fwd_bn_supported(int B, int HW, int C, int Co);
+int sd_head_bwd_bn_supported(int B, int HW, int C, int Co);
+int sd_head_fwd_bn(const float* x_nhwc, const float* w, const float* bias, float* y_nchw, int B, int HW, int C, int Co, const float* mean,
+                   const float* invstd, const float* gamma, const float* beta, int relu, sd_stream_t stream);
+int sd_head_bwd_bn(const float* dy_nchw, const float* x_nhwc, const float* w, float* dx_nhwc, float* dw, float* dbias, int B, int HW,
+                   int C, int Co, const float* mean, const float* invstd, const float* gamma, const float* beta, int relu, int accumulate,
+                   void* workspace, size_t workspace_bytes, sd_stream_t stream);
 int sd_head_bwd_bf16(const float* dy, const void* x_bf16, const float* w, void* dx_bf16, float* dw, float* dbias, int B, int HW, int C, int Co,
                      int accumulate, void* workspace, size_t workspace_bytes, sd_stream_t stream);
 
diff --git a/structuredetector_amd/_lib.py b/structuredetector_amd/_lib.py
--- a/structuredetector_amd/_lib.py
+++ b/structuredetector_amd/_lib.py
@@ -127,6 +127,8 @@
     "sd_col_reduce_workspace_bytes": (c_size, [c_i64, c_int]),
     "sd_bn_train_stats": (c_int, [c_vp, c_i64, c_int, c_float, c_float, c_vp, c_vp, c_vp, c_vp, c_vp, c_size, c_vp]),
     "sd_bn_apply": (c_int, [c_vp, c_vp, c_i64, c_int, c_vp, c_vp, c_vp, c_vp, c_vp, c_int, c_vp, c_vp]),
+    "sd_bn_apply_res_bn_supported": (c_int, [c_i64, c_int]),
+    "sd_bn_apply_res_bn": (c_int, [c_vp, c_vp, c_i64, c_int] + [c_vp] * 9 + [c_int, c_vp, c_vp]),
     "sd_bn_fold": (c_int, [c_vp, c_vp, c_vp, c_vp, c_float, c_int, c_vp, c_vp, c_vp]),
     "sd_bn_bwd": (c_int, [c_vp, c_vp, c_vp, c_int, c_i64, c_int, c_vp, c_vp, c_vp, c_vp, c_vp, c_vp, c_vp, c_vp, c_int, c_vp, c_size, c_vp]),
     "sd_col_sum": (c_int, [c_vp, c_i64, c_int, c_vp, c_int, c_vp, c_size, c_vp]),
@@ -137,6 +139,10 @@
     "sd_head_bwd_workspace_bytes": (c_size, [c_int] * 4),
     "sd_head_bwd": (c_int, [c_vp] * 6 + [c_int] * 5 + [c_vp, c_size, c_vp]),
     "sd_head_bwd_bf16": (c_int, [c_vp] * 6 + [c_int] * 5 + [c_vp, c_size, c_vp]),
+    "sd_head_fwd_bn_supported": (c_int, [c_int] * 4),
+    "sd_head_bwd_bn_supported": (c_int, [c_int] * 4),
+    "sd_head_fwd_bn": (c_int, [c_vp] * 4 + [c_int] * 4 + [c_vp] * 4 + [c_int, c_vp]),
+    "sd_head_bwd_bn": (c_int, [c_vp] * 6 + [c_int] * 4 + [c_vp] * 4 + [c_int, c_int, c_vp, c_size, c_vp]),
     "sd_adam_step": (c_int, [c_vp, c_vp, c_vp, c_vp, c_i64, c_int, c_float, c_float, c_float, c_float, c_float, c_vp]),
     "sd_conv2d_kernel_name": (C.c_char_p, [c_vp, c_int]),
     "sd_set_option": (c_int, [C.c_char_p, c_int]),
diff --git a/structuredetector_amd/csrc/sd_common.h b/structuredetector_amd/csrc/sd_common.h
--- a/structuredetector_amd/csrc/sd_common.h
+++ b/structuredetector_amd/csrc/sd_common.h
@@ -58,6 +58,11 @@
     return make_float4(bf16_to_f32((uint16_t)(r.x & 0xffff)), bf16_to_f32((uint16_t)(r.x >> 16)), bf16_to_f32((uint16_t)(r.y & 0xffff)),
                        bf16_to_f32((uint16_t)(r.y >> 16)));
 }
+__device__ __forceinline__ float bn_affine(float v, float mean, float invstd, float gamma, float beta) { return fmaf(gamma, (v - mean) * invstd, beta); }
+__device__ __forceinline__ float4 bn_affine4(const float4 v, const float4 mu, const float4 is, const float4 g, const float4 b) {
+    return make_float4(bn_affine(v.x, mu.x, is.x, g.x, b.x), bn_affine(v.y, mu.y, is.y, g.y, b.y), bn_affine(v.z, mu.z, is.z, g.z, b.z),
+                       bn_affine(v.w, mu.w, is.w, g.w, b.w));
+}
 __device__ __forceinline__ void st4(float* p, int64_t i, const float4 v) { reinterpret_cast<float4*>(p)[i] = v; }
 __device__ __forceinline__ void st4(uint16_t* p, int64_t i, const float4 v) {
     uint2 pk;
diff --git a/structuredetector_amd/csrc/sd_nn.hip b/structuredetector_amd/csrc/sd_nn.hip
--- a/structuredetector_amd/csrc/sd_nn.hip
+++ b/structuredetector_amd/csrc/sd_nn.hip
@@ -164,12 +164,45 @@
             g = reinterpret_cast<const float4*>(gamma)[col]; b = reinterpret_cast<const float4*>(beta)[col];
         }
         float4 o;
-        o.x = (v.x - mu.x) * is.x * g.x + b.x; o.y = (v.y - mu.y) * is.y * g.y + b.y;
-        o.z = (v.z - mu.z) * is.z * g.z + b.z; o.w = (v.w - mu.w) * is.w * g.w + b.w;
+        o.x = bn_affine(v.x, mu.x, is.x, g.x, b.x); o.y = bn_affine(v.y, mu.y, is.y, g.y, b.y);
+        o.z = bn_affine(v.z, mu.z, is.z, g.z, b.z); o.w = bn_affine(v.w, mu.w, is.w, g.w, b.w);
         if (res) {
             const float4 r = ld4(res, i);
             o.x += r.x; o.y += r.y; o.z += r.z; o.w += r.w;
         }
+        if (mask) mask[i] = (uint8_t)((o.x > 0.f ? 1 : 0) | (o.y > 0.f ? 2 : 0) | (o.z > 0.f ? 4 : 0) | (o.w > 0.f ? 8 : 0));
+        if (relu) { o.x = fmaxf(o.x, 0.f); o.y = fmaxf(o.y, 0.f); o.z = fmaxf(o.z, 0.f); o.w = fmaxf(o.w, 0.f); }
+        st4(y, i, o);
+    }
+}
+
+__global__ __launch_bounds__(256) void k_bn_apply_resbn(const float* __restrict__ x, float* __restrict__ y, int64_t n4, int C,
+                                                         const float* __restrict__ mean, const float* __restrict__ invstd,
+                                                         const float* __restrict__ gamma, const float* __restrict__ beta,
+                                                         const float* __restrict__ res, const float* __restrict__ rmean,
+                                                         const float* __restrict__ rinvstd, const float* __restrict__ rgamma,
+                                                         const float* __restrict__ rbeta, int relu, uint8_t* __restrict__ mask) {
+    const int64_t stride = (int64_t)gridDim.x * 256;
+    const int cols = C >> 2;
+    const bool fixed = stride % cols == 0;
+    const int col0 = (int)(((int64_t)blockIdx.x * 256 + threadIdx.x) % cols);
+    float4 mu = reinterpret_cast<const float4*>(mean)[col0], is = reinterpret_cast<const float4*>(invstd)[col0];
+    float4 g = reinterpret_cast<const float4*>(gamma)[col0], b = reinterpret_cast<const float4*>(beta)[col0];
+    float4 rmu = reinterpret_cast<const float4*>(rmean)[col0], ris = reinterpret_cast<const float4*>(rinvstd)[col0];
+    float4 rg = reinterpret_cast<const float4*>(rgamma)[col0], rb = reinterpret_cast<const float4*>(rbeta)[col0];
+    for (int64_t i = (int64_t)blockIdx.x * 256 + threadIdx.x; i < n4; i += stride) {
+        const float4 v = ld4(x, i);
+        const float4 rv = ld4(res, i);
+        if (!fixed) {
+            const int col = (int)(i % cols);
+            mu = reinterpret_cast<const float4*>(mean)[col]; is = reinterpret_cast<const float4*>(invstd)[col];
+            g = reinterpret_cast<const float4*>(gamma)[col]; b = reinterpret_cast<const float4*>(beta)[col];
+            rmu = reinterpret_cast<const float4*>(rmean)[col]; ris = reinterpret_cast<const float4*>(rinvstd)[col];
+            rg = reinterpret_cast<const float4*>(rgamma)[col]; rb = reinterpret_cast<const float4*>(rbeta)[col];
+        }
+        float4 o = bn_affine4(v, mu, is, g, b);
+        const float4 r = bn_affine4(rv, rmu, ris, rg, rb);
+        o.x += r.x; o.y += r.y; o.z += r.z; o.w += r.w;
         if (mask) mask[i] = (uint8_t)((o.x > 0.f ? 1 : 0) | (o.y > 0.f ? 2 : 0) | (o.z > 0.f ? 4 : 0) | (o.w > 0.f ? 8 : 0));
         if (relu) { o.x = fmaxf(o.x, 0.f); o.y = fmaxf(o.y, 0.f); o.z = fmaxf(o.z, 0.f); o.w = fmaxf(o.w, 0.f); }
         st4(y, i, o);
@@ -677,9 +710,25 @@
 }
 
 constexpr int HF_NST = 4;
-__global__ __launch_bounds__(256) void k_head_fwd_f32_c128(const float* __restrict__ x, const float* __restrict__ w, const float* __restrict__ bias,
-                                                            float* __restrict__ y, int HW, int Co, int ntiles) {
-    extern __shared__ __attribute__((aligned(16))) float hf_lds[];
+struct HeadBN {
+    const float* mean;
+    const float* invstd;
+    const float* gamma;
+    const float* beta;
+};
+__device__ __forceinline__ f32x4 ldf4(const float* p) { return *reinterpret_cast<const f32x4*>(p); }
+__device__ __forceinline__ f32x4 head_bn4(f32x4 v, f32x4 mu, f32x4 is, f32x4 g, f32x4 b, bool relu) {
+    f32x4 o;
+#pragma unroll
+    for (int t = 0; t < 4; ++t) {
+        o[t] = bn_affine(v[t], mu[t], is[t], g[t], b[t]);
+        if (relu) o[t] = fmaxf(o[t], 0.f);
+    }
+    return o;
+}
+template <bool BN, bool RELU>
+__device__ __forceinline__ void head_fwd_f32_c128(float* __restrict__ hf_lds, const float* __restrict__ x, const float* __restrict__ w,
+                                                  const float* __restrict__ bias, float* __restrict__ y, int HW, int Co, int ntiles, HeadBN bn) {
     const int lane = threadIdx.x & 63, wave = __builtin_amdgcn_readfirstlane(threadIdx.x >> 6);
     float* const T = hf_lds + wave * (HF_NST * 2048);
     const uint32_t t_base = lds_addr(T);
@@ -689,6 +738,14 @@
     for (int j = 0; j < 8; ++j) {
         bw[j] = f32x4{0.f, 0.f, 0.f, 0.f};
         if (row < Co) bw[j] = *reinterpret_cast<const f32x4*>(w + row * 128 + 16 * j + 4 * kq);
+    }
+    f32x4 pm[BN ? 8 : 1], pi[BN ? 8 : 1], pg[BN ? 8 : 1], pb[BN ? 8 : 1];
+    if constexpr (BN) {
+#pragma unroll
+        for (int j = 0; j < 8; ++j) {
+            const int c = 16 * j + 4 * kq;
+            pm[j] = ldf4(bn.mean + c); pi[j] = ldf4(bn.invstd + c); pg[j] = ldf4(bn.gamma + c); pb[j] = ldf4(bn.beta + c);
+        }
     }
     const float bv = row < Co ? bias[row] : 0.f;
     const int nwaves = gridDim.x * 4;
@@ -715,6 +772,10 @@
         for (int j = 0; j < 8; ++j) a[j] = lds_read128_async<0>(a0 + (uint32_t)(((4 * j + kq) ^ row) << 4));
         SD_LDS_WAIT4(0, a[0], a[1], a[2], a[3]);
         SD_LDS_WAIT4(0, a[4], a[5], a[6], a[7]);
+        if constexpr (BN) {
+#pragma unroll
+            for (int j = 0; j < 8; ++j) a[j] = head_bn4(a[j], pm[j], pi[j], pg[j], pb[j], RELU);
+        }
         f32x4 acc0 = {0.f, 0.f, 0.f, 0.f}, acc1 = {0.f, 0.f, 0.f, 0.f};
 #pragma unroll
         for (int j = 0; j < 8; j += 2)
@@ -733,6 +794,17 @@
     }
     wait_vmcnt<0>();
 #undef HF_ISSUE
+}
+__global__ __launch_bounds__(256) void k_head_fwd_f32_c128(const float* __restrict__ x, const float* __restrict__ w, const float* __restrict__ bias,
+                                                            float* __restrict__ y, int HW, int Co, int ntiles) {
+    extern __shared__ __attribute__((aligned(16))) float hf_lds[];
+    head_fwd_f32_c128<false, false>(hf_lds, x, w, bias, y, HW, Co, ntiles, HeadBN{});
+}
+template <bool RELU>
+__global__ __launch_bounds__(256) void k_head_fwd_f32_c128_bn(const float* __restrict__ x, const float* __restrict__ w, const float* __restrict__ bias,
+                                                               float* __restrict__ y, int HW, int Co, int ntiles, HeadBN bn) {
+    extern __shared__ __attribute__((aligned(16))) float hf_lds[];
+    head_fwd_f32_c128<true, RELU>(hf_lds, x, w, bias, y, HW, Co, ntiles, bn);
 }
 
 constexpr int HEAD_WG_PIX = 1024;
@@ -907,9 +979,9 @@
 }
 
 constexpr int HWG_STAGE = 2048 + 256;
-__global__ __launch_bounds__(256) void k_head_wgrad_f32_c128(const float* __restrict__ dy, const float* __restrict__ x, float* __restrict__ partial,
-                                                              int HW, int Co, int ntiles) {
-    extern __shared__ __attribute__((aligned(16))) float hw_lds[];
+template <bool BN, bool RELU>
+__device__ __forceinline__ void head_wgrad_f32_c128(float* __restrict__ hw_lds, const float* __restrict__ dy, const float* __restrict__ x,
+                                                    float* __restrict__ partial, int HW, int Co, int ntiles, HeadBN bn) {
     const int lane = threadIdx.x & 63, wave = __builtin_amdgcn_readfirstlane(threadIdx.x >> 6);
     float* const T = hw_lds + wave * (HF_NST * HWG_STAGE);
     const uint32_t t_base = lds_addr(T);
@@ -917,6 +989,14 @@
     const int gw = blockIdx.x * 4 + wave, nwaves = gridDim.x * 4;
     const int dr = lane >> 5, dsl = lane & 31;
     const int nco = min(n, Co - 1);
+    f32x4 pm[BN ? 2 : 1], pi[BN ? 2 : 1], pg[BN ? 2 : 1], pb[BN ? 2 : 1];
+    if constexpr (BN) {
+#pragma unroll
+        for (int h = 0; h < 2; ++h) {
+            const int c = 64 * h + 4 * n;
+            pm[h] = ldf4(bn.mean + c); pi[h] = ldf4(bn.invstd + c); pg[h] = ldf4(bn.gamma + c); pb[h] = ldf4(bn.beta + c);
+        }
+    }
 #define HWG_ISSUE(t_, st_)                                                                                         \
     {                                                                                                              \
         const uint32_t m0_ = (uint32_t)min((t_), ntiles - 1) * 16u;                              \
@@ -951,6 +1031,13 @@
         SD_LDS_WAIT4(0, xa[0], xa[1], xa[2], xa[3]);
         SD_LDS_WAIT4(0, xb[0], xb[1], xb[2], xb[3]);
         SD_LDS_WAIT2(0, a, xa[0]);
+        if constexpr (BN) {
+#pragma unroll
+            for (int i = 0; i < 4; ++i) {
+                xa[i] = head_bn4(xa[i], pm[0], pi[0], pg[0], pb[0], RELU);
+                xb[i] = head_bn4(xb[i], pm[1], pi[1], pg[1], pb[1], RELU);
+            }
+        }
         if (n >= Co) a = f32x4{0.f, 0.f, 0.f, 0.f};
 #pragma unroll
         for (int i = 0; i < 4; ++i)
@@ -976,6 +1063,17 @@
     bsum += __shfl_xor(bsum, 16);
     bsum += __shfl_xor(bsum, 32);
     if (kq == 0 && n < Co) dst[Co * 128 + n] = bsum;
+}
+__global__ __launch_bounds__(256) void k_head_wgrad_f32_c128(const float* __restrict__ dy, const float* __restrict__ x, float* __restrict__ partial,
+                                                              int HW, int Co, int ntiles) {
+    extern __shared__ __attribute__((aligned(16))) float hw_lds[];
+    head_wgrad_f32_c128<false, false>(hw_lds, dy, x, partial, HW, Co, ntiles, HeadBN{});
+}
+template <bool RELU>
+__global__ __launch_bounds__(256) void k_head_wgrad_f32_c128_bn(const float* __restrict__ dy, const float* __restrict__ x, float* __restrict__ partial,
+                                                                 int HW, int Co, int ntiles, HeadBN bn) {
+    extern __shared__ __attribute__((aligned(16))) float hw_lds[];
+    head_wgrad_f32_c128<true, RELU>(hw_lds, dy, x, partial, HW, Co, ntiles, bn);
 }
 
 __global__ __launch_bounds__(256) void k_head_wgrad_fin(const float* __restrict__ partial, int nblocks, int n, float* __restrict__ dw,
@@ -1463,6 +1561,24 @@
     const int64_t n4 = M * C / 4;
     hipLaunchKernelGGL(k_bn_apply<float>, dim3(ew_grid(n4)), dim3(256), 0, (hipStream_t)stream, x, y, n4, C, mean, invstd, gamma, beta, residual, relu,
                        relu_mask_out);
+    SD_LAUNCH_CHECK();
+    return 0;
+}
+
+int sd_bn_apply_res_bn_supported(int64_t M, int C) { return check_mc("sd_bn_apply_res_bn", M, C) == 0 ? 1 : 0; }
+
+int sd_bn_apply_res_bn(const float* x, float* y, int64_t M, int C, const float* mean, const float* invstd, const float* gamma, const float* beta,
+                       const float* residual, const float* res_mean, const float* res_invstd, const float* res_gamma, const float* res_beta,
+                       int relu, uint8_t* relu_mask_out, sd_stream_t stream) {
+    if (int e = check_mc("sd_bn_apply_res_bn", M, C)) return e;
+    SD_REQUIRE(x && y && mean && invstd && gamma && beta && residual && res_mean && res_invstd && res_gamma && res_beta, SD_ERR_INVALID,
+               "sd_bn_apply_res_bn: null pointer");
+    SD_REQUIRE(aligned16(x) && aligned16(y) && aligned16(residual) && aligned16(mean) && aligned16(invstd) && aligned16(gamma) && aligned16(beta) &&
+               aligned16(res_mean) && aligned16(res_invstd) && aligned16(res_gamma) && aligned16(res_beta), SD_ERR_ALIGN,
+               "sd_bn_apply_res_bn: tensors and parameters must be 16-byte aligned");
+    const int64_t n4 = M * C / 4;
+    hipLaunchKernelGGL(k_bn_apply_resbn, dim3(ew_grid(n4)), dim3(256), 0, (hipStream_t)stream, x, y, n4, C, mean, invstd, gamma, beta, residual,
+                       res_mean, res_invstd, res_gamma, res_beta, relu, relu_mask_out);
     SD_LAUNCH_CHECK();
     return 0;
 }
@@ -1799,6 +1915,40 @@
     return 0;
 }
 
+static bool head_bn_shape_ok(int B, int HW, int C, int Co) {
+    return B > 0 && HW > 0 && C == 128 && Co > 0 && Co <= 16 && HW % 16 == 0 && (int64_t)B * HW < (1ll << 31);
+}
+static int head_bn_check(const char* what, const float* mean, const float* invstd, const float* gamma, const float* beta, int B, int HW, int C, int Co) {
+    SD_REQUIRE(head_bn_shape_ok(B, HW, C, Co), SD_ERR_INVALID, "%s: needs C == 128, 1 <= Co <= 16, HW %% 16 == 0, B * HW < 2^31", what);
+    SD_REQUIRE(mean && invstd && gamma && beta, SD_ERR_INVALID, "%s: null BatchNorm parameter", what);
+    SD_REQUIRE(aligned16(mean) && aligned16(invstd) && aligned16(gamma) && aligned16(beta), SD_ERR_ALIGN, "%s: BatchNorm parameters must be 16-byte aligned", what);
+    return 0;
+}
+int sd_head_fwd_bn_supported(int B, int HW, int C, int Co) { return head_bn_shape_ok(B, HW, C, Co) ? 1 : 0; }
+int sd_head_bwd_bn_supported(int B, int HW, int C, int Co) { return head_bn_shape_ok(B, HW, C, Co) ? 1 : 0; }
+
+int sd_head_fwd_bn(const float* x, const float* w, const float* bias, float* y, int B, int HW, int C, int Co, const float* mean, const float* invstd,
+                   const float* gamma, const float* beta, int relu, sd_stream_t stream) {
+    SD_REQUIRE(x && w && bias && y, SD_ERR_INVALID, "sd_head_fwd_bn: null pointer");
+    if (int e = head_bn_check("sd_head_fwd_bn", mean, invstd, gamma, beta, B, HW, C, Co)) return e;
+    SD_REQUIRE(aligned16(x) && aligned16(w) && aligned16(y), SD_ERR_ALIGN, "sd_head_fwd_bn: x, w and y must be 16-byte aligned");
+    const int ntiles = (int)((int64_t)B * HW / 16);
+    const size_t lds_b = (size_t)4 * HF_NST * 2048 * sizeof(float);
+    const HeadBN bn{mean, invstd, gamma, beta};
+    const dim3 grid(std::min(cdiv(ntiles, 4), 256));
+    if (relu) {
+        static const hipError_t attr_once = hipFuncSetAttribute(reinterpret_cast<const void*>(&k_head_fwd_f32_c128_bn<true>), hipFuncAttributeMaxDynamicSharedMemorySize, (int)lds_b);
+        SD_HIP(attr_once);
+        hipLaunchKernelGGL(k_head_fwd_f32_c128_bn<true>, grid, dim3(256), lds_b, (hipStream_t)stream, x, w, bias, y, HW, Co, ntiles, bn);
+    } else {
+        static const hipError_t attr_once = hipFuncSetAttribute(reinterpret_cast<const void*>(&k_head_fwd_f32_c128_bn<false>), hipFuncAttributeMaxDynamicSharedMemorySize, (int)lds_b);
+        SD_HIP(attr_once);
+        hipLaunchKernelGGL(k_head_fwd_f32_c128_bn<false>, grid, dim3(256), lds_b, (hipStream_t)stream, x, w, bias, y, HW, Co, ntiles, bn);
+    }
+    SD_LAUNCH_CHECK();
+    return 0;
+}
+
 static int head_wgrad_wave_rows(int64_t M) { return (int)std::min<int64_t>(1024, (cdiv(M, 16) + 3) / 4 * 4); }
 size_t sd_head_bwd_workspace_bytes(int B, int HW, int C, int Co) {
     const int64_t M = (int64_t)B * HW;
@@ -1846,6 +1996,36 @@
     return 0;
 }
 
+int sd_head_bwd_bn(const float* dy, const float* x, const float* w, float* dx, float* dw, float* dbias, int B, int HW, int C, int Co,
+                   const float* mean, const float* invstd, const float* gamma, const float* beta, int relu, int accumulate, void* workspace,
+                   size_t workspace_bytes, sd_stream_t stream) {
+    SD_REQUIRE(dy && x && w && dx && dw && dbias && workspace, SD_ERR_INVALID, "sd_head_bwd_bn: null pointer");
+    if (int e = head_bn_check("sd_head_bwd_bn", mean, invstd, gamma, beta, B, HW, C, Co)) return e;
+    SD_REQUIRE(aligned16(x) && aligned16(dy), SD_ERR_ALIGN, "sd_head_bwd_bn: x and dy must be 16-byte aligned");
+    SD_REQUIRE(workspace_bytes >= sd_head_bwd_workspace_bytes(B, HW, C, Co), SD_ERR_WORKSPACE, "sd_head_bwd_bn: workspace too small");
+    const int64_t M = (int64_t)B * HW;
+    hipStream_t st = (hipStream_t)stream;
+    const int nb = head_wgrad_wave_rows(M);
+    const size_t lds_b = (size_t)4 * HF_NST * HWG_STAGE * sizeof(float);
+    const HeadBN bn{mean, invstd, gamma, beta};
+    if (relu) {
+        static const hipError_t attr_once = hipFuncSetAttribute(reinterpret_cast<const void*>(&k_head_wgrad_f32_c128_bn<true>), hipFuncAttributeMaxDynamicSharedMemorySize, (int)lds_b);
+        SD_HIP(attr_once);
+        hipLaunchKernelGGL(k_head_wgrad_f32_c128_bn<true>, dim3(nb / 4), dim3(256), lds_b, st, dy, x, (float*)workspace, HW, Co, (int)(M / 16), bn);
+    } else {
+        static const hipError_t attr_once = hipFuncSetAttribute(reinterpret_cast<const void*>(&k_head_wgrad_f32_c128_bn<false>), hipFuncAttributeMaxDynamicSharedMemorySize, (int)lds_b);
+        SD_HIP(attr_once);
+        hipLaunchKernelGGL(k_head_wgrad_f32_c128_bn<false>, dim3(nb / 4), dim3(256), lds_b, st, dy, x, (float*)workspace, HW, Co, (int)(M / 16), bn);
+    }
+    SD_LAUNCH_CHECK();
+    const int n = Co * C + Co;
+    hipLaunchKernelGGL(k_head_wgrad_fin, dim3(cdiv(n, 8)), dim3(256), 0, st, (const float*)workspace, nb, n, dw, dbias, Co * C, accumulate);
+    SD_LAUNCH_CHECK();
+    hipLaunchKernelGGL(k_head_dgrad<float>, dim3(cdiv(M, 64)), dim3(256), (size_t)Co * C * sizeof(float), st, dy, w, dx, M, HW, C, Co);
+    SD_LAUNCH_CHECK();
+    return 0;
+}
+
 int sd_head_bwd_bf16(const float* dy, const void* x_bf16, const float* w, void* dx_bf16, float* dw, float* dbias, int B, int HW, int C, int Co,
                      int accumulate, void* workspace, size_t workspace_bytes, sd_stream_t stream) {
     SD_REQUIRE(dy && x_bf16 && w && dx_bf16 && dw && dbias && workspace && B > 0 && HW > 0, SD_ERR_INVALID, "sd_head_bwd_bf16: bad arguments");
diff --git a/structuredetector_amd/model/network.py b/structuredetector_amd/model/network.py
--- a/structuredetector_amd/model/network.py
+++ b/structuredetector_amd/model/network.py
@@ -122,6 +122,7 @@
         self.stem_ring = True
         self.fuse_head = True
         self.small_batch_kernel = True
+        self.fold_bn = True
 
     def _kname(self, d, which):
         if self.prof is None:
@@ -238,6 +239,17 @@
         if update_running:
             self._nbt.append(bn.num_batches_tracked)
         return (y, mean, invstd, mask) if want_mask else (y, mean, invstd)
+
+    def bn_train_res_bn(self, x, bn: BNParams, stats, res, res_bn: BNParams, res_stats):
+        Mrows, Cc = x.numel() // x.shape[-1], x.shape[-1]
+        (mean, invstd), (rmean, rinvstd) = stats, res_stats
+        y = torch.empty_like(x)
+        mask = torch.empty(x.numel() // 4, dtype=torch.uint8, device=x.device)
+        L.check(self.lib.sd_bn_apply_res_bn(x.data_ptr(), y.data_ptr(), Mrows, Cc, mean.data_ptr(), invstd.data_ptr(), bn.weight.data_ptr(),
+                                            bn.bias.data_ptr(), res.data_ptr(), rmean.data_ptr(), rinvstd.data_ptr(), res_bn.weight.data_ptr(),
+                                            res_bn.bias.data_ptr(), 1, mask.data_ptr(), L.stream()), "sd_bn_apply_res_bn")
+        self._nbt += [res_bn.num_batches_tracked, bn.num_batches_tracked]
+        return y, mean, invstd, mask
 
     def bn_fold(self, bn: BNParams):
         cached = self.net._folded.get(id(bn))
@@ -310,11 +322,15 @@
                     c2, d2, st2 = self.conv_stats(a1, blk.conv2, B, d1.Ho, d1.Wo, blk.bn2, amp=amp)
                     if blk.downsample is not None:
                         cd, dd, std_ = self.conv_stats(cur, blk.downsample[0], B, Hc, Wc, blk.downsample[1], amp=amp)
-                        idt, md, idd = self.bn_train(cd, blk.downsample[1], relu=False, stats=std_)
+                        md, idd = std_
+                        if self.fold_bn and not amp and lib.sd_bn_apply_res_bn_supported(cd.numel() // cd.shape[-1], cd.shape[-1]):
+                            out, m2, i2, msk = self.bn_train_res_bn(c2, blk.bn2, st2, cd, blk.downsample[1], std_)
+                        else:
+                            idt, md, idd = self.bn_train(cd, blk.downsample[1], relu=False, stats=std_)
+                            out, m2, i2, msk = self.bn_train(c2, blk.bn2, res=idt, relu=True, stats=st2, want_mask=True)
                     else:
                         cd = dd = md = idd = None
-                        idt = cur
-                    out, m2, i2, msk = self.bn_train(c2, blk.bn2, res=idt, relu=True, stats=st2, want_mask=True)
+                        out, m2, i2, msk = self.bn_train(c2, blk.bn2, res=cur, relu=True, stats=st2, want_mask=True)
                     if rec:
                         blocks_tape.append((blk, cur, (Hc, Wc), d1, c1, a1, m1, i1, d2, c2, m2, i2, out, dd, cd, md, idd, msk))
                 else:
@@ -335,13 +351,22 @@
         T.push("fwd:fpn")
         f, _ = self.conv(p5, net.up1, B, H5, W5, shift=net.up1.bias, amp=amp, sb=not training)
         fpn_tape = []
+        hc = net.head.conv
+        head_bn = None
+        fold_head = training and not amp and self.fold_bn and bool(lib.sd_head_fwd_bn_supported(B, H2 * W2, hc.cin, hc.cout)) \
+            and bool(lib.sd_head_bwd_bn_supported(B, H2 * W2, hc.cin, hc.cout))
         for fpn, (sc_t, Hs, Ws) in ((net.up2, (p4, H4, W4)), (net.up3, (p3, H3, W3)), (net.up4, (p2, H2, W2))):
             t, dl = self.conv(sc_t, fpn.lateral, B, Hs, Ws, shift=fpn.lateral.bias, res=f, res_up2=True, amp=amp, sb=not training)
             if training:
                 c, dc, stf = self.conv_stats(t, fpn.conv[0], B, Hs, Ws, fpn.conv[1], amp=amp)
-                fn, mf, if_ = self.bn_train(c, fpn.conv[1], stats=stf)
+                if fold_head and fpn is net.up4:
+                    (mf, if_), fn = stf, c
+                    head_bn = (mf, if_, fpn.conv[1])
+                    self._nbt.append(fpn.conv[1].num_batches_tracked)
+                else:
+                    fn, mf, if_ = self.bn_train(c, fpn.conv[1], stats=stf)
                 if rec:
-                    fpn_tape.append((fpn, sc_t, (Hs, Ws), dl, t, dc, c, mf, if_, fn))
+                    fpn_tape.append((fpn, sc_t, (Hs, Ws), dl, t, dc, c, mf, if_, None if fn is c else fn))
             else:
                 sf, hf = self.bn_fold(fpn.conv[1])
                 fn, _ = self.conv(t, fpn.conv[0], B, Hs, Ws, scale=sf, shift=hf, relu=True, sb=True)
@@ -349,14 +374,18 @@
         T.pop()
 
         T.push("fwd:head")
-        hc = net.head.conv
         out = torch.empty((B, hc.cout, H2, W2), dtype=torch.float32, device=x.device)
-        head_fwd = lib.sd_head_fwd_bf16 if amp else lib.sd_head_fwd
-        L.check(head_fwd(f.data_ptr(), hc.weight.data_ptr(), hc.bias.data_ptr(), out.data_ptr(), B, H2 * W2, hc.cin, hc.cout,
-                         L.stream()), "sd_head_fwd")
+        if head_bn is not None:
+            mf, if_, bnf = head_bn
+            L.check(lib.sd_head_fwd_bn(f.data_ptr(), hc.weight.data_ptr(), hc.bias.data_ptr(), out.data_ptr(), B, H2 * W2, hc.cin, hc.cout,
+                                       mf.data_ptr(), if_.data_ptr(), bnf.weight.data_ptr(), bnf.bias.data_ptr(), 1, L.stream()), "sd_head_fwd_bn")
+        else:
+            head_fwd = lib.sd_head_fwd_bf16 if amp else lib.sd_head_fwd
+            L.check(head_fwd(f.data_ptr(), hc.weight.data_ptr(), hc.bias.data_ptr(), out.data_ptr(), B, H2 * W2, hc.cin, hc.cout,
+                             L.stream()), "sd_head_fwd")
         T.pop()
         if rec:
-            tape.update(blocks=blocks_tape, fpn=fpn_tape, p5=(p5, H5, W5), f1=f, B=B, hw=(H2, W2))
+            tape.update(blocks=blocks_tape, fpn=fpn_tape, p5=(p5, H5, W5), f1=f, f1_bn=head_bn, B=B, hw=(H2, W2))
         if self._nbt:
             torch._foreach_add_(self._nbt, 1)
             self._nbt = []
@@ -598,6 +627,13 @@
             L.check(lib.sd_head_bwd_bf16(dhead.data_ptr(), f1.data_ptr(), hc.weight.data_ptr(), df.data_ptr(), net.grad_of(hc.weight).data_ptr(),
                                          net.grad_of(hc.bias).data_ptr(), B, H2 * W2, hc.cin, hc.cout, 0, ws.data_ptr(), ws.numel(), L.stream()),
                     "sd_head_bwd_bf16")
+        elif tape.get("f1_bn") is not None:
+            f1 = tape["f1"]
+            mf, if_, bnf = tape["f1_bn"]
+            df = torch.empty_like(f1)
+            L.check(lib.sd_head_bwd_bn(dhead.data_ptr(), f1.data_ptr(), hc.weight.data_ptr(), df.data_ptr(), net.grad_of(hc.weight).data_ptr(),
+                                       net.grad_of(hc.bias).data_ptr(), B, H2 * W2, hc.cin, hc.cout, mf.data_ptr(), if_.data_ptr(),
+                                       bnf.weight.data_ptr(), bnf.bias.data_ptr(), 1, 0, ws.data_ptr(), ws.numel(), L.stream()), "sd_head_bwd_bn")
         else:
             f1 = self._to_f32(tape["f1"]) if amp else tape["f1"]
             df = torch.empty_like(f1)
```

Result: no change. 881.0 (median of 6 runs) (+0.2%).
